# ucsdmanorlab/bootstrapper

Measured on AMD Instinct MI355X. Metric: Mvoxels/s predict+segment, 1024^3 vol in 128^3 blocks, higher is better.
Workload: dtype bf16x3

## Files before the change

### bootstrapper_amd/_lib.py

```python
import ctypes as C
import os

import torch

_HERE = os.path.dirname(os.path.abspath(__file__))
LIB_PATH = os.environ.get("BSMI_LIB") or os.path.join(_HERE, "libbsmi.so")

MAX_LEVELS, MAX_CONVS, MAX_HEADS, NAME_LEN = 8, 4, 4, 32
PREC_F32, PREC_BF16, PREC_BF16X3 = 0, 1, 2
RAW_U8, RAW_F32, RAW_U8_UNIT = 0, 1, 2
ERR_INVALID, ERR_HIP, ERR_STATE, ERR_MISSING, ERR_OVERFLOW = -1, -2, -3, -4, -5


class UNetConfig(C.Structure):
    _fields_ = [
        ("in_channels", C.c_int32),
        ("num_fmaps", C.c_int32),
        ("fmap_inc_factor", C.c_int32),
        ("num_levels", C.c_int32),
        ("downsample_factors", (C.c_int32 * 3) * MAX_LEVELS),
        ("n_convs_down", C.c_int32 * MAX_LEVELS),
        ("kernel_size_down", ((C.c_int32 * 3) * MAX_CONVS) * MAX_LEVELS),
        ("n_convs_up", C.c_int32 * MAX_LEVELS),
        ("kernel_size_up", ((C.c_int32 * 3) * MAX_CONVS) * MAX_LEVELS),
        ("num_heads", C.c_int32),
        ("head_name", (C.c_char * NAME_LEN) * MAX_HEADS),
        ("head_dims", C.c_int32 * MAX_HEADS),
        ("num_fmaps_out", C.c_int32),
    ]


class StepInfo(C.Structure):
    _fields_ = [("type", C.c_int32), ("materialised", C.c_int32), ("shape", C.c_int32 * 4), ("conv_index", C.c_int32),
                ("form", C.c_int32), ("flags", C.c_int32), ("bn", C.c_int32), ("ksteps", C.c_int32), ("head", C.c_int32),
                ("factor", C.c_int32 * 3), ("offset", C.c_int32 * 3), ("prefix", C.c_char * 64)]


class TrainWgradInfo(C.Structure):
    _fields_ = [(n, C.c_int32) for n in ("family", "residual", "n", "c", "cbase", "kx", "tile_n", "tile_c", "ranges", "lines_per_range",
                                         "det_workspace")]


class TrainStepInfo(C.Structure):
    _fields_ = [("type", C.c_int32), ("n_wgrad", C.c_int32), ("wgrad", TrainWgradInfo * 4), ("dgrad", C.c_int32), ("dgrad_raw", C.c_int32),
                ("dgrad_converted", C.c_int32), ("dgrad_bn", C.c_int32), ("dgrad_ksteps", C.c_int32), ("dgrad_split_k", C.c_int32),
                ("dgrad_scatter", C.c_int32), ("dgrad_residual", C.c_int32), ("border", C.c_int32 * 3), ("has_split", C.c_int32),
                ("bias", C.c_int32), ("up", C.c_int32), ("fwd_split", C.c_int32), ("deterministic", C.c_int32)]


WGRAD_FAMILIES = ("none", "wave-f32", "tiled-f32", "split-bf16")
TRAIN_TENSORS = {"dout": 0, "gmask": 1, "gsplit": 2, "gsplit_hi": 3, "gsplit_lo": 4, "dcat": 5, "head_dp": 6, "pad_count": 7}
STEP_TYPES = ("input", "conv", "pool", "up", "head")
CONV_FORMS = ("gather", "raster-halo", "box-halo", "halo-resident", "first-pass", "winograd F(2x2)", "winograd F(4x4)")
STEP_FLAGS = {1: "fused-up", 2: "res-low", 4: "split-k"}
STEP_BELOW_UP = 8


class Codec(C.Structure):
    _fields_ = [("id", C.c_int32), ("level", C.c_int32), ("cname", C.c_int32), ("shuffle", C.c_int32),
                ("typesize", C.c_int32), ("blocksize", C.c_int32)]


class ChunkCopy(C.Structure):
    _fields_ = [("path", C.c_char_p), ("base", C.c_void_p), ("start", C.c_int64 * 4), ("extent", C.c_int64 * 4),
                ("stride", C.c_int64 * 4), ("read_modify_write", C.c_int32), ("reserved", C.c_int32)]


class BatchFragArgs(C.Structure):
    _fields_ = [("affs_dev", C.c_void_p), ("frags_dev", C.c_void_p), ("max_id_dev", C.c_void_p), ("labels_dev", C.c_void_p),
                ("num_labels_dev", C.c_void_p), ("id_offset", C.c_uint64), ("size_dev", C.c_void_p), ("sums_dev", C.c_void_p)]


class BatchGraphArgs(C.Structure):
    _fields_ = [("affs_dev", C.c_void_p), ("frags_dev", C.c_void_p), ("edges_dev", C.c_void_p), ("sums_dev", C.c_void_p),
                ("pair_counts_dev", C.c_void_p), ("counts_dev", C.c_void_p), ("edge_capacity", C.c_uint64)]


class Aug2dDraw(C.Structure):
    _fields_ = [("a", C.c_float * 4), ("src", C.c_float * 2), ("inv_spacing", C.c_float * 2), ("flags", C.c_int32), ("n", C.c_int32 * 2),
                ("lattice_offset", C.c_int32), ("crop", C.c_int32 * 2), ("crop_offset", C.c_int32), ("reserved", C.c_int32)]


class Aug2dIDraw(C.Structure):
    _fields_ = [("seed", C.c_uint64), ("impulse_threshold", C.c_uint64), ("noise_sigma", C.c_float), ("contrast_scale", C.c_float),
                ("nodes", C.c_int32), ("radius", C.c_int32), ("taps_offset", C.c_int32), ("reserved", C.c_int32 * 3)]


CODEC_RAW, CODEC_ZLIB, CODEC_GZIP, CODEC_ZSTD, CODEC_LZ4, CODEC_BLOSC = range(6)
BLOSC_LZ4, BLOSC_ZLIB, BLOSC_ZSTD = 1, 3, 4
CHUNK_MISSING = 1
MORPH_DILATE, MORPH_ERODE = 0, 1
RESCALE_DOWN, RESCALE_UP = 0, 1


class BsmiError(RuntimeError):
    def __init__(self, code, msg):
        super().__init__(f"libbsmi error {code}: {msg}")
        self.code = code
        self.msg = msg


def _load():
    if not os.path.exists(LIB_PATH):
        raise ImportError(
            f"{LIB_PATH} not found: build it with `python -c 'import __graft_entry__ as g; g.build()'` "
            "(or `make -C bootstrapper_amd/csrc`).  There is no CPU fallback.")
    lib = C.CDLL(LIB_PATH)
    p, i32, i64p, vp = C.c_void_p, C.c_int, C.POINTER(C.c_int64), C.c_void_p
    sigs = {
        "bsmi_last_error": (C.c_char_p, []),
        "bsmi_version": (i32, []),
        "bsmi_unet_create": (i32, [C.POINTER(UNetConfig), i32, C.POINTER(p)]),
        "bsmi_unet_destroy": (i32, [p]),
        "bsmi_unet_load_weight": (i32, [p, C.c_char_p, vp, i64p, i32]),
        "bsmi_unet_finalize": (i32, [p, i32]),
        "bsmi_unet_output_shape": (i32, [p, i64p, i64p]),
        "bsmi_unet_flops": (i32, [p, i64p, C.POINTER(C.c_double)]),
        "bsmi_unet_forward": (i32, [p, i32, vp, i32, i64p, C.POINTER(vp), C.POINTER(vp), vp]),
        "bsmi_unet_debug_activation": (i32, [p, i32, i32, i64p, vp, C.c_uint64]),
        "bsmi_unet_debug_step_info": (i32, [p, i32, C.POINTER(StepInfo), C.POINTER(i32)]),
        "bsmi_unet_profile_enable": (i32, [p, i32]),
        "bsmi_unet_profile_read": (i32, [p, i32, C.POINTER(i32), C.POINTER(C.c_int32), C.POINTER(C.c_double),
                                         C.POINTER(C.c_double)]),
        "bsmi_unet_profile_totals": (i32, [p, C.POINTER(C.c_double), C.POINTER(C.c_double), i64p, i32]),
        "bsmi_extract_block_reflect_u8": (i32, [vp, i64p, i64p, i64p, vp, vp]),
        "bsmi_seg_create": (i32, [i32, i64p, C.POINTER(p)]),
        "bsmi_seg_destroy": (i32, [p]),
        "bsmi_ws_fragments_u8": (i32, [p, vp, i64p, i32, i32, vp, vp, vp]),
        "bsmi_ws_fragments_seeds_u8": (i32, [p, vp, i64p, i32, i32, vp, vp, vp, vp]),
        "bsmi_rag_agglomerate_u8": (i32, [p, vp, vp, i64p, C.c_float, C.c_int, vp]),
        "bsmi_rag_edge_stats": (i32, [p, vp, vp, C.c_uint64, vp]),
        "bsmi_agglomerate_mean_u8": (i32, [p, vp, vp, i64p, C.POINTER(C.c_float), i32, vp, vp]),
        "bsmi_agglomerate_hist_u8": (i32, [p, vp, vp, i64p, C.POINTER(C.c_float), i32, i32, i32, vp, vp]),
        "bsmi_agglomerate_hist_graph": (i32, [C.c_uint32, C.c_uint32, vp, vp, vp, i32, i32, C.POINTER(C.c_float), i32, vp]),
        "bsmi_frag_postprocess_u8": (i32, [p, vp, vp, i64p, C.c_double, C.c_int64, i64p, i64p, C.c_uint64, vp, vp, vp]),
        "bsmi_label_stats": (i32, [p, vp, i64p, C.c_uint64, C.c_uint64, vp, vp, vp]),
        "bsmi_rag_merge_scores_u8": (i32, [p, vp, vp, i64p, C.c_float, C.c_int, vp, vp, C.c_uint64, vp, vp, vp, vp]),
        "bsmi_lut_relabel": (i32, [C.c_int, vp, C.c_uint64, vp, vp, C.c_uint64, vp, vp]),
        "bsmi_lut_relabel_multi": (i32, [i32, vp, C.c_uint64, vp, vp, C.c_uint64, i32, vp, vp]),
        "bsmi_connected_components": (i32, [vp, C.c_uint64, vp, vp, C.c_uint64, C.c_float, vp]),
        "bsmi_connected_components_multi": (i32, [vp, C.c_uint64, vp, vp, C.c_uint64, vp, C.c_int, vp]),
        "bsmi_cc_affs_u8": (i32, [p, vp, i64p, C.c_int, C.c_int64, vp, vp, vp, vp]),
        "bsmi_mws_agglom_f64": (i32, [C.c_int, vp, C.c_int, vp, vp, C.c_uint32, i64p, vp, vp]),
        "bsmi_mws_cluster": (i32, [C.c_uint64, vp, vp, C.c_uint64, vp]),
        "bsmi_frag_pair_affinity_u8": (i32, [C.c_int, vp, C.c_int, vp, vp, i64p, C.c_uint64, vp, vp, vp, vp, vp]),
        "bsmi_label_table_u64": (i32, [p, vp, i64p, C.c_int64, vp, vp, vp, vp, C.c_uint64, vp, vp]),
        "bsmi_seg_status": (i32, [p, vp]),
        "bsmi_seg_set_host_flood": (i32, [p, i32]),
        "bsmi_seg_batch_create": (i32, [C.POINTER(p), i32, C.POINTER(p)]),
        "bsmi_seg_batch_destroy": (i32, [p]),
        "bsmi_seg_batch_fragments_u8": (i32, [p, i32, C.POINTER(BatchFragArgs), i64p, i32, i32, C.c_double, C.c_int64, i64p, i64p, C.c_uint64, vp]),
        "bsmi_seg_batch_rag_graph_u8": (i32, [p, i32, C.POINTER(BatchGraphArgs), i64p, vp]),
        "bsmi_rag_graph_u8": (i32, [p, vp, vp, i64p, vp, vp, vp, C.c_uint64, vp, vp]),
        "bsmi_rag_merge_scores_host": (i32, [i32, vp, vp, vp, vp, C.c_float, i32, vp, i32]),
        "bsmi_rag_merge_scores_host_rule": (i32, [i32, vp, vp, vp, vp, C.c_float, i32, i32, vp, i32]),
        "bsmi_unet_train_set_arithmetic": (i32, [p, i32]),
        "bsmi_unet_train_set_deterministic": (i32, [p, i32]),
        "bsmi_unet_train_begin": (i32, [p, i64p]),
        "bsmi_unet_train_forward_backward": (i32, [p, vp, C.POINTER(C.c_void_p), C.POINTER(C.c_void_p), C.POINTER(C.c_float), vp]),
        "bsmi_unet_train_num_params": (i32, [p, C.POINTER(C.c_uint64)]),
        "bsmi_unet_train_buffers": (i32, [p, C.POINTER(C.c_void_p), C.POINTER(C.c_void_p)]),
        "bsmi_unet_train_param_info": (i32, [p, C.c_char_p, C.POINTER(C.c_uint64), C.POINTER(C.c_uint64)]),
        "bsmi_unet_train_adam_step": (i32, [p, C.c_float, C.c_float, C.c_float, C.c_float, C.c_float, vp]),
        "bsmi_unet_train_read_param": (i32, [p, C.c_char_p, C.c_int, vp]),
        "bsmi_unet_train_last_loss": (i32, [p, C.POINTER(C.c_float), vp]),
        "bsmi_unet_train_prediction": (i32, [p, i32, C.POINTER(C.c_void_p), C.POINTER(C.c_uint64)]),
        "bsmi_unet_train_grad_groups": (i32, [p, i32, C.POINTER(i32), C.POINTER(C.c_uint64), C.POINTER(C.c_uint64)]),
        "bsmi_unet_train_wait_grad_group": (i32, [p, i32, vp]),
        "bsmi_unet_train_write_param": (i32, [p, C.c_char_p, C.c_int, vp]),
        "bsmi_unet_train_step_count": (i32, [p, C.c_int, C.POINTER(C.c_int)]),
        "bsmi_unet_train_end": (i32, [p]),
        "bsmi_unet_train_debug_tensor": (i32, [p, i32, i32, i64p, vp, C.c_uint64]),
        "bsmi_unet_train_debug_step_info": (i32, [p, i32, C.POINTER(TrainStepInfo)]),
        "bsmi_train_affinity_targets": (i32, [C.c_int, vp, vp, i64p, C.POINTER(C.c_int32), C.c_int, C.c_int, C.c_int, C.c_float,
                                              C.c_float, vp, vp, vp]),
        "bsmi_train_lsd_targets": (i32, [C.c_int, vp, vp, i64p, i64p, i64p, C.POINTER(C.c_float), C.POINTER(C.c_float), C.c_int, vp, vp, vp]),
        "bsmi_train_lsd2d_targets": (i32, [C.c_int, vp, vp, C.c_int, i64p, i64p, i64p, C.POINTER(C.c_float), C.POINTER(C.c_float), C.c_int,
                                           vp, vp, vp]),
        "bsmi_train_affinity_targets_roi": (i32, [C.c_int, vp, vp, C.c_int, i64p, i64p, i64p, C.POINTER(C.c_int32), C.c_int, C.c_int,
                                                  C.c_int, C.c_float, C.c_float, vp, vp, vp]),
        "bsmi_train_mask_sat": (i32, [C.c_int, vp, C.c_int, C.c_int, C.c_int, vp, vp]),
        "bsmi_unet_set_persistent_grid": (i32, [p, C.c_int]),
        "bsmi_unet_profile_executed": (i32, [p, C.POINTER(C.c_double), C.c_int]),
        "bsmi_debug_lds_canary": (i32, [i32, i32, i32, vp, vp]),
        "bsmi_debug_check_guards": (i32, []),
        "bsmi_stream_create_cu_mask": (i32, [C.c_int, vp, C.c_int, C.POINTER(C.c_void_p)]),
        "bsmi_stream_destroy": (i32, [C.c_int, vp]),
        "bsmi_eval_create": (i32, [i32, C.c_uint64, C.POINTER(p)]),
        "bsmi_eval_destroy": (i32, [p]),
        "bsmi_eval_aff_errors_u8": (i32, [p, vp, i64p, i64p, vp, i32, i64p, vp, C.POINTER(C.c_int32), i64p, C.c_float, C.c_float,
                                          C.c_int64, vp, vp, vp, vp]),
        "bsmi_eval_lsd_errors_u8": (i32, [p, vp, i64p, i64p, vp, vp, i64p, i64p, i64p, i64p, C.POINTER(C.c_float), C.POINTER(C.c_float),
                                          i32, C.c_float, C.c_float, C.c_int64, C.c_uint64, vp, vp, vp, vp, vp, vp, vp, vp]),
        "bsmi_eval_pairs_u64": (i32, [p, vp, vp, vp, i64p, i32, vp]),
        "bsmi_eval_pairs_read": (i32, [p, vp, vp, vp, C.c_uint64, vp, vp]),
        "bsmi_eval_status": (i32, [p, vp]),
        "bsmi_label_morph_u64": (i32, [i32, vp, i64p, i32, i32, i32, vp, vp, vp]),
        "bsmi_label_fill_holes_scratch_bytes": (C.c_size_t, [i64p, C.c_uint64]),
        "bsmi_label_fill_holes_u64": (i32, [i32, vp, i64p, i32, vp, vp, C.c_size_t, C.c_uint64, C.POINTER(C.c_uint64), vp]),
        "bsmi_mask_closing_work_bytes": (C.c_size_t, [i64p, i32]),
        "bsmi_mask_closing_disk_u8": (i32, [i32, vp, i64p, i32, vp, vp, C.c_size_t, vp]),
        "bsmi_downscale_mean": (i32, [i32, vp, i32, i64p, C.POINTER(C.c_int32), C.POINTER(C.c_int32), vp, i64p, vp]),
        "bsmi_rescale_sample": (i32, [i32, vp, i32, i64p, C.POINTER(C.c_int32), C.POINTER(C.c_int32), i32, vp, i64p, vp]),
        "bsmi_nonzero_bbox": (i32, [i32, vp, i32, i64p, i64p, vp, vp]),
        "bsmi_synth_create": (i32, [i32, i64p, C.POINTER(p)]),
        "bsmi_synth_destroy": (i32, [p]),
        "bsmi_synth_dilate_points": (i32, [p, i64p, vp, i32, vp, vp, vp, vp, vp]),
        "bsmi_synth_label_i32": (i32, [p, vp, i64p, vp, C.POINTER(C.c_uint64), vp]),
        "bsmi_synth_expand_i32": (i32, [p, vp, i64p, i32, C.c_int32, vp, vp]),
        "bsmi_synth_tubes_i32": (i32, [p, vp, i64p, vp, C.POINTER(C.c_uint64), vp]),
        "bsmi_synth_gaussian_f32": (i32, [p, vp, i64p, vp, i32, vp, vp]),
        "bsmi_synth_argmax_filter_f32": (i32, [p, vp, i64p, i32, vp, vp]),
        "bsmi_synth_basins_f32": (i32, [p, vp, vp, vp, i64p, vp, C.POINTER(C.c_uint64), vp]),
        "bsmi_synth_finish_i32": (i32, [p, vp, i64p, i32, i32, i32, vp, vp]),
        "bsmi_synth_grow_boundary_i64": (i32, [i32, vp, i64p, C.c_uint64, i32, vp, vp]),
        "bsmi_synth_merge_i64": (i32, [i32, vp, i64p, C.POINTER(C.c_int32), i32, C.c_int64, C.c_int64, vp]),
        "bsmi_synth_stamp_i64": (i32, [i32, vp, i64p, i32, i32, i32, vp, i32, i32, C.c_int64, vp]),
        "bsmi_synth_present_i64": (i32, [p, vp, C.c_uint64, vp, C.c_uint32, C.POINTER(C.c_uint32), vp]),
        "bsmi_synth_split_i64": (i32, [p, vp, i64p, C.c_int64, i32, C.POINTER(C.c_int32), i32, C.c_int64, C.POINTER(C.c_uint64), vp]),
        "bsmi_aug_coords": (i32, [i32, i64p, C.POINTER(C.c_float), C.POINTER(C.c_float), C.POINTER(C.c_float), i32, i32, vp, vp,
                                  C.POINTER(C.c_int32), C.POINTER(C.c_float), vp, vp]),
        "bsmi_aug_sample_f32_u8": (i32, [i32, vp, i64p, i64p, i64p, vp, i64p, vp, vp]),
        "bsmi_aug_sample_nearest_i64": (i32, [i32, vp, i64p, i64p, i64p, vp, i64p, vp, vp]),
        "bsmi_aug_sample_nearest_u8": (i32, [i32, vp, i64p, i64p, i64p, vp, i64p, vp, vp]),
        "bsmi_aug_sample_unit_f32_u8": (i32, [i32, vp, i64p, i64p, i64p, vp, i64p, vp, vp]),
        "bsmi_aug_noise_f32": (i32, [i32, i64p, vp, C.c_uint64, C.c_float, vp]),
        "bsmi_aug_section_stats_f32": (i32, [i32, i64p, vp, vp, vp, vp]),
        "bsmi_aug_intensity_f32": (i32, [i32, i64p, vp, vp, vp, vp, vp]),
        "bsmi_aug_gamma_f32": (i32, [i32, i64p, vp, vp, vp, vp]),
        "bsmi_aug_impulse_f32": (i32, [i32, i64p, vp, C.c_uint64, C.c_uint64, vp]),
        "bsmi_aug_smooth_f32": (i32, [i32, i64p, vp, vp, C.POINTER(C.c_float), i32, vp]),
        "bsmi_aug_defect_f32": (i32, [i32, i64p, vp, vp, vp, C.c_float, i32, vp]),
        "bsmi_aug2d_coords": (i32, [i32, C.POINTER(Aug2dDraw), vp, i32, i32, i64p, i64p, i64p, vp, vp, C.c_int64, vp, vp]),
        "bsmi_aug2d_sample_f32_u8": (i32, [i32, C.POINTER(Aug2dDraw), vp, i32, i32, vp, i64p, i64p, i64p, vp, C.c_int64, vp, vp]),
        "bsmi_aug2d_sample_nearest_i64": (i32, [i32, C.POINTER(Aug2dDraw), vp, i32, i32, vp, i64p, i64p, i64p, vp, C.c_int64, vp, vp]),
        "bsmi_aug2d_sample_nearest_u8": (i32, [i32, C.POINTER(Aug2dDraw), vp, i32, i32, vp, i64p, i64p, i64p, vp, C.c_int64, vp, vp]),
        "bsmi_aug2d_sample_unit_f32_u8": (i32, [i32, C.POINTER(Aug2dDraw), vp, C.POINTER(Aug2dIDraw), vp, i32, i32, vp, i64p, i64p, i64p, vp,
                                                C.c_int64, vp, vp]),
        "bsmi_aug2d_noise_f32": (i32, [i32, C.POINTER(Aug2dIDraw), vp, i32, i32, i64p, vp, vp]),
        "bsmi_aug2d_intensity_f32": (i32, [i32, C.POINTER(Aug2dIDraw), vp, i32, i32, i64p, vp, vp, vp, vp, vp]),
        "bsmi_aug2d_gamma_f32": (i32, [i32, C.POINTER(Aug2dIDraw), vp, i32, i32, i64p, vp, vp, vp, vp]),
        "bsmi_aug2d_impulse_f32": (i32, [i32, C.POINTER(Aug2dIDraw), vp, i32, i32, i64p, vp, vp]),
        "bsmi_aug2d_smooth_f32": (i32, [i32, C.POINTER(Aug2dIDraw), vp, i32, i32, i64p, vp, vp, vp, C.c_int64, vp]),
        "bsmi_aug2d_defect_f32": (i32, [i32, C.POINTER(Aug2dIDraw), vp, i32, i32, i64p, vp, vp, C.POINTER(C.c_int32), vp, i32, vp]),
        "bsmi_augin_group_mean_f32": (i32, [i32, i64p, vp, vp, i32, vp, vp]),
        "bsmi_augin_intensity_f32": (i32, [i32, i64p, vp, vp, vp, vp, i32, vp]),
        "bsmi_augin_smooth_f32": (i32, [i32, i64p, vp, vp, vp, vp, i32, vp]),
        "bsmi_augin_contrast_f32": (i32, [i32, i64p, vp, vp, vp, C.c_float, vp]),
        "bsmi_codec_bound": (C.c_size_t, [C.POINTER(Codec), C.c_size_t]),
        "bsmi_codec_decode": (i32, [C.POINTER(Codec), vp, C.c_size_t, vp, C.c_size_t, C.POINTER(C.c_size_t)]),
        "bsmi_codec_encode": (i32, [C.POINTER(Codec), vp, C.c_size_t, vp, C.c_size_t, C.POINTER(C.c_size_t)]),
        "bsmi_chunks_read": (i32, [C.POINTER(Codec), i32, C.POINTER(C.c_char_p), C.POINTER(vp), C.POINTER(C.c_size_t),
                                   C.POINTER(C.c_size_t), C.POINTER(i32), i32]),
        "bsmi_chunks_write": (i32, [C.POINTER(Codec), i32, C.POINTER(C.c_char_p), C.POINTER(vp), C.POINTER(C.c_size_t),
                                    C.POINTER(i32), i32]),
        "bsmi_blosc_dev_frame_bound": (C.c_size_t, [C.c_size_t]),
        "bsmi_blosc_dev_scratch_bytes": (C.c_size_t, [i32, C.c_size_t]),
        "bsmi_blosc_encode_dev_u64": (i32, [i32, vp, C.c_int64, C.c_int64, i32, i64p, i64p, i64p, vp, C.c_size_t, vp, C.c_size_t, vp, vp]),
        "bsmi_blosc_dev_u8_frame_bound": (C.c_size_t, [C.c_size_t]),
        "bsmi_blosc_dev_u8_scratch_bytes": (C.c_size_t, [i32, C.c_size_t]),
        "bsmi_blosc_encode_dev_u8": (i32, [i32, vp, i64p, i32, i64p, i64p, i64p, vp, C.c_size_t, vp, C.c_size_t, vp, vp]),
        "bsmi_rag_write_sqlite": (i32, [C.c_char_p, C.c_uint64, vp, vp, vp, C.c_uint64, vp, vp]),
        "bsmi_chunks_read_into": (i32, [C.POINTER(Codec), i32, C.POINTER(ChunkCopy), i64p, i32, vp, C.POINTER(i32), i32]),
        "bsmi_chunks_write_from": (i32, [C.POINTER(Codec), i32, C.POINTER(ChunkCopy), i64p, i32, vp, C.POINTER(i32), i32]),
    }
    for name, (res, args) in sigs.items():
        fn = getattr(lib, name)
        fn.restype = res
        fn.argtypes = args
    return lib, sorted(sigs)


lib, SYMBOLS = _load()
# ... 14 lines not shown
```

### bootstrapper_amd/csrc/unet_debug.hip

```cpp
#include <cstring>

#include "unet_internal.h"

extern "C" {

int bsmi_unet_debug_activation(bsmi_unet* h, int step, int what, int64_t shape_out[4], float* host_out, uint64_t capacity) {
  if (!h || !shape_out) BSMI_FAIL(BSMI_ERR_INVALID, "null argument");
  Plan* plan = h->last_plan;
  if (!plan) BSMI_FAIL(BSMI_ERR_STATE, "no forward has run");
  if (step < 0 || step >= (int)plan->steps.size()) BSMI_FAIL(BSMI_ERR_INVALID, "step %d out of range (%zu steps)", step, plan->steps.size());
  const PlanStep& st = plan->steps[step];
  if (st.type == PlanStep::HEAD) BSMI_FAIL(BSMI_ERR_INVALID, "head steps write into the caller's buffers");
  if (plan->fused_first && step < 2)
    BSMI_FAIL(BSMI_ERR_STATE, "step %d is not materialised: the first ConvPass ran as one launch (first_pass), which writes step 2 only", step);
  if (st.type == PlanStep::UP && st.skip)
    BSMI_FAIL(BSMI_ERR_STATE, "step %d is not materialised: the upsampling is fused into the Winograd stages that read it", step);
  const TDesc& t = st.out;
  shape_out[0] = t.D; shape_out[1] = t.H; shape_out[2] = t.W; shape_out[3] = t.C;
  if (!host_out) return BSMI_OK;
  const size_t nvox = (size_t)t.D * t.H * t.W;
  if (capacity < nvox * t.C) BSMI_FAIL(BSMI_ERR_INVALID, "buffer of %llu floats too small", (unsigned long long)capacity);
  BSMI_HIP(hipSetDevice(h->device));
  BSMI_HIP(hipDeviceSynchronize());
  const int es = esize(plan->prec);
  const bool split = t.lo_off != 0;
  const size_t bytes = nvox * t.Cpad * es * (split ? 2 : 1);
  std::vector<uint8_t> raw(bytes);
  BSMI_HIP(hipMemcpy(raw.data(), t.ptr, raw.size(), hipMemcpyDeviceToHost));
  for (size_t v = 0; v < nvox; ++v)
    for (int c = 0; c < t.C; ++c) {
      float x;
      if (plan->prec == BSMI_PREC_F32) {
        x = ((const float*)raw.data())[v * t.Cpad + c];
      } else if (!split) {
        x = host_bf16_to_f32(((const uint16_t*)raw.data())[v * t.Cpad + c]);
      } else {
        const size_t i = 2 * v * t.Cpad + (size_t)((c >> 3) << 4) + (c & 7);
        const float hi = host_bf16_to_f32(((const uint16_t*)raw.data())[i]);
        const float lo = host_bf16_to_f32(((const uint16_t*)raw.data())[i + 8]);
        x = what == 1 ? hi : (what == 2 ? lo : hi + lo);
      }
      host_out[v * t.C + c] = x;
    }
  return BSMI_OK;
}

int bsmi_unet_debug_step_info(bsmi_unet* h, int step, bsmi_unet_step_info* info, int* n_steps) {
  if (!h) BSMI_FAIL(BSMI_ERR_INVALID, "null handle");
  Plan* plan = h->last_plan;
  if (!plan) BSMI_FAIL(BSMI_ERR_STATE, "no forward has run");
  if (n_steps) *n_steps = (int)plan->steps.size();
  if (!info) return BSMI_OK;
  if (step < 0 || step >= (int)plan->steps.size()) BSMI_FAIL(BSMI_ERR_INVALID, "step %d out of range (%zu steps)", step, plan->steps.size());
  const PlanStep& st = plan->steps[step];
  memset(info, 0, sizeof *info);
  info->type = (int32_t)st.type;
  const bool in_first = plan->fused_first && step < 3;
  info->materialised = !((plan->fused_first && step < 2) || (st.type == PlanStep::UP && st.skip));
  const TDesc& t = st.type == PlanStep::HEAD ? st.in : st.out;
  info->shape[0] = t.D; info->shape[1] = t.H; info->shape[2] = t.W;
  info->shape[3] = st.type == PlanStep::HEAD ? h->heads[st.head].cout : t.C;
  const std::string* prefix = nullptr;
  if (st.type == PlanStep::HEAD) {
    info->head = st.head;
    prefix = &h->heads[st.head].prefix;
  } else if (st.type == PlanStep::POOL || st.type == PlanStep::UP) {
    for (int d = 0; d < 3; ++d) { info->factor[d] = st.f[d]; info->offset[d] = st.type == PlanStep::UP ? st.o[d] : 0; }
  } else if (st.type == PlanStep::CONV) {
    prefix = &st.site->prefix;
    info->conv_index = st.ci;
    const int sk_grid = h->sk_grid > 0 ? h->sk_grid : 0;
    if (in_first) {
      info->form = BSMI_FORM_FIRST_PASS;
    } else if (st.use_wino) {
      info->form = st.wino_in.m == 4 ? BSMI_FORM_WINO4 : BSMI_FORM_WINO2;
      info->bn = tile_bn(st.tile);
      info->ksteps = st.wino_gemm.nsteps;
      bool up = false;
      for (int q = 0; q < st.wino_in.nsrc; ++q) up = up || st.wino_in.upf[q] > 0;
      if (up || st.wino_out.low || st.wino_has_below) info->flags |= BSMI_STEP_FUSED_UP;
      if (st.wino_has_below) info->flags |= BSMI_STEP_BELOW_UP;
      if (st.wino_has_res_low) info->flags |= BSMI_STEP_RES_LOW;
      if (conv_igemm_split_k(st.wino_gemm, plan->prec, st.tile, sk_grid) ||
          (st.wino_has_res && conv_igemm_split_k(st.wino_res, plan->prec, st.tile, sk_grid)) ||
          (st.wino_has_res_low && conv_igemm_split_k(st.wino_res_low, plan->prec, st.tile, sk_grid)) ||
          (st.wino_has_below && conv_igemm_split_k(st.wino_below, plan->prec, st.below_tile, sk_grid)))
        info->flags |= BSMI_STEP_SPLIT_K;
    } else if (st.use_h16) {
      info->form = BSMI_FORM_HALO_RESIDENT;
      info->bn = st.h16.Npad;
      info->ksteps = st.h16.nsteps;
    } else if (st.use_box) {
      info->form = BSMI_FORM_BOX_HALO;
    } else if (st.use_rh) {
      info->form = BSMI_FORM_RASTER_HALO;
      info->bn = tile_bn(st.tile);
      info->ksteps = st.rh.nsteps;
      if (conv_rh_split_k(st.rh, st.tile, sk_grid)) info->flags |= BSMI_STEP_SPLIT_K;
    } else {
      info->form = BSMI_FORM_GATHER;
      info->bn = tile_bn(st.tile);
      info->ksteps = st.conv.nsteps;
      if (conv_igemm_split_k(st.conv, plan->prec, st.tile, sk_grid)) info->flags |= BSMI_STEP_SPLIT_K;
    }
  }
  if (prefix) snprintf(info->prefix, sizeof info->prefix, "%s", prefix->c_str());
  return BSMI_OK;
}

}
```

### bootstrapper_amd/csrc/unet_internal.h

```cpp
#pragma once
#include <cstring>
#include <map>
#include <memory>
#include <string>
#include <vector>

#include "conv_igemm.h"
#include "conv_rh.h"
#include "conv_h16.h"
#include "conv_box.h"
#include "first_pass.h"
#include "wino.h"

namespace bsmi {

struct HostWeight {
  std::vector<int64_t> shape;
  std::vector<float> data;
  bool loaded = false;
};

struct PackEntry {
  int slot;
  int dz, dy, dx;
  int c0;
  int wsrc;
  int tap;
  int cin_base;
  int creal;
  bool dummy;
  int phase;
};

struct PackPhase {
  int slot, c0, kind, first_unit, nunits;
};

struct PackedConv {
  bool ready = false;
  std::vector<PackEntry> entries;
  std::vector<PackPhase> phases;
  void* w = nullptr;
  int ks = 1;
  size_t lo_image_bytes = 0;
  float* bias = nullptr;
  int Npad = 0;
  TileCfg tile = TILE_256x32;
};

struct PackedWino {
  bool ready = false;
  int m = 2;
  bool fused_only = false;
  std::vector<WinoUnit> units;
  std::vector<int> cin_of_v;
  int Cv = 0;
  void* w = nullptr;
  size_t lo_image_bytes = 0, batch_bytes = 0;
  int Npad = 0;
  TileCfg tile = TILE_256x32;
  std::vector<PackEntry> res_entries;
  void* res_w = nullptr;
  size_t res_lo_image_bytes = 0;
  std::vector<PackEntry> res_part[2];
  void* res_part_w[2] = {nullptr, nullptr};
  size_t res_part_lo[2] = {0, 0};
  bool below_ready = false;
  std::vector<WinoUnit> skip_units, below_units;
  std::vector<int> skip_cin_of_v;
  int skip_Cv = 0;
  void* skip_w = nullptr;
  size_t skip_lo_image_bytes = 0, skip_batch_bytes = 0;
  void* below_w = nullptr;
  size_t below_lo_image_bytes = 0, below_batch_bytes = 0;
  int below_Npad = 0;
  bool below_dense = false;
  TileCfg below_tile = TILE_256x320;
};

struct H16PhaseHost {
  int slot, c0, dz, kind;
  int first_step, nsteps;
};
struct PackedH16 {
  bool ready = false;
  std::vector<PackEntry> entries;
  std::vector<H16PhaseHost> phases;
  void* w = nullptr;
  size_t lo_image_bytes = 0;
  int Npad = 0;
};

struct PassSite {
  std::string prefix;
  int nslots = 1;
  int cin[2] = {0, 0};
  int cout = 0;
  int nconv = 0;
  int k[BSMI_MAX_CONVS][3];
  PackedConv packed[BSMI_NUM_PREC][BSMI_MAX_CONVS];
  PackedWino wino[BSMI_MAX_CONVS];
  PackedH16 h16[BSMI_MAX_CONVS];
};

struct HeadSite {
  std::string prefix;
  int cin = 0, cout = 0;
  float* hw = nullptr;
  float* hb = nullptr;
};

struct TDesc {
  void* ptr = nullptr;
  int C = 0, Cpad = 0, D = 0, H = 0, W = 0;
  size_t lo_off = 0;
};

struct PlanStep {
  enum Type { INPUT, CONV, POOL, UP, HEAD } type;
  ConvArgs conv;
  RhArgs rh;
  bool use_rh = false;
  H16Args h16;
  bool use_h16 = false;
  int h16_rows = 0;
  BoxArgs box;
  bool use_box = false;
  bool use_wino = false;
  WinoInArgs wino_in;
  ConvArgs wino_gemm, wino_res, wino_res_low;
  bool wino_has_res = false, wino_has_res_low = false;
  ConvArgs wino_below;
  bool wino_has_below = false;
  TileCfg below_tile = TILE_256x320;
  WinoOutArgs wino_out;
  TileCfg tile;
  TDesc in, out;
  int f[3], o[3];
  bool skip = false;
  bool pool_fused = false;
  int head = 0;
  double flops = 0;
  double exec_flops = 0;
  struct PassSite* site = nullptr;
  int ci = 0;
  TDesc slots[kMaxConvTensors];
  int so[kMaxConvTensors][3] = {{0, 0, 0}, {0, 0, 0}, {0, 0, 0}};
  int nsl = 0;
  struct TrainFwdX3* tx3 = nullptr;
};

struct Plan {
  std::vector<float> last_ms;
  bool pending = false;
  std::vector<void*> allocs;
  std::vector<PlanStep> steps;
  int64_t out_shape[3] = {0, 0, 0};
  double flops = 0;
  size_t bytes = 0;
  std::vector<hipEvent_t> events;
  std::vector<std::vector<hipEvent_t>> inflight, spare;
  bool profiled = false;
  bool fused_first = false;
  int prec = 0;
};

struct TrainState;

static inline uint16_t host_f32_to_bf16(float f) {
  uint32_t u;
  memcpy(&u, &f, 4);
  if ((u & 0x7fffffffu) > 0x7f800000u) return (uint16_t)((u >> 16) | 0x40);
  u += 0x7fffu + ((u >> 16) & 1u);
  return (uint16_t)(u >> 16);
}
static inline float host_bf16_to_f32(uint16_t b) {
  const uint32_t u = (uint32_t)b << 16;
  float f;
  memcpy(&f, &u, 4);
  return f;
}

int esize(int prec);
int ksplit(int prec);
int bke(int prec);
int sube(int prec);
void build_entries(const PassSite& p, int ci, int prec, std::vector<PackEntry>& out, std::vector<PackPhase>* phases_out = nullptr);

}

using namespace bsmi;

struct bsmi_unet {
  bsmi_unet_config cfg;
  int device = 0;
  int nl = 0;
  std::vector<PassSite> l_conv, r_conv;
  std::vector<HeadSite> heads;
  int crop_factor[BSMI_MAX_LEVELS][3];
  std::map<std::string, HostWeight> weights;
  bool finalized[BSMI_NUM_PREC] = {false, false, false};
  int profile_period = 0;
  uint64_t profile_count = 0;
  Plan* last_plan = nullptr;
  double prof_ms[5] = {0, 0, 0, 0, 0}, prof_flops[5] = {0, 0, 0, 0, 0};
  double prof_exec = 0;
  int64_t prof_launches[5] = {0, 0, 0, 0, 0};
  std::map<std::vector<int64_t>, std::unique_ptr<Plan>> plans;
  float* sk_ws = nullptr;
  int sk_grid = 0;
  int sk_request = -1;
  bsmi::TrainState* train = nullptr;
  bool train_forward = false;
  int train_split = 1;
  int train_det = 0;
  bsmi::FirstPassWeights first_pass;
  bsmi::FirstPassWeights first_pass_x3;
};

namespace bsmi {
int pack_conv(bsmi_unet* h, PassSite& p, int ci, int prec);
int pack_wino(bsmi_unet* h, PassSite& p, int ci);
int pack_h16(bsmi_unet* h, PassSite& p, int ci);
void release(PackedConv& pc);
void release(PackedWino& pw);
void release(PackedH16& ph);

bool x3_fused_for(TileCfg tile);
bool wino_eligible(const PassSite& p, int ci);
int wino_tile_edge();
bool wino_narrow_last(const bsmi_unet* h, const PassSite& p, int ci);
bool below_up_site(const bsmi_unet* h, const PassSite& p, int ci);
bool fuse_up_enabled();
bool pool_fuse_enabled();
int h16_mode();
int h16_only_npad();
bool h16_balanced();
bool rh_enabled(int prec, TileCfg tile, size_t nsteps);
bool box_enabled();
bool first_pass_eligible(const bsmi_unet* h);

int check_shape_arg(const int64_t s[3]);
int get_plan(bsmi_unet* h, int precision, const int64_t in_shape[3], Plan** out);
int dry_plan(bsmi_unet* h, const int64_t in_shape[3], Plan& plan);
void free_plan(Plan* p);
void free_train_state(bsmi_unet* h);
int train_forward_conv_x3(bsmi_unet* h, const PlanStep& st, hipStream_t s);
int train_refresh_f32_images(bsmi_unet* h, hipStream_t s);
}
```

### bootstrapper_amd/csrc/unet_pack.hip

```cpp
#include <cstdlib>
#include <cstring>

#include "unet_internal.h"

#include "dev_guard.h"

namespace bsmi {

int esize(int prec) { return prec == BSMI_PREC_F32 ? 4 : 2; }
int ksplit(int prec) { return prec == BSMI_PREC_BF16X3 ? 3 : 1; }
int bke(int prec) { return kStepRowBytes / esize(prec); }
int sube(int prec) { return 32 / esize(prec); }

static inline void split_bf16(float v, uint16_t& hi, uint16_t& lo) {
  hi = host_f32_to_bf16(v);
  lo = host_f32_to_bf16(v - host_bf16_to_f32(hi));
}

template <class T>
static void release_image(T*& w) {
  if (w) (void)hipFree(w);
  w = nullptr;
}
void release(PackedConv& pc) {
// ... 27 lines not shown
  auto add_taps = [&](int slot, const int* k, int cin_base, int creal) {
    const int cpad = round_up(creal, kChanPad);
    if (cpad == SUB) {
      PackPhase ph{slot, 0, 0, (int)out.size(), 0};
      for (int z = 0; z < k[0]; ++z)
        for (int y = 0; y < k[1]; ++y)
          for (int x = 0; x < k[2]; x += kUnitsPerStep)
            for (int j = 0; j < kUnitsPerStep; ++j) {
              if (x + j < k[2])
                out.push_back(PackEntry{slot, z, y, x + j, 0, 0, (z * k[1] + y) * k[2] + x + j, cin_base, creal, false, (int)phases.size()});
              else
                out.push_back(PackEntry{slot, 0, 0, 0, 0, 0, 0, 0, 0, true, (int)phases.size()});
            }
      close_phase(ph);
      return;
    }
    for (int c32 = 0; c32 < cpad; c32 += kUnitsPerStep * SUB) {
      PackPhase ph{slot, c32, 0, (int)out.size(), 0};
      for (int z = 0; z < k[0]; ++z)
        for (int y = 0; y < k[1]; ++y)
          for (int x = 0; x < k[2]; ++x) {
            for (int c0 = c32; c0 < std::min(cpad, c32 + kUnitsPerStep * SUB); c0 += SUB)
              out.push_back(PackEntry{slot, z, y, x, c0, 0, (z * k[1] + y) * k[2] + x, cin_base, creal, false, (int)phases.size()});
            while ((out.size() - ph.first_unit) % kUnitsPerStep)
              out.push_back(PackEntry{slot, 0, 0, 0, 0, 0, 0, 0, 0, true, (int)phases.size()});
          }
      close_phase(ph);
    }
  };
  auto add_residual = [&](int slot, const int* crop, int cin_base, int creal) {
    const int cpad = round_up(creal, kChanPad);
    for (int c32 = 0; c32 < cpad; c32 += kUnitsPerStep * SUB) {
      PackPhase ph{slot, c32, 1, (int)out.size(), 0};
      for (int c0 = c32; c0 < std::min(cpad, c32 + kUnitsPerStep * SUB); c0 += SUB)
        out.push_back(PackEntry{slot, crop[0] / 2, crop[1] / 2, crop[2] / 2, c0, 1, 0, cin_base, creal, false, (int)phases.size()});
      close_phase(ph);
    }
  };
  const int* k = p.k[ci];
  if (ci == 0) {
    int base = 0;
    for (int s = 0; s < p.nslots; ++s) {
      add_taps(s, k, base, p.cin[s]);
      base += p.cin[s];
    }
  } else {
    add_taps(0, k, 0, p.cout);
  }
  if (last) {
    int crop[3] = {0, 0, 0};
    for (int i = 0; i < p.nconv; ++i)
      for (int d = 0; d < 3; ++d) crop[d] += p.k[i][d] - 1;
    const int first_slot = ci == 0 ? 0 : 1;
    int base = 0;
    for (int s = 0; s < p.nslots; ++s) {
      add_residual(first_slot + s, crop, base, p.cin[s]);
      base += p.cin[s];
    }
  }
  if ((out.size() / kUnitsPerStep) % 2)
    for (int j = 0; j < kUnitsPerStep; ++j) out.push_back(PackEntry{0, 0, 0, 0, 0, 0, 0, 0, 0, true, (int)phases.size() - 1});
  if (phases_out) *phases_out = phases;
}

int pack_conv(bsmi_unet* h, PassSite& p, int ci, int prec) {
  PackedConv& pc = p.packed[prec][ci];
  if (pc.ready) return BSMI_OK;
  pc.entries.clear();
  build_entries(p, ci, prec, pc.entries, &pc.phases);
  pc.tile = choose_tile(p.cout);
  pc.Npad = round_up(p.cout, tile_bn(pc.tile));
  const int BKE = bke(prec);
  const bool last = ci == p.nconv - 1;
  const HostWeight& wm = h->weights[p.prefix + ".conv_pass." + std::to_string(2 * ci) + ".weight"];
  const HostWeight& bm = h->weights[p.prefix + ".conv_pass." + std::to_string(2 * ci) + ".bias"];
  const HostWeight& wr = h->weights[p.prefix + ".residual.0.weight"];
  const HostWeight& br = h->weights[p.prefix + ".residual.0.bias"];
  const int64_t cin_m = wm.shape[1], ntap_m = wm.shape[2] * wm.shape[3] * wm.shape[4];
  const int64_t cin_r = wr.shape[1];
  const int SUB = sube(prec);
  const bool fused = prec == BSMI_PREC_BF16X3 && x3_fused_for(pc.tile);
  const int KS = pc.ks = fused ? 1 : ksplit(prec);
  const size_t nsteps = pc.entries.size() / kUnitsPerStep * KS;
  const size_t nelem = (nsteps * (size_t)pc.Npad + kWeightRowSlack) * BKE;
  std::vector<float> bias(pc.Npad, 0.f);
  for (int n = 0; n < p.cout; ++n) bias[n] = bm.data[n] + (last ? br.data[n] : 0.f);

  pc.lo_image_bytes = fused ? nelem * esize(prec) : 0;
  std::vector<uint8_t> packed(nelem * esize(prec) * (fused ? 2 : 1), 0);
  host_parallel_for((size_t)p.cout, [&](size_t n_) {
    const int n = (int)n_;
    for (size_t u = 0; u < pc.entries.size(); ++u) {
      const PackEntry& e = pc.entries[u];
      if (e.dummy) continue;
      const size_t s = u / kUnitsPerStep, j = u % kUnitsPerStep;
      for (int kk = 0; kk < SUB; ++kk) {
        const int c = e.c0 + kk;
        if (c >= e.creal) break;
        float v;
        if (e.wsrc == 0) v = wm.data[((size_t)n * cin_m + (e.cin_base + c)) * ntap_m + e.tap];
        else v = wr.data[(size_t)n * cin_r + (e.cin_base + c)];
        const size_t idx = (s * KS * pc.Npad + n) * BKE + j * SUB + kk;
        if (prec == BSMI_PREC_F32) {
          ((float*)packed.data())[idx] = v;
        } else if (prec == BSMI_PREC_BF16) {
          ((uint16_t*)packed.data())[idx] = host_f32_to_bf16(v);
        } else {
          uint16_t hi, lo;
          split_bf16(v, hi, lo);
          uint16_t* w16 = (uint16_t*)packed.data();
          if (fused) {
            w16[idx] = hi;
            w16[idx + nelem] = lo;
          } else {
            const size_t blk = (size_t)pc.Npad * BKE;
            w16[idx] = hi;
            w16[idx + blk] = hi;
            w16[idx + 2 * blk] = lo;
          }
        }
      }
    }
  });
  BSMI_HIP(hipMalloc(&pc.w, packed.size()));
  BSMI_HIP(hipMemcpy(pc.w, packed.data(), packed.size(), hipMemcpyHostToDevice));
  BSMI_HIP(hipMalloc((void**)&pc.bias, bias.size() * sizeof(float)));
  BSMI_HIP(hipMemcpy(pc.bias, bias.data(), bias.size() * sizeof(float), hipMemcpyHostToDevice));
  pc.ready = true;
  return BSMI_OK;
}

int pack_wino(bsmi_unet* h, PassSite& p, int ci) {
  PackedWino& pw = p.wino[ci];
  release(pw);
  pw.fused_only = wino_narrow_last(h, p, ci);
  if (!wino_eligible(p, ci) && !pw.fused_only) return BSMI_OK;
  const HostWeight& wm = h->weights[p.prefix + ".conv_pass." + std::to_string(2 * ci) + ".weight"];
  const HostWeight& wr = h->weights[p.prefix + ".residual.0.weight"];
  const int cin_m = (int)wm.shape[1];
  pw.cin_of_v.clear();
  if (ci == 0) {
    int base = 0;
    for (int s = 0; s < p.nslots; ++s) {
      for (int c = 0; c < round_up(p.cin[s], kChanPad); ++c) pw.cin_of_v.push_back(c < p.cin[s] ? base + c : -1);
      base += p.cin[s];
    }
  } else {
    for (int c = 0; c < round_up(p.cout, kChanPad); ++c) pw.cin_of_v.push_back(c < p.cout ? c : -1);
  }
  pw.Cv = (int)pw.cin_of_v.size();
  pw.m = wino_tile_edge();
  pw.tile = choose_tile(p.cout);
  pw.Npad = round_up(p.cout, tile_bn(pw.tile));
  wino_units(pw.Cv, pw.units);
  {
    size_t image_elems = 0, batch_elems = 0;
    static const bool on_host = [] { const char* e = getenv("BSMI_WINO_PACK_HOST"); return e && e[0] == '1'; }();
    if (on_host) {
      std::vector<uint16_t> packed;
      wino_pack_weights(wm.data.data(), p.cout, cin_m, pw.cin_of_v, pw.Npad, pw.units, packed, image_elems, batch_elems, pw.m);
      BSMI_HIP(hipMalloc(&pw.w, packed.size() * 2));
      BSMI_HIP(hipMemcpy(pw.w, packed.data(), packed.size() * 2, hipMemcpyHostToDevice));
    } else {
      const int rc = wino_pack_weights_dev(wm.data.data(), p.cout, cin_m, pw.cin_of_v, pw.Npad, pw.units, pw.m, &pw.w, image_elems, batch_elems);
      if (rc) return rc;
    }
    pw.lo_image_bytes = image_elems * 2;
    pw.batch_bytes = batch_elems * 2;
  }
  pw.res_entries.clear();
  if (ci == p.nconv - 1) {
    std::vector<PackEntry> all;
    build_entries(p, ci, BSMI_PREC_BF16X3, all);
    for (size_t u = 0; u + 1 < all.size(); u += kUnitsPerStep) {
      bool res = false;
      for (int j = 0; j < kUnitsPerStep; ++j) res |= !all[u + j].dummy && all[u + j].wsrc == 1;
      if (res)
        for (int j = 0; j < kUnitsPerStep; ++j) pw.res_entries.push_back(all[u + j]);
    }
    if ((pw.res_entries.size() / kUnitsPerStep) % 2)
      for (int j = 0; j < kUnitsPerStep; ++j) pw.res_entries.push_back(PackEntry{0, 0, 0, 0, 0, 0, 0, 0, 0, true, 0});
    const int64_t cin_r = wr.shape[1];
    auto pack_res = [&](const std::vector<PackEntry>& ents, void** w_out, size_t* lo_out) -> int {
      const size_t nsteps = ents.size() / kUnitsPerStep;
      const size_t nelem = (nsteps * (size_t)pw.Npad + kWeightRowSlack) * 32;
      std::vector<uint16_t> packed(2 * nelem, 0);
      for (size_t u = 0; u < ents.size(); ++u) {
        const PackEntry& e = ents[u];
        if (e.dummy) continue;
        const size_t s = u / kUnitsPerStep, j = u % kUnitsPerStep;
        for (int n = 0; n < p.cout; ++n)
          for (int kk = 0; kk < 16; ++kk) {
            const int c = e.c0 + kk;
            if (c >= e.creal) break;
            const float v = wr.data[(size_t)n * cin_r + (e.cin_base + c)];
            const size_t idx = (s * pw.Npad + n) * 32 + j * 16 + kk;
            split_bf16(v, packed[idx], packed[nelem + idx]);
          }
      }
      *lo_out = nelem * 2;
      BSMI_HIP(hipMalloc(w_out, packed.size() * 2));
      BSMI_HIP(hipMemcpy(*w_out, packed.data(), packed.size() * 2, hipMemcpyHostToDevice));
      return BSMI_OK;
    };
    int rc = pack_res(pw.res_entries, &pw.res_w, &pw.res_lo_image_bytes);
    if (rc) return rc;
    for (int part = 0; part < 2; ++part) pw.res_part[part].clear();
    if (p.nslots == 2) {
      const int up_slot = (ci == 0 ? 0 : 1) + 1;
      for (size_t u = 0; u + 1 < pw.res_entries.size(); u += kUnitsPerStep) {
        int slot = -1;
        for (int j = 0; j < kUnitsPerStep; ++j)
          if (!pw.res_entries[u + j].dummy) slot = pw.res_entries[u + j].slot;
        if (slot < 0) continue;
        for (int j = 0; j < kUnitsPerStep; ++j) pw.res_part[slot == up_slot ? 1 : 0].push_back(pw.res_entries[u + j]);
      }
      for (int part = 0; part < 2; ++part) {
        if ((pw.res_part[part].size() / kUnitsPerStep) % 2)
          for (int j = 0; j < kUnitsPerStep; ++j) pw.res_part[part].push_back(PackEntry{0, 0, 0, 0, 0, 0, 0, 0, 0, true, 0});
        if ((rc = pack_res(pw.res_part[part], &pw.res_part_w[part], &pw.res_part_lo[part]))) return rc;
      }
    }
  }
  if (below_up_site(h, p, ci) && pw.m == 4) {
    pw.skip_cin_of_v.assign(pw.cin_of_v.begin(), pw.cin_of_v.begin() + round_up(p.cin[0], kChanPad));
    pw.skip_Cv = (int)pw.skip_cin_of_v.size();
    wino_units(pw.skip_Cv, pw.skip_units);
    size_t image_elems = 0, batch_elems = 0;
    int rc = wino_pack_weights_dev(wm.data.data(), p.cout, cin_m, pw.skip_cin_of_v, pw.Npad, pw.skip_units, pw.m, &pw.skip_w, image_elems, batch_elems);
    if (rc) return rc;
    pw.skip_lo_image_bytes = image_elems * 2;
    pw.skip_batch_bytes = batch_elems * 2;
    const int cpad_low = round_up(p.cin[1], kChanPad), cpad_out = round_up(p.cout, kChanPad);
    wino_units(cpad_low, pw.below_units);
    pw.below_dense = p.cout <= 64;
    pw.below_tile = pw.below_dense ? TILE_256x320 : pw.tile;
    pw.below_Npad = pw.below_dense ? round_up(9 * cpad_out, tile_bn(pw.below_tile)) : pw.Npad;
    const size_t nsteps = pw.below_units.size() / kUnitsPerStep;
    const size_t tap_elems = nsteps * (size_t)pw.below_Npad * 32;
    const size_t nelem = (pw.below_dense ? 1 : 9) * tap_elems + (size_t)kWeightRowSlack * 32;
    std::vector<uint16_t> packed(2 * nelem, 0);
    const bool dense = pw.below_dense;
    const int cin1 = p.cin[1], cbase = p.cin[0];
    host_parallel_for((size_t)p.cout, [&](size_t n_) {
      const int n = (int)n_;
      for (size_t u = 0; u < pw.below_units.size(); ++u) {
        const WinoUnit& un = pw.below_units[u];
        if (un.dummy) continue;
        const size_t s = u / kUnitsPerStep, j = u % kUnitsPerStep;
        for (int kk = 0; kk < 16; ++kk) {
          const int c = un.vc0 + kk;
          if (c >= cin1) break;
          const float* g = wm.data.data() + (((size_t)n * cin_m + (cbase + c)) * 3 + un.kz) * 9;
          for (int tap = 0; tap < 9; ++tap) {
            const size_t idx = dense ? (s * pw.below_Npad + (size_t)tap * cpad_out + n) * 32 + j * 16 + kk
                                     : (size_t)tap * tap_elems + (s * pw.below_Npad + n) * 32 + j * 16 + kk;
            split_bf16(g[tap], packed[idx], packed[nelem + idx]);
          }
        }
      }
    });
    pw.below_lo_image_bytes = nelem * 2;
    pw.below_batch_bytes = dense ? 0 : tap_elems * 2;
    BSMI_HIP(hipMalloc(&pw.below_w, packed.size() * 2));
    BSMI_HIP(hipMemcpy(pw.below_w, packed.data(), packed.size() * 2, hipMemcpyHostToDevice));
    pw.below_ready = true;
  }
  pw.ready = true;
  return BSMI_OK;
}

static void build_entries_h16(const PassSite& p, int ci, std::vector<PackEntry>& out, std::vector<H16PhaseHost>& phases) {
  const bool last = ci == p.nconv - 1;
  const int* k = p.k[ci];
  const PackEntry dummy{0, 0, 0, 0, 0, 0, 0, 0, 0, true, 0};
  auto add_taps = [&](int slot, int cin_base, int creal) {
    const int cpad = round_up(creal, kChanPad);
    for (int z = 0; z < k[0]; ++z)
      for (int c0 = 0; c0 < cpad; c0 += 16) {
        H16PhaseHost ph{slot, c0, z, 0, (int)(out.size() / kUnitsPerStep), 0};
        const int ntap = k[1] * k[2];
        for (int i = 0; i < ntap; i += 2) {
          for (int j = 0; j < 2; ++j) {
            if (i + j < ntap) {
              const int y = (i + j) / k[2], x = (i + j) % k[2];
              out.push_back(PackEntry{slot, z, y, x, c0, 0, (z * k[1] + y) * k[2] + x, cin_base, creal, false, (int)phases.size()});
            } else {
              out.push_back(dummy);
            }
          }
          ++ph.nsteps;
        }
        phases.push_back(ph);
      }
  };
  if (ci == 0) {
    int base = 0;
    for (int s = 0; s < p.nslots; ++s) {
      add_taps(s, base, p.cin[s]);
      base += p.cin[s];
    }
  } else {
    add_taps(0, 0, p.cout);
  }
  if (last) {
    int crop[3] = {0, 0, 0};
    for (int i = 0; i < p.nconv; ++i)
      for (int d = 0; d < 3; ++d) crop[d] += p.k[i][d] - 1;
    const int first_slot = ci == 0 ? 0 : 1;
    int base = 0;
    for (int s = 0; s < p.nslots; ++s) {
      const int cpad = round_up(p.cin[s], kChanPad);
      for (int c0 = 0; c0 < cpad; c0 += 16) {
        phases.push_back(H16PhaseHost{first_slot + s, c0, crop[0] / 2, 1, (int)(out.size() / kUnitsPerStep), 1});
        out.push_back(PackEntry{first_slot + s, crop[0] / 2, crop[1] / 2, crop[2] / 2, c0, 1, 0, base, p.cin[s], false, (int)phases.size() - 1});
        out.push_back(dummy);
      }
// ... 43 lines not shown
```

### bootstrapper_amd/csrc/unet_plan.hip

```cpp
#include <algorithm>
#include <cmath>
#include <cstdlib>
#include <cstring>
#include <memory>

#include "unet_plan.h"

#include "dev_guard.h"

namespace bsmi {

int upload_ksteps(Plan* plan, const std::vector<KStep>& ks, ConvArgs& a) {
  KStep* dks = nullptr;
  BSMI_HIP(hipMalloc((void**)&dks, ks.size() * sizeof(KStep)));
  plan->allocs.push_back(dks);
  BSMI_HIP(hipMemcpy(dks, ks.data(), ks.size() * sizeof(KStep), hipMemcpyHostToDevice));
  a.steps = dks;
  a.nsteps = (int)ks.size();
  return BSMI_OK;
}

void set_strides(ConvArgs& a, const void* base, int H, int W, int C, int bytes_per_channel) {
  for (int sl = 0; sl < kMaxConvTensors; ++sl) {
    a.t[sl].base = (uint64_t)(uintptr_t)base;
// ... 308 lines not shown
    TDesc o;
    o.C = p.cout;
    o.D = sp[0] - (p.k[ci][0] - 1);
    o.H = sp[1] - (p.k[ci][1] - 1);
    o.W = sp[2] - (p.k[ci][2] - 1);
    if (o.D <= 0 || o.H <= 0 || o.W <= 0)
      BSMI_FAIL(BSMI_ERR_INVALID, "%s: input extent (%d,%d,%d) too small for kernel (%d,%d,%d)",
                p.prefix.c_str(), sp[0], sp[1], sp[2], p.k[ci][0], p.k[ci][1], p.k[ci][2]);
    int rc = alloc(o);
    if (rc) return rc;

    TDesc slots[kMaxConvTensors];
    int so[kMaxConvTensors][3] = {{0, 0, 0}, {0, 0, 0}, {0, 0, 0}};
    int nsl = 0;
    if (ci == 0) {
      for (int s = 0; s < p.nslots; ++s) {
        slots[nsl] = in[s];
        for (int d = 0; d < 3; ++d) so[nsl][d] = org[s][d];
        ++nsl;
      }
    } else {
      slots[nsl++] = cur;
      if (last)
        for (int s = 0; s < p.nslots; ++s) {
          slots[nsl] = in[s];
          for (int d = 0; d < 3; ++d) so[nsl][d] = org[s][d];
          ++nsl;
        }
    }

    const double M = (double)o.D * o.H * o.W;
    double kreal = 0;
    {
      std::vector<PackEntry> ents;
      build_entries(p, ci, prec, ents);
      for (auto& e : ents) if (!e.dummy) kreal += std::max(0, std::min(e.creal - e.c0, sube(prec)));
    }
    plan->flops += 2.0 * M * p.cout * kreal;

    if (!dry) {
      PackedConv& pc = p.packed[prec][ci];
      PlanStep st;
      st.type = PlanStep::CONV;
      st.tile = pc.tile;
      ConvArgs& a = st.conv;
      memset(&a, 0, sizeof a);
      const int KS = pc.ks;
      std::vector<KStep> ks(pc.entries.size() / kUnitsPerStep * KS);
      const int64_t es = esize(prec) * (prec == BSMI_PREC_BF16X3 ? 2 : 1);
      for (int sl = 0; sl < kMaxConvTensors; ++sl) {
        const TDesc& t = slots[sl < nsl ? sl : 0];
        a.t[sl].base = (uint64_t)(uintptr_t)t.ptr;
        a.t[sl].sz = (int32_t)((int64_t)t.H * t.W * t.Cpad * es);
        a.t[sl].sy = (int32_t)((int64_t)t.W * t.Cpad * es);
        a.t[sl].sx = (int32_t)((int64_t)t.Cpad * es);
      }
      for (size_t s = 0; s < ks.size() / KS; ++s) {
        const int slot = pc.entries[kUnitsPerStep * s].slot;
        const TDesc& t = slots[slot];
        KStep k;
        memset(&k, 0, sizeof k);
        k.tensor = slot;
        for (int j = 0; j < kUnitsPerStep; ++j) {
          const PackEntry& e = pc.entries[kUnitsPerStep * s + j];
          if (e.dummy) continue;
          const int64_t off = ((((int64_t)(e.dz + so[slot][0]) * t.H) + (e.dy + so[slot][1])) * t.W +
                               (e.dx + so[slot][2])) * t.Cpad + e.c0;
          k.delta[j] = (int32_t)(off * es);
        }
        ks[s * KS] = k;
        if (KS == 3) {
          KStep lo = k;
          for (int j = 0; j < kUnitsPerStep; ++j)
            if (!pc.entries[kUnitsPerStep * s + j].dummy) lo.delta[j] = (int32_t)(k.delta[j] + (int64_t)t.lo_off);
          ks[s * KS + 1] = lo;
          ks[s * KS + 2] = k;
        }
      }
      if ((rc = upload_ksteps(plan, ks, a))) return rc;
      a.w = pc.w;
      a.w_lo = pc.lo_image_bytes ? (const char*)pc.w + pc.lo_image_bytes : nullptr;
      a.bias = pc.bias;
      a.out = o.ptr;
      a.Do = o.D; a.Ho = o.H; a.Wo = o.W; a.Co = o.Cpad;
      a.M = o.D * o.H * o.W;
      a.Npad = pc.Npad;
      a.relu = 1;
      st.flops = 2.0 * M * p.cout * kreal;
      {
        const double x3 = prec == BSMI_PREC_BF16X3 ? 3.0 : 1.0;
        const double kstep = (double)kUnitsPerStep * sube(prec);
        st.exec_flops = 2.0 * (double)round_up(a.M, 256) * pc.Npad * ((double)(ks.size() / KS) * kstep) * x3;
      }
      st.site = &p;
      st.ci = ci;
      st.nsl = nsl;
      for (int sl = 0; sl < nsl; ++sl) {
        st.slots[sl] = slots[sl];
        for (int d = 0; d < 3; ++d) st.so[sl][d] = so[sl][d];
      }
      st.out = o;
      rc = plan_rh(p, ci, pc, slots, so, o, st);
      if (rc) return rc;
      rc = plan_box(p, ci, slots, so, o, st);
      if (rc) return rc;
      rc = plan_wino(p, ci, pc, slots, so, nsl, o, st);
      if (rc) return rc;
      if (!st.use_wino && !st.use_box) {
        rc = plan_h16(p, ci, pc, slots, so, o, st);
        if (rc) return rc;
      }
      if (getenv("BSMI_PLAN_DEBUG"))
        fprintf(stderr, "[bsmi plan] %s conv %d: out (%d,%d,%d)x%d tile BN=%d K-steps %d %s\n", p.prefix.c_str(), ci, o.D, o.H, o.W,
                p.cout, tile_bn(st.tile), st.use_wino ? st.wino_gemm.nsteps : a.nsteps,
                st.use_wino ? (st.wino_in.m == 4 ? "winograd F(4x4,3x3)" : "winograd F(2x2,3x3)") : st.use_h16 ? "halo-resident" : st.use_box ? "box-halo" : st.use_rh ? "raster-halo" : "gather");
      plan->steps.push_back(st);
    }
    cur = o;
    sp[0] = o.D; sp[1] = o.H; sp[2] = o.W;
  }
  out = cur;
  return BSMI_OK;
}

int Planner::rec(int level, const TDesc& f_in, TDesc& f_out) {
  const int i = h->nl - level - 1;
  TDesc f_left;
  const int org0[1][3] = {{0, 0, 0}};
  const int sp[3] = {f_in.D, f_in.H, f_in.W};
  int rc = pass(h->l_conv[i], &f_in, org0, sp, f_left);
  if (rc) return rc;
  if (level == 0) {
    f_out = f_left;
    return BSMI_OK;
  }
  const int* f = h->cfg.downsample_factors[i];
  const int dims[3] = {f_left.D, f_left.H, f_left.W};
  for (int d = 2; d >= 0; --d)
    if (dims[d] % f[d] != 0)
      BSMI_FAIL(BSMI_ERR_INVALID,
                "Can not downsample shape (%d, %d, %d) with factor (%d, %d, %d), mismatch in spatial dimension %d",
                dims[0], dims[1], dims[2], f[0], f[1], f[2], d);
  TDesc g_in;
  g_in.C = f_left.C; g_in.D = f_left.D / f[0]; g_in.H = f_left.H / f[1]; g_in.W = f_left.W / f[2];
  rc = alloc(g_in);
  if (rc) return rc;
  if (!dry) {
    PlanStep st;
    st.type = PlanStep::POOL;
    st.in = f_left; st.out = g_in;
    for (int d = 0; d < 3; ++d) st.f[d] = f[d];
    PlanStep& prod = plan->steps.back();
    if (pool_fuse_enabled() && prec == BSMI_PREC_BF16X3 && f[0] == 1 && f[1] == 2 && f[2] == 2 && prod.type == PlanStep::CONV && prod.use_wino &&
        prod.wino_out.m == 4 && !prod.wino_out.low && prod.wino_out.out == f_left.ptr && !(f_left.H & 1) && !(f_left.W & 1)) {
      prod.wino_out.pool = g_in.ptr;
      st.pool_fused = true;
    }
    plan->steps.push_back(st);
  }
  TDesc g_out;
  rc = rec(level - 1, g_in, g_out);
  if (rc) return rc;

  PassSite& rp = h->r_conv[i];
  const int up[3] = {g_out.D * f[0], g_out.H * f[1], g_out.W * f[2]};
  int conv_crop[3] = {0, 0, 0};
  for (int c = 0; c < rp.nconv; ++c)
    for (int d = 0; d < 3; ++d) conv_crop[d] += rp.k[c][d] - 1;
  int target[3];
  for (int d = 0; d < 3; ++d) {
    const int cf = h->crop_factor[i][d];
    const int n = (int)std::floor((double)(up[d] - conv_crop[d]) / cf);
    target[d] = n * cf + conv_crop[d];
    if (target[d] != up[d] && target[d] <= conv_crop[d])
      BSMI_FAIL(BSMI_ERR_INVALID,
                "Feature map with shape (%d, %d, %d) is too small to ensure translation equivariance",
                up[0], up[1], up[2]);
  }
  TDesc g_c;
  g_c.C = g_out.C; g_c.D = target[0]; g_c.H = target[1]; g_c.W = target[2];
  rc = alloc(g_c);
  if (rc) return rc;
  int so[2][3];
  for (int d = 0; d < 3; ++d) {
    so[0][d] = (dims[d] - target[d]) / 2;
    so[1][d] = 0;
    if (dims[d] < target[d])
      BSMI_FAIL(BSMI_ERR_INVALID, "skip connection (%d,%d,%d) smaller than upsampled map (%d,%d,%d)",
                dims[0], dims[1], dims[2], target[0], target[1], target[2]);
  }
  UpFuse uf;
  bool fuse = false;
  if (!dry && prec == BSMI_PREC_BF16X3 && f[0] == 1 && f[1] == 2 && f[2] == 2 && rp.nslots == 2 && rp.wino[0].ready &&
      rp.wino[rp.nconv - 1].ready && !rp.wino[rp.nconv - 1].res_part[1].empty() && g_out.ptr) {
    fuse = fuse_up_enabled();
    int sp[3] = {target[0], target[1], target[2]};
    for (int c = 0; c < rp.nconv && fuse; ++c) {
      for (int d = 0; d < 3; ++d) sp[d] -= rp.k[c][d] - 1;
      const int wm = rp.wino[c].m;
      if ((c == 0 || c == rp.nconv - 1) && ((wm == 2 && ((sp[1] & 1) || (sp[2] & 1))) || sp[0] <= 0 || sp[1] <= 0 || sp[2] <= 0)) fuse = false;
      if ((c == 0 || c == rp.nconv - 1) && (size_t)(sp[0] + 2) * ((sp[1] + wm - 1) / wm) * ((sp[2] + wm - 1) / wm) * rp.wino[c].Cv * 4 >= ((size_t)1 << 31)) fuse = false;
    }
  }
  if (!dry) {
    PlanStep st;
    st.type = PlanStep::UP;
    st.in = g_out; st.out = g_c;
    for (int d = 0; d < 3; ++d) { st.f[d] = f[d]; st.o[d] = (up[d] - target[d]) / 2; }
    st.skip = fuse;
    plan->steps.push_back(st);
  }
  if (fuse) {
    uf.low = g_out;
    for (int d = 0; d < 3; ++d) { uf.f[d] = f[d]; uf.o[d] = (up[d] - target[d]) / 2; }
    fuse_up = &uf;
    if (getenv("BSMI_PLAN_DEBUG")) fprintf(stderr, "[bsmi plan] %s: upsampling fused into the Winograd stages\n", rp.prefix.c_str());
  }
  const TDesc ins[2] = {f_left, g_c};
  rc = pass(rp, ins, so, target, f_out);
  fuse_up = nullptr;
  return rc;
}

int Planner::run(const int64_t in_shape[3]) {
  TDesc x;
  x.C = h->cfg.in_channels; x.D = (int)in_shape[0]; x.H = (int)in_shape[1]; x.W = (int)in_shape[2];
  int rc = alloc(x);
  if (rc) return rc;
  if (!dry) {
    PlanStep st;
    st.type = PlanStep::INPUT;
    st.out = x;
    plan->steps.push_back(st);
  }
  TDesc z;
  rc = rec(h->nl - 1, x, z);
  if (rc) return rc;
  plan->out_shape[0] = z.D; plan->out_shape[1] = z.H; plan->out_shape[2] = z.W;
  for (size_t hd = 0; hd < h->heads.size(); ++hd) {
    plan->flops += 2.0 * 2.0 * (double)z.D * z.H * z.W * h->heads[hd].cin * h->heads[hd].cout;
    if (!dry) {
      PlanStep st;
      st.type = PlanStep::HEAD;
      st.in = z;
      st.head = (int)hd;
      st.flops = 2.0 * 2.0 * (double)z.D * z.H * z.W * h->heads[hd].cin * h->heads[hd].cout;
      plan->steps.push_back(st);
    }
  }
  return BSMI_OK;
}

void free_plan(Plan* p) {
for (void* a : p->allocs) (void)hipFree(a);
p->allocs.clear();
for (auto* sets : {&p->inflight, &p->spare})
  for (auto& set : *sets)
    for (hipEvent_t e : set) (void)hipEventDestroy(e);
p->inflight.clear();
p->spare.clear();
p->events.clear();
}

int get_plan(bsmi_unet* h, int precision, const int64_t in_shape[3], Plan** out) {
  const std::vector<int64_t> key = {precision, in_shape[0], in_shape[1], in_shape[2]};
  auto it = h->plans.find(key);
  if (it == h->plans.end()) {
    std::unique_ptr<Plan> plan(new Plan);
    plan->prec = precision;
    Planner pl{h, precision, plan.get(), false};
    const int rc = pl.run(in_shape);
    if (rc) {
      free_plan(plan.get());
      return rc;
    }
    const std::vector<PlanStep>& ps = plan->steps;
    const bool fp_ready = precision == BSMI_PREC_BF16 ? h->first_pass.ready : precision == BSMI_PREC_BF16X3 && h->first_pass_x3.ready;
    plan->fused_first = fp_ready && first_pass_eligible(h) && ps.size() > 3 &&
                        ps[0].type == PlanStep::INPUT && ps[1].type == PlanStep::CONV && ps[2].type == PlanStep::CONV &&
                        ps[1].site == &h->l_conv[0] && ps[2].site == &h->l_conv[0] && ps[2].out.Cpad == 16;
    if (plan->fused_first && plan->steps[3].type == PlanStep::POOL && plan->steps[3].pool_fused) {
      plan->steps[3].pool_fused = false;
      plan->steps[2].wino_out.pool = nullptr;
    }
    BSMI_HIP(hipDeviceSynchronize());
    it = h->plans.emplace(key, std::move(plan)).first;
  }
  *out = it->second.get();
  return BSMI_OK;
}

int check_shape_arg(const int64_t s[3]) {
  for (int d = 0; d < 3; ++d)
    if (s[d] <= 0 || s[d] > 4096) BSMI_FAIL(BSMI_ERR_INVALID, "bad input shape (%lld,%lld,%lld)", (long long)s[0], (long long)s[1], (long long)s[2]);
  return BSMI_OK;
}

int dry_plan(bsmi_unet* h, const int64_t in_shape[3], Plan& plan) {
  int rc = check_shape_arg(in_shape);
  if (rc) return rc;
  Planner pl{h, BSMI_PREC_BF16, &plan, true};
  return pl.run(in_shape);
}

}
```

### bootstrapper_amd/csrc/unet_plan_wino.hip

```cpp
#include <cstring>

#include "unet_plan.h"

#include "dev_guard.h"

namespace bsmi {

namespace {

void raw_gemm(ConvArgs& a, const void* w, size_t lo_image_bytes, int Npad) {
  a.w = w;
  a.w_lo = (const char*)w + lo_image_bytes;
  a.Npad = Npad;
  a.relu = 0;
  a.raw = 1;
  a.nbatch = 0;
  a.a_batch = a.w_batch = 0;
}

struct WinoStage {
  Plan* plan;
  const UpFuse* fuse_up;
  const PassSite& p;
  int ci;
  const PackedConv& pc;
  const PackedWino& pw;
  const TDesc* slots;
  const int (*so)[3];
  const TDesc& o;
  PlanStep& st;
  bool below;
  bool cut;
  int wm, nbatch, Dv, Ty, Tx, Cv;
  size_t vbatch, Mrows;
  void *V = nullptr, *Mbuf = nullptr, *addend = nullptr, *low = nullptr, *Ybuf = nullptr;
  size_t Mbelow = 0;
  int low_off[3] = {0, 0, 0}, below_off[3] = {0, 0, 0};

  int input_transform() {
    WinoInArgs& wi = st.wino_in;
    memset(&wi, 0, sizeof wi);
    const int nsrc = below ? 1 : ci == 0 ? p.nslots : 1;
    int cv0 = 0;
    for (int q = 0; q < nsrc; ++q) {
      const TDesc& t = slots[q];
      wi.src[q] = t.ptr;
      wi.H[q] = t.H; wi.W[q] = t.W; wi.Cpad[q] = t.Cpad;
      wi.oz[q] = so[q][0]; wi.oy[q] = so[q][1]; wi.ox[q] = so[q][2];
      wi.cv0[q] = cv0;
      cv0 += t.Cpad;
      if (fuse_up && ci == 0 && q == 1) {
        if (fuse_up->low.Cpad != t.Cpad) BSMI_FAIL(BSMI_ERR_STATE, "%s: fused upsampling with a different channel padding", p.prefix.c_str());
        wi.src[q] = fuse_up->low.ptr;
        wi.H[q] = fuse_up->low.H; wi.W[q] = fuse_up->low.W;
        wi.oz[q] += fuse_up->o[0]; wi.oy[q] += fuse_up->o[1]; wi.ox[q] += fuse_up->o[2];
        wi.upf[q] = fuse_up->f[1];
      }
    }
    if (cv0 != Cv) BSMI_FAIL(BSMI_ERR_STATE, "%s conv %d: winograd channel layout %d != %d", p.prefix.c_str(), ci, cv0, Cv);
    wi.nsrc = nsrc;
    wi.V = V;
    wi.Dv = Dv; wi.Ty = Ty; wi.Tx = Tx; wi.Cv = Cv;
    wi.m = wm;
    return BSMI_OK;
  }

  int batched_gemm() {
    const std::vector<WinoUnit>& units = below ? pw.skip_units : pw.units;
    ConvArgs& g = st.wino_gemm;
    memset(&g, 0, sizeof g);
    set_strides(g, V, Ty, Tx, Cv, 4);
    std::vector<KStep> ks(units.size() / kUnitsPerStep);
    for (size_t s = 0; s < ks.size(); ++s) {
      KStep k;
      memset(&k, 0, sizeof k);
      for (int j = 0; j < kUnitsPerStep; ++j) {
        const WinoUnit& u = units[kUnitsPerStep * s + j];
        if (!u.dummy) k.delta[j] = (int32_t)(((int64_t)u.kz * Ty * Tx * Cv + u.vc0) * 4);
      }
      ks[s] = k;
    }
    const int rc = upload_ksteps(plan, ks, g);
    if (rc) return rc;
    raw_gemm(g, below ? pw.skip_w : pw.w, below ? pw.skip_lo_image_bytes : pw.lo_image_bytes, pw.Npad);
    g.bias = pc.bias;
    g.out = Mbuf;
    g.Do = o.D; g.Ho = Ty; g.Wo = Tx; g.Co = o.Cpad;
    g.M = (int)Mrows;
    g.nbatch = nbatch;
    g.a_batch = (int64_t)vbatch;
    g.w_batch = (int64_t)(below ? pw.skip_batch_bytes : pw.batch_bytes);
    return BSMI_OK;
  }

  int below_up() {
    const TDesc& lt = fuse_up->low;
    for (int d = 0; d < 3; ++d) below_off[d] = so[1][d] + fuse_up->o[d];
    if (fuse_up->f[1] != 2 || fuse_up->f[2] != 2 || lt.Cpad != slots[1].Cpad || below_off[0] < 0 || below_off[0] + o.D + 2 > lt.D || below_off[1] < 0 ||
        below_off[2] < 0 || below_off[1] + o.H + 2 > 2 * lt.H || below_off[2] + o.W + 2 > 2 * lt.W)
      BSMI_FAIL(BSMI_ERR_STATE, "%s: the low-resolution tensor does not cover the stage's input", p.prefix.c_str());
    Mbelow = (size_t)o.D * lt.H * lt.W;
    const size_t ybytes = 9 * Mbelow * o.Cpad * sizeof(float);
    if (Mbelow * 9 >= ((size_t)1 << 31)) BSMI_FAIL(BSMI_ERR_STATE, "%s: too many rows of sums below the upsampling", p.prefix.c_str());
    BSMI_HIP(hipMalloc(&Ybuf, ybytes));
    plan->allocs.push_back(Ybuf);
    plan->bytes += ybytes;
    ConvArgs& r = st.wino_below;
    memset(&r, 0, sizeof r);
    set_strides(r, lt.ptr, lt.H, lt.W, lt.Cpad, 4);
    std::vector<KStep> ks(pw.below_units.size() / kUnitsPerStep);
    for (size_t s = 0; s < ks.size(); ++s) {
      KStep k;
      memset(&k, 0, sizeof k);
      for (int j = 0; j < kUnitsPerStep; ++j) {
        const WinoUnit& u = pw.below_units[kUnitsPerStep * s + j];
        if (!u.dummy) k.delta[j] = (int32_t)(((int64_t)(u.kz + below_off[0]) * lt.H * lt.W * lt.Cpad + u.vc0) * 4);
      }
      ks[s] = k;
    }
    const int rc = upload_ksteps(plan, ks, r);
    if (rc) return rc;
    raw_gemm(r, pw.below_w, pw.below_lo_image_bytes, pw.below_Npad);
    r.bias = pc.bias;
    r.out = Ybuf;
    r.Do = o.D; r.Ho = lt.H; r.Wo = lt.W;
    r.Co = pw.below_dense ? 9 * o.Cpad : o.Cpad;
    r.M = (int)Mbelow;
    r.nbatch = pw.below_dense ? 0 : 9;
    r.w_batch = (int64_t)pw.below_batch_bytes;
    st.below_tile = pw.below_tile;
    st.wino_has_below = true;
    return BSMI_OK;
  }

  int residual_low() {
    const TDesc& g = fuse_up->low;
    const size_t Mlow = (size_t)g.D * g.H * g.W;
    BSMI_HIP(hipMalloc(&low, Mlow * o.Cpad * sizeof(float)));
    plan->allocs.push_back(low);
    plan->bytes += Mlow * o.Cpad * sizeof(float);
    ConvArgs& r = st.wino_res_low;
    memset(&r, 0, sizeof r);
    set_strides(r, g.ptr, g.H, g.W, g.Cpad, 4);
    const std::vector<PackEntry>& ents = pw.res_part[1];
    std::vector<KStep> ks(ents.size() / kUnitsPerStep);
    int up_slot = -1;
    for (size_t s = 0; s < ks.size(); ++s) {
      KStep k;
      memset(&k, 0, sizeof k);
      for (int j = 0; j < kUnitsPerStep; ++j) {
        const PackEntry& e = ents[kUnitsPerStep * s + j];
        if (e.dummy) continue;
        k.delta[j] = (int32_t)((int64_t)e.c0 * 4);
        up_slot = e.slot;
        low_off[0] = e.dz; low_off[1] = e.dy; low_off[2] = e.dx;
      }
      ks[s] = k;
    }
    if (up_slot < 0) BSMI_FAIL(BSMI_ERR_STATE, "%s: empty low-resolution residual", p.prefix.c_str());
    for (int d = 0; d < 3; ++d) low_off[d] += so[up_slot][d] + fuse_up->o[d];
    const int rc = upload_ksteps(plan, ks, r);
    if (rc) return rc;
    raw_gemm(r, pw.res_part_w[1], pw.res_part_lo[1], pw.Npad);
    r.bias = pc.bias;
    r.out = low;
    r.Do = g.D; r.Ho = g.H; r.Wo = g.W; r.Co = o.Cpad;
    r.M = (int)Mlow;
    st.wino_has_res_low = true;
    return BSMI_OK;
  }

  int residual() {
    const std::vector<PackEntry>& res_entries = cut ? pw.res_part[0] : pw.res_entries;
    BSMI_HIP(hipMalloc(&addend, (size_t)o.D * o.H * o.W * o.Cpad * sizeof(float)));
    plan->allocs.push_back(addend);
    plan->bytes += (size_t)o.D * o.H * o.W * o.Cpad * sizeof(float);
    ConvArgs& r = st.wino_res;
    r = st.conv;
    std::vector<KStep> ks(res_entries.size() / kUnitsPerStep);
    for (size_t s = 0; s < ks.size(); ++s) {
      KStep k;
      memset(&k, 0, sizeof k);
      const PackEntry& e0 = res_entries[kUnitsPerStep * s];
      k.tensor = e0.dummy ? 0 : e0.slot;
      for (int j = 0; j < kUnitsPerStep; ++j) {
        const PackEntry& e = res_entries[kUnitsPerStep * s + j];
        if (e.dummy) continue;
        const TDesc& t = slots[e.slot];
        const int64_t off = ((((int64_t)(e.dz + so[e.slot][0]) * t.H) + (e.dy + so[e.slot][1])) * t.W + (e.dx + so[e.slot][2])) * t.Cpad + e.c0;
        k.delta[j] = (int32_t)(off * 4);
      }
      ks[s] = k;
    }
    const int rc = upload_ksteps(plan, ks, r);
    if (rc) return rc;
    raw_gemm(r, cut ? pw.res_part_w[0] : pw.res_w, cut ? pw.res_part_lo[0] : pw.res_lo_image_bytes, pw.Npad);
    r.out = addend;
    return BSMI_OK;
  }

  void output_transform(int prec) {
    WinoOutArgs& wo = st.wino_out;
    memset(&wo, 0, sizeof wo);
    wo.M = (const float*)Mbuf;
    wo.addend = (const float*)addend;
    if (cut) {
      wo.low = (const float*)low;
      wo.lD = fuse_up->low.D; wo.lH = fuse_up->low.H; wo.lW = fuse_up->low.W;
      wo.lf = fuse_up->f[1];
      wo.loz = low_off[0]; wo.loy = low_off[1]; wo.lox = low_off[2];
    }
    if (below) {
      wo.below = (const float*)Ybuf;
      wo.btap = pw.below_dense ? (int64_t)o.Cpad : (int64_t)Mbelow * o.Cpad;
      wo.brow = pw.below_dense ? 9 * o.Cpad : o.Cpad;
      wo.boy = below_off[1]; wo.box = below_off[2];
      wo.lD = fuse_up->low.D; wo.lH = fuse_up->low.H; wo.lW = fuse_up->low.W;
      wo.lf = fuse_up->f[1];
    }
    wo.bias = pc.bias;
    wo.out = o.ptr;
    wo.Do = o.D; wo.Ty = Ty; wo.Tx = Tx; wo.Co = o.Cpad;
    wo.m = wm; wo.Ho = o.H; wo.Wo = o.W;
    wo.relu = 1;
    const double kstep = (double)kUnitsPerStep * sube(prec);
    st.exec_flops = 2.0 * (double)round_up((int)Mrows, 256) * pw.Npad * ((double)st.wino_gemm.nsteps * kstep) * nbatch * 3.0;
    if (st.wino_has_res) st.exec_flops += 2.0 * (double)round_up(st.wino_res.M, 256) * pw.Npad * ((double)st.wino_res.nsteps * kstep) * 3.0;
    if (st.wino_has_res_low) st.exec_flops += 2.0 * (double)round_up(st.wino_res_low.M, 256) * pw.Npad * ((double)st.wino_res_low.nsteps * kstep) * 3.0;
    if (st.wino_has_below)
      st.exec_flops += 2.0 * (double)round_up(st.wino_below.M, 256) * pw.below_Npad * (pw.below_dense ? 1 : 9) * ((double)st.wino_below.nsteps * kstep) * 3.0;
  }
};

}

int Planner::plan_wino(PassSite& p, int ci, const PackedConv& pc, const TDesc* slots, const int (*so)[3], int nsl, const TDesc& o, PlanStep& st) {
  st.use_wino = false;
  const PackedWino& pw = p.wino[ci];
  const bool wants_fused = fuse_up && (ci == 0 || ci == p.nconv - 1);
  if (pw.fused_only && !fuse_up) return BSMI_OK;
  const int wm = pw.m, nbatch = wino_batches(wm);
  if (prec != BSMI_PREC_BF16X3 || !pw.ready || (wm == 2 && ((o.H & 1) || (o.W & 1))) || st.use_box || st.use_rh) {
    if (wants_fused) BSMI_FAIL(BSMI_ERR_STATE, "%s conv %d: the upsampling was fused into this stage, which cannot take the Winograd form", p.prefix.c_str(), ci);
    return BSMI_OK;
  }
  const bool below = fuse_up && ci == 0 && pw.below_ready && wm == 4 && nsl == 2;
  const int Dv = o.D + 2, Ty = (o.H + wm - 1) / wm, Tx = (o.W + wm - 1) / wm, Cv = below ? pw.skip_Cv : pw.Cv;
  const size_t vbatch = (size_t)Dv * Ty * Tx * Cv * 4;
  if (vbatch >= ((size_t)1 << 31)) {
    if (wants_fused) BSMI_FAIL(BSMI_ERR_STATE, "%s conv %d: fused upsampling, but the transformed input is too large", p.prefix.c_str(), ci);
    return BSMI_OK;
  }
  const size_t Mrows = (size_t)o.D * Ty * Tx;
  const bool cut = fuse_up && ci == p.nconv - 1;
  WinoStage w{plan, fuse_up, p, ci, pc, pw, slots, so, o, st, below, cut, wm, nbatch, Dv, Ty, Tx, Cv, vbatch, Mrows};
  BSMI_HIP(hipMalloc(&w.V, nbatch * vbatch + 4096));
  plan->allocs.push_back(w.V);
  BSMI_HIP(hipMalloc(&w.Mbuf, nbatch * Mrows * o.Cpad * sizeof(float)));
  plan->allocs.push_back(w.Mbuf);
  plan->bytes += nbatch * (vbatch + Mrows * o.Cpad * sizeof(float));
  int rc = w.input_transform();
  if (rc || (rc = w.batched_gemm())) return rc;
  st.wino_has_below = false;
  if (below && (rc = w.below_up())) return rc;
  if (cut && (pw.res_part[0].empty() || pw.res_part[1].empty())) BSMI_FAIL(BSMI_ERR_STATE, "%s: fused upsampling without a cut residual branch", p.prefix.c_str());
  st.wino_has_res = !(cut ? pw.res_part[0] : pw.res_entries).empty();
  st.wino_has_res_low = false;
  if (cut && (rc = w.residual_low())) return rc;
  if (st.wino_has_res && (rc = w.residual())) return rc;
  w.output_transform(prec);
  st.tile = pw.tile;
  st.use_wino = true;
  return BSMI_OK;
}

}
```

### bootstrapper_amd/csrc/unet_rules.hip

```cpp
#include <cstdlib>

#include "unet_internal.h"

namespace bsmi {

static int x3_fused_mode() {
  static const int m = [] { const char* e = getenv("BSMI_X3_FUSED"); return e ? atoi(e) : 1; }();
  return m;
}
bool x3_fused_for(TileCfg tile) {
  if (!two_waves_per_simd()) return false;
  return x3_fused_mode() == 1 || x3_fused_mode() == 2 || (x3_fused_mode() == 3 && tile != TILE_256x320);
}

static int wino_mode() {
  static const int m = [] { const char* e = getenv("BSMI_WINO"); return e ? atoi(e) : 1; }();
  return m;
}

static int wino4_mode() {
  static const int m = [] { const char* e = getenv("BSMI_WINO4"); return e ? atoi(e) : 1; }();
  return m;
}
int wino_tile_edge() { return wino4_mode() == 0 ? 2 : 4; }

bool wino_eligible(const PassSite& p, int ci) {
  if (wino_mode() == 0 || p.k[ci][0] != 3 || p.k[ci][1] != 3 || p.k[ci][2] != 3) return false;
  if (ci == 0 && p.nslots > kWinoMaxSrc) return false;
  if (!x3_fused_for(choose_tile(p.cout))) return false;
  if (wino_mode() >= 2) return true;
  int cin = p.cout;
  if (ci == 0) {
    cin = 0;
    for (int s = 0; s < p.nslots; ++s) cin += p.cin[s];
  }
  if (cin >= 256 && p.cout >= 256) return true;
  return wino4_mode() == 1 && (int64_t)cin * p.cout >= 16384 && cin >= 32 && p.cout >= 32;
}

static bool fuse_up_narrow() {
  static const bool on = [] { const char* e = getenv("BSMI_FUSE_UP_NARROW"); return !(e && e[0] == '0'); }();
  return on;
}
bool wino_narrow_last(const bsmi_unet* h, const PassSite& p, int ci) {
  if (!fuse_up_narrow() || wino_mode() == 0 || p.nslots != 2 || p.nconv < 2 || ci != p.nconv - 1) return false;
  if (&p < h->r_conv.data() || &p >= h->r_conv.data() + h->r_conv.size()) return false;
  const int* f = h->cfg.downsample_factors[&p - h->r_conv.data()];
  if (f[0] != 1 || f[1] != 2 || f[2] != 2) return false;
  if (p.k[ci][0] != 3 || p.k[ci][1] != 3 || p.k[ci][2] != 3 || p.cout < 32 || !x3_fused_for(choose_tile(p.cout))) return false;
  return wino_eligible(p, 0) && !wino_eligible(p, ci);
}

static int conv_below_up_mode() {
  static const int m = [] { const char* e = getenv("BSMI_CONV_BELOW_UP"); return e ? atoi(e) : -1; }();
  return m;
}
bool below_up_site(const bsmi_unet* h, const PassSite& p, int ci) {
  if (conv_below_up_mode() == 0 || ci != 0 || p.nslots != 2 || p.nconv < 2 || !wino_eligible(p, 0)) return false;
  if (&p < h->r_conv.data() || &p >= h->r_conv.data() + h->r_conv.size()) return false;
  const int* f = h->cfg.downsample_factors[&p - h->r_conv.data()];
  if (f[0] != 1 || f[1] != 2 || f[2] != 2) return false;
  if (p.cout <= 64 && !x3_fused_for(TILE_256x320)) return false;
  return true;
}

bool fuse_up_enabled() {
  static const bool on = [] { const char* e = getenv("BSMI_FUSE_UP"); return !(e && e[0] == '0'); }();
  return on;
}
bool pool_fuse_enabled() {
  static const bool pool_fuse = [] { const char* e = getenv("BSMI_POOL_FUSE"); return !(e && e[0] == '0'); }();
  return pool_fuse;
}

int h16_mode() {
  static const int m = [] { const char* e = getenv("BSMI_H16"); return e ? atoi(e) : 1; }();
  return m;
}
int h16_only_npad() {
  static const int only_npad = [] { const char* e = getenv("BSMI_H16_NPAD"); return e ? atoi(e) : 0; }();
  return only_npad;
}
bool h16_balanced() {
  static const bool balanced = [] { const char* e = getenv("BSMI_H16_BALANCE"); return !(e && e[0] == '0'); }();
  return balanced;
}

bool rh_enabled(int prec, TileCfg tile, size_t nsteps) {
  static const int mode = [] { const char* e = getenv("BSMI_USE_RH"); return !e ? 2 : (e[0] == '1' ? 1 : 0); }();
  return prec != BSMI_PREC_BF16X3 && (mode == 1 || (mode == 2 && tile_bn(tile) <= 64 && nsteps >= 200));
}

bool box_enabled() {
  static const bool enabled = [] { const char* e = getenv("BSMI_USE_BOX"); return !(e && e[0] == '0'); }();
  return enabled;
}

bool first_pass_eligible(const bsmi_unet* h) {
  if (h->cfg.in_channels != 1 || h->l_conv.empty()) return false;
  const PassSite& p = h->l_conv[0];
  if (p.nconv != 2 || p.cout > 16) return false;
  for (int c = 0; c < 2; ++c)
    for (int d = 0; d < 3; ++d)
      if (p.k[c][d] != 3) return false;
  const char* e = getenv("BSMI_FUSED_FIRST");
  return !(e && e[0] == '0');
}

}
```

### bootstrapper_amd/csrc/wino.h

```cpp
#pragma once
#include <vector>

#include "conv_igemm.h"

namespace bsmi {

constexpr int kWinoBatch = 16;
constexpr int kWinoMaxBatch = 36;
inline int wino_batches(int m) { return (m + 2) * (m + 2); }
constexpr int kWinoMaxSrc = 2;

struct WinoInArgs {
  const void* src[kWinoMaxSrc];
  int H[kWinoMaxSrc], W[kWinoMaxSrc], Cpad[kWinoMaxSrc];
  int oz[kWinoMaxSrc], oy[kWinoMaxSrc], ox[kWinoMaxSrc];
  int cv0[kWinoMaxSrc];
  int upf[kWinoMaxSrc];
  int nsrc;
  void* V;
  int Dv, Ty, Tx, Cv;
  int m;
};

struct WinoOutArgs {
  const float* M;
  const float* addend;
  const float* low;
  int lD, lH, lW, lf, loz, loy, lox;
  const float* below;
  int64_t btap;
  int brow, boy, box;
  const float* bias;
  void* out;
  int Do, Ty, Tx, Co;
  int relu;
  int m, Ho, Wo;
  void* pool;
};

int launch_wino_in(const WinoInArgs& a, hipStream_t s);
int launch_wino_out(const WinoOutArgs& a, hipStream_t s);

struct WinoUnit {
  int kz, vc0;
  bool dummy;
};
void wino_units(int Cv, std::vector<WinoUnit>& out);

void wino_pack_weights(const float* w, int cout, int cin, const std::vector<int>& cin_of_v, int Npad, const std::vector<WinoUnit>& units,
                       std::vector<uint16_t>& packed, size_t& image_elems, size_t& batch_elems, int m = 2);

int wino_pack_weights_dev(const float* w, int cout, int cin, const std::vector<int>& cin_of_v, int Npad, const std::vector<WinoUnit>& units, int m,
                          void** image_dev, size_t& image_elems, size_t& batch_elems);

}
```

### bootstrapper_amd/csrc/wino.hip

```cpp
#include "wino.h"

#include <cstdlib>
#include <cstring>

#include "dev_guard.h"

namespace bsmi {

typedef uint32_t u32x4_t __attribute__((ext_vector_type(4)));
typedef float f32x4_t __attribute__((ext_vector_type(4)));

namespace {

__device__ __forceinline__ uint16_t to_bf16(float f) {
  __bf16 h = (__bf16)f;
  return __builtin_bit_cast(uint16_t, h);
}
__device__ __forceinline__ void unpack8(u32x4_t v, float* f) {
  const uint32_t w[4] = {v.x, v.y, v.z, v.w};
#pragma unroll
  for (int i = 0; i < 4; ++i) {
    f[2 * i] = __uint_as_float(w[i] << 16);
    f[2 * i + 1] = __uint_as_float(w[i] & 0xffff0000u);
  }
// ... 202 lines not shown
    float mm[4][8];
#pragma unroll
    for (int xi = 0; xi < 4; ++xi) {
      const float* p = a.M + ((size_t)(4 * xi + nu) * Mrows + m) * a.Co + 8 * cv;
      const f32x4_t v0 = __builtin_nontemporal_load((const f32x4_t*)p);
      const f32x4_t v1 = __builtin_nontemporal_load((const f32x4_t*)(p + 4));
#pragma unroll
      for (int k = 0; k < 4; ++k) {
        mm[xi][k] = v0[k];
        mm[xi][4 + k] = v1[k];
      }
    }
#pragma unroll
    for (int k = 0; k < 8; ++k) {
      tp[0][nu][k] = mm[0][k] + mm[1][k] + mm[2][k];
      tp[1][nu][k] = mm[1][k] - mm[2][k] - mm[3][k];
    }
  }
#pragma unroll
  for (int p = 0; p < 2; ++p)
#pragma unroll
    for (int k = 0; k < 8; ++k) {
      y[p][0][k] = tp[p][0][k] + tp[p][1][k] + tp[p][2][k];
      y[p][1][k] = tp[p][1][k] - tp[p][2][k] - tp[p][3][k];
    }
  float bv[8];
#pragma unroll
  for (int k = 0; k < 8; ++k) bv[k] = a.bias[8 * cv + k];
  const int Ho = 2 * a.Ty, Wo = 2 * a.Tx;
  uint16_t* out = (uint16_t*)a.out;
#pragma unroll
  for (int p = 0; p < 2; ++p)
#pragma unroll
    for (int q = 0; q < 2; ++q) {
      const size_t e = (((size_t)z * Ho + (2 * ty + p)) * Wo + (2 * tx + q)) * a.Co + 8 * cv;
      float v[8];
#pragma unroll
      for (int k = 0; k < 8; ++k) v[k] = y[p][q][k] + bv[k];
      if (a.addend) {
        const f32x4_t r0 = __builtin_nontemporal_load((const f32x4_t*)(a.addend + e));
        const f32x4_t r1 = __builtin_nontemporal_load((const f32x4_t*)(a.addend + e + 4));
#pragma unroll
        for (int k = 0; k < 4; ++k) {
          v[k] += r0[k];
          v[4 + k] += r1[k];
        }
      }
      if constexpr (LOW) {
        int y0, y1, x0, x1;
        float wy0, wy1, wx0, wx1;
        lin_src(2 * ty + p + a.loy, a.lf, a.lH, y0, y1, wy0, wy1);
        lin_src(2 * tx + q + a.lox, a.lf, a.lW, x0, x1, wx0, wx1);
        const float* base = a.low + ((size_t)(z + a.loz) * a.lH * a.lW) * a.Co + 8 * cv;
        float r[4][8];
        const size_t o[4] = {((size_t)y0 * a.lW + x0) * a.Co, ((size_t)y0 * a.lW + x1) * a.Co, ((size_t)y1 * a.lW + x0) * a.Co,
                             ((size_t)y1 * a.lW + x1) * a.Co};
#pragma unroll
        for (int t4 = 0; t4 < 4; ++t4) {
          const f32x4_t r0 = *(const f32x4_t*)(base + o[t4]);
          const f32x4_t r1 = *(const f32x4_t*)(base + o[t4] + 4);
#pragma unroll
          for (int k = 0; k < 4; ++k) {
            r[t4][k] = r0[k];
            r[t4][4 + k] = r1[k];
          }
        }
#pragma unroll
        for (int k = 0; k < 8; ++k) {
          const float pa = wx0 * r[0][k] + wx1 * r[1][k];
          const float pb = wx0 * r[2][k] + wx1 * r[3][k];
          v[k] += wy0 * pa + wy1 * pb;
        }
      }
      if (a.relu) {
#pragma unroll
        for (int k = 0; k < 8; ++k) v[k] = v[k] > 0.f ? v[k] : 0.f;
      }
      store_split8<false>(out, e, v);
    }
}


constexpr float kR2 = 1.41421356237309504880f;
__host__ __device__ constexpr float bt4(int i, int j) {
  constexpr float B[6][6] = {{1.f, 0.f, -2.5f, 0.f, 1.f, 0.f},
                             {0.f, kR2, 2.f, -0.5f * kR2, -1.f, 0.f},
                             {0.f, -kR2, 2.f, 0.5f * kR2, -1.f, 0.f},
                             {0.f, -kR2, -1.f, 2.f * kR2, 2.f, 0.f},
                             {0.f, kR2, -1.f, -2.f * kR2, 2.f, 0.f},
                             {0.f, 1.f, 0.f, -2.5f, 0.f, 1.f}};
  return B[i][j];
}
__device__ __forceinline__ void bt4_apply(const float (*d)[4], float (*r)[4]) {
#pragma unroll
  for (int k = 0; k < 4; ++k) {
    const float e = 2.f * d[2][k] - d[4][k], o = kR2 * (d[1][k] - 0.5f * d[3][k]);
    const float e2 = 2.f * d[4][k] - d[2][k], o2 = kR2 * (2.f * d[3][k] - d[1][k]);
    r[0][k] = d[0][k] - 2.5f * d[2][k] + d[4][k];
    r[1][k] = e + o;
    r[2][k] = e - o;
    r[3][k] = e2 + o2;
    r[4][k] = e2 - o2;
    r[5][k] = d[1][k] - 2.5f * d[3][k] + d[5][k];
  }
}
__device__ __forceinline__ void at4_apply(const float (*m)[4], float (*y)[4]) {
  constexpr float a = 0.70710678118654752440f, b = kR2, a3 = 0.35355339059327376220f, b3 = 2.82842712474619009760f;
#pragma unroll
  for (int k = 0; k < 4; ++k) {
    const float s12 = m[1][k] + m[2][k], d12 = m[1][k] - m[2][k], s34 = m[3][k] + m[4][k], d34 = m[3][k] - m[4][k];
    y[0][k] = m[0][k] + s12 + s34;
    y[1][k] = a * d12 + b * d34;
    y[2][k] = 0.5f * s12 + 2.f * s34;
    y[3][k] = a3 * d12 + b3 * d34 + m[5][k];
  }
}
typedef uint32_t u32x2_t __attribute__((ext_vector_type(2)));
__device__ __forceinline__ void load_split4(const uint16_t* base, size_t e, int hf, float* f) {
  const uint16_t* p = base + 2 * e + 4 * hf;
  const u32x2_t h = *(const u32x2_t*)p, l = *(const u32x2_t*)(p + 8);
  f[0] = __uint_as_float(h.x << 16) + __uint_as_float(l.x << 16);
  f[1] = __uint_as_float(h.x & 0xffff0000u) + __uint_as_float(l.x & 0xffff0000u);
  f[2] = __uint_as_float(h.y << 16) + __uint_as_float(l.y << 16);
  f[3] = __uint_as_float(h.y & 0xffff0000u) + __uint_as_float(l.y & 0xffff0000u);
}
__device__ __forceinline__ void store_split4(uint16_t* base, size_t e, int hf, const float* f) {
  uint16_t* p = base + 2 * e + 4 * hf;
  uint16_t hb[4], lb[4];
#pragma unroll
  for (int k = 0; k < 4; ++k) {
    hb[k] = to_bf16(f[k]);
    lb[k] = to_bf16(f[k] - __uint_as_float((uint32_t)hb[k] << 16));
  }
  const u32x2_t hv = {(uint32_t)hb[0] | ((uint32_t)hb[1] << 16), (uint32_t)hb[2] | ((uint32_t)hb[3] << 16)};
  const u32x2_t lv = {(uint32_t)lb[0] | ((uint32_t)lb[1] << 16), (uint32_t)lb[2] | ((uint32_t)lb[3] << 16)};
  *(u32x2_t*)p = hv;
  *(u32x2_t*)(p + 8) = lv;
}
__device__ __forceinline__ uint32_t swap_pair(uint32_t v) { return (uint32_t)__builtin_amdgcn_update_dpp(0, (int)v, 0xB1, 0xf, 0xf, false); }
__device__ __forceinline__ void store_split4_pair(uint16_t* p, int hf, const float* f) {
  uint16_t hb[4], lb[4];
#pragma unroll
  for (int k = 0; k < 4; ++k) {
    hb[k] = to_bf16(f[k]);
    lb[k] = to_bf16(f[k] - __uint_as_float((uint32_t)hb[k] << 16));
  }
  const u32x2_t hv = {(uint32_t)hb[0] | ((uint32_t)hb[1] << 16), (uint32_t)hb[2] | ((uint32_t)hb[3] << 16)};
  const u32x2_t lv = {(uint32_t)lb[0] | ((uint32_t)lb[1] << 16), (uint32_t)lb[2] | ((uint32_t)lb[3] << 16)};
  const uint32_t r0 = swap_pair(hf ? hv.x : lv.x), r1 = swap_pair(hf ? hv.y : lv.y);
  const u32x4_t o = {hf ? r0 : hv.x, hf ? r1 : hv.y, hf ? lv.x : r0, hf ? lv.y : r1};
  __builtin_nontemporal_store(o, (u32x4_t*)p);
}

__global__ __launch_bounds__(256, 2) void wino4_in_kernel(const WinoInArgs a, int src, size_t total, int S, int nseg) {
  const unsigned nb = gridDim.x, q = nb >> 3, r = nb & 7, xcd = blockIdx.x & 7, j = blockIdx.x >> 3;
  const unsigned blk = (xcd < r ? xcd * (q + 1) : r * (q + 1) + (xcd - r) * q) + j;
  const size_t i = (size_t)blk * blockDim.x + threadIdx.x;
  if (i >= total) return;
  const int ncg = a.Cpad[src] >> 2;
  const int cg = (int)(i % ncg), cv = cg >> 1, hf = cg & 1;
  size_t t = i / ncg;
  const int tx0 = (int)(t % nseg) * S, tx1 = tx0 + S < a.Tx ? tx0 + S : a.Tx;
  t /= nseg;
  const int ty = (int)(t % a.Ty);
  const int z = (int)(t / a.Ty);
  const uint16_t* sp = (const uint16_t*)a.src[src];
  const int H = a.H[src], W = a.W[src], C = a.Cpad[src];
  size_t erow[6];
#pragma unroll
  for (int rr = 0; rr < 6; ++rr) {
    int y = 4 * ty + a.oy[src] + rr;
    y = y < H - 1 ? y : H - 1;
    erow[rr] = (((size_t)(z + a.oz[src]) * H + y) * W) * C + 8 * cv;
  }
  const size_t plane = (size_t)a.Dv * a.Ty * a.Tx * a.Cv;
  const size_t e_out = (((size_t)z * a.Ty + ty) * a.Tx) * a.Cv + a.cv0[src] + 8 * cv;
  float col[6][6][4];
  auto load_col = [&](int c, int x) __attribute__((always_inline)) {
    x += a.ox[src];
    x = x < W - 1 ? x : W - 1;
    float d[6][4];
#pragma unroll
    for (int rr = 0; rr < 6; ++rr) load_split4(sp, erow[rr] + (size_t)x * C, hf, d[rr]);
    bt4_apply(d, col[c]);
  };
  load_col(0, 4 * tx0);
  load_col(1, 4 * tx0 + 1);
  uint16_t* vt = (uint16_t*)a.V + 2 * (e_out + (size_t)tx0 * a.Cv) + 8 * hf;
  for (int tx = tx0; tx < tx1; ++tx) {
#pragma unroll
    for (int c = 2; c < 6; ++c) load_col(c, 4 * tx + c);
    uint16_t* vp = vt;
#pragma unroll
    for (int xi = 0; xi < 6; ++xi) {
      float in[6][4], v[6][4];
#pragma unroll
      for (int c = 0; c < 6; ++c)
#pragma unroll
        for (int k = 0; k < 4; ++k) in[c][k] = col[c][xi][k];
      bt4_apply(in, v);
#pragma unroll
      for (int nu = 0; nu < 6; ++nu) {
        store_split4_pair(vp, hf, v[nu]);
        vp += 2 * plane;
      }
    }
    vt += 2 * a.Cv;
#pragma unroll
    for (int xi = 0; xi < 6; ++xi)
#pragma unroll
      for (int k = 0; k < 4; ++k) {
        col[0][xi][k] = col[4][xi][k];
        col[1][xi][k] = col[5][xi][k];
      }
  }
}

__host__ __device__ constexpr float up4(int par, int row, int k) {
  const int f = par ? row / 2 : (row + 1) / 2;
  const bool first_heavy = par ? (row & 1) == 0 : (row & 1) == 1;
  return k == f ? (first_heavy ? 0.75f : 0.25f) : (k == f + 1 ? (first_heavy ? 0.25f : 0.75f) : 0.f);
}
__host__ __device__ constexpr float tu4(int par, int xi, int k) {
  float s = 0.f;
  for (int r = 0; r < 6; ++r) s += bt4(xi, r) * up4(par, r, k);
  return s;
}
template <int PY, int PX>
__global__ __launch_bounds__(256, 2) void wino4_in_up_kernel(const WinoInArgs a, int src, size_t total, int S, int nseg) {
  const unsigned nb = gridDim.x, q = nb >> 3, r = nb & 7, xcd = blockIdx.x & 7, j = blockIdx.x >> 3;
  const unsigned blk = (xcd < r ? xcd * (q + 1) : r * (q + 1) + (xcd - r) * q) + j;
  const size_t i = (size_t)blk * blockDim.x + threadIdx.x;
  if (i >= total) return;
  const int ncg = a.Cpad[src] >> 2;
  const int cg = (int)(i % ncg), cv = cg >> 1, hf = cg & 1;
  size_t t = i / ncg;
  const int tx0 = (int)(t % nseg) * S, tx1 = tx0 + S < a.Tx ? tx0 + S : a.Tx;
  t /= nseg;
  const int ty = (int)(t % a.Ty);
  const int z = (int)(t / a.Ty);
  const uint16_t* sp = (const uint16_t*)a.src[src];
  const int H = a.H[src], W = a.W[src], C = a.Cpad[src];
  const size_t e_low = ((size_t)(z + a.oz[src]) * H) * W * C + 8 * cv;
  const int ay = ((4 * ty + a.oy[src]) >> 1) - 1 + PY;
  int wy[5];
#pragma unroll
  for (int k = 0; k < 5; ++k) {
    const int y = ay + k;
    wy[k] = y < 0 ? 0 : (y > H - 1 ? H - 1 : y);
  }
  const int bx = (a.ox[src] >> 1) - 1 + PX;
  const size_t plane = (size_t)a.Dv * a.Ty * a.Tx * a.Cv;
  const size_t e_out = (((size_t)z * a.Ty + ty) * a.Tx) * a.Cv + a.cv0[src] + 8 * cv;
  float ct[5][6][4];
  auto load_ct = [&](int c, int xlow) __attribute__((always_inline)) {
    const int x = xlow < 0 ? 0 : (xlow > W - 1 ? W - 1 : xlow);
    float L[5][4];
#pragma unroll
    for (int k = 0; k < 5; ++k) load_split4(sp, e_low + ((size_t)wy[k] * W + x) * C, hf, L[k]);
#pragma unroll
    for (int xi = 0; xi < 6; ++xi)
#pragma unroll
      for (int ch = 0; ch < 4; ++ch) {
        float acc = 0.f;
#pragma unroll
        for (int k = 0; k < 5; ++k)
          if (tu4(PY, xi, k) != 0.f) acc += tu4(PY, xi, k) * L[k][ch];
        ct[c][xi][ch] = acc;
      }
  };
  load_ct(0, bx + 2 * tx0);
  load_ct(1, bx + 2 * tx0 + 1);
  load_ct(2, bx + 2 * tx0 + 2);
  uint16_t* vt = (uint16_t*)a.V + 2 * (e_out + (size_t)tx0 * a.Cv) + 8 * hf;
  for (int tx = tx0; tx < tx1; ++tx) {
    load_ct(3, bx + 2 * tx + 3);
    load_ct(4, bx + 2 * tx + 4);
    uint16_t* vp = vt;
#pragma unroll
    for (int xi = 0; xi < 6; ++xi) {
#pragma unroll
      for (int nu = 0; nu < 6; ++nu) {
        float v[4];
#pragma unroll
        for (int ch = 0; ch < 4; ++ch) {
          float acc = 0.f;
#pragma unroll
          for (int c = 0; c < 5; ++c)
            if (tu4(PX, nu, c) != 0.f) acc += tu4(PX, nu, c) * ct[c][xi][ch];
          v[ch] = acc;
        }
        store_split4_pair(vp, hf, v);
        vp += 2 * plane;
      }
    }
    vt += 2 * a.Cv;
#pragma unroll
    for (int c = 0; c < 3; ++c)
#pragma unroll
      for (int xi = 0; xi < 6; ++xi)
#pragma unroll
        for (int ch = 0; ch < 4; ++ch) ct[c][xi][ch] = ct[c + 2][xi][ch];
  }
}

__device__ __forceinline__ constexpr int up2_rel(int e) { return (e >> 1) + (e & 1); }
template <bool LOW, bool POOL = false, int BELOW = -1>
__global__ __launch_bounds__(256) void wino4_out_kernel(const WinoOutArgs a, size_t total) {
  const size_t i = (size_t)blockIdx.x * blockDim.x + threadIdx.x;
  if (i >= total) return;
  const int ncg = a.Co >> 2;
  const int cg = (int)(i % ncg), cv = cg >> 1, hf = cg & 1;
  size_t t = i / ncg;
  const int tx = (int)(t % a.Tx);
  t /= a.Tx;
  const int ty = (int)(t % a.Ty);
  const int z = (int)(t / a.Ty);
  const size_t Mrows = (size_t)a.Do * a.Ty * a.Tx;
  const size_t m = ((size_t)z * a.Ty + ty) * a.Tx + tx;
  [[maybe_unused]] float bacc[4][4][4];
  if constexpr (BELOW >= 0) {
    constexpr int PY = BELOW >> 1, PX = BELOW & 1;
    const int uy = 4 * ty + a.boy, ux = 4 * tx + a.box;
    const int wy_0 = (uy >> 1) - 1, wx_0 = (ux >> 1) - 1;
    float wy0[6], wy1[6], wx0[6], wx1[6];
#pragma unroll
    for (int s = 0; s < 6; ++s) {
      int i0, i1;
      lin_src(uy + s, 2, a.lH, i0, i1, wy0[s], wy1[s]);
      lin_src(ux + s, 2, a.lW, i0, i1, wx0[s], wx1[s]);
    }
    uint32_t roff[5], coff[5];
#pragma unroll
    for (int r = 0; r < 5; ++r) {
      const int y = wy_0 + r, x = wx_0 + r;
      roff[r] = (uint32_t)(y < 0 ? 0 : (y > a.lH - 1 ? a.lH - 1 : y)) * (uint32_t)(a.lW * a.brow);
      coff[r] = (uint32_t)(x < 0 ? 0 : (x > a.lW - 1 ? a.lW - 1 : x)) * (uint32_t)a.brow;
    }
#pragma unroll
    for (int p = 0; p < 4; ++p)
#pragma unroll
      for (int q = 0; q < 4; ++q)
#pragma unroll
        for (int k = 0; k < 4; ++k) bacc[p][q][k] = 0.f;
    const float* yb = a.below + (size_t)z * a.lH * a.lW * a.brow + 4 * cg;
#pragma unroll
    for (int ky = 0; ky < 3; ++ky)
#pragma unroll
      for (int kx = 0; kx < 3; ++kx) {
        const float* yt = yb + (size_t)(3 * ky + kx) * a.btap;
        const int r_lo = up2_rel(PY + ky), nr = up2_rel(PY + ky + 3) + 2 - r_lo;
        const int c_lo = up2_rel(PX + kx), nc = up2_rel(PX + kx + 3) + 2 - c_lo;
        f32x4_t win[4][4];
#pragma unroll
        for (int r = 0; r < 4; ++r)
#pragma unroll
          for (int c = 0; c < 4; ++c)
            if (r < nr && c < nc) win[r][c] = *(const f32x4_t*)(yt + (roff[r_lo + r] + coff[c_lo + c]));
#pragma unroll
        for (int p = 0; p < 4; ++p) {
          const int ra = up2_rel(PY + ky + p) - r_lo;
          float rowb[4][4];
#pragma unroll
          for (int c = 0; c < 4; ++c)
            if (c < nc) {
#pragma unroll
              for (int k = 0; k < 4; ++k) rowb[c][k] = wy0[ky + p] * win[ra][c][k] + wy1[ky + p] * win[ra + 1][c][k];
            }
#pragma unroll
          for (int q = 0; q < 4; ++q) {
            const int ca = up2_rel(PX + kx + q) - c_lo;
#pragma unroll
            for (int k = 0; k < 4; ++k) bacc[p][q][k] += wx0[kx + q] * rowb[ca][k] + wx1[kx + q] * rowb[ca + 1][k];
          }
        }
#pragma unroll
        for (int p = 0; p < 4; ++p)
#pragma unroll
          for (int q = 0; q < 4; ++q)
#pragma unroll
            for (int k = 0; k < 4; ++k) asm volatile("" : "+v"(bacc[p][q][k]) : : "memory");
      }
  }
  float tp[6][4][4];
#pragma unroll
  for (int nu = 0; nu < 6; ++nu) {
    float mm[6][4];
#pragma unroll
    for (int xi = 0; xi < 6; ++xi) {
      const f32x4_t v = __builtin_nontemporal_load((const f32x4_t*)(a.M + ((size_t)(6 * xi + nu) * Mrows + m) * a.Co + 4 * cg));
#pragma unroll
      for (int k = 0; k < 4; ++k) mm[xi][k] = v[k];
    }
    at4_apply(mm, tp[nu]);
  }
  float bv[4];
#pragma unroll
  for (int k = 0; k < 4; ++k) bv[k] = a.bias[4 * cg + k];
  uint16_t* out = (uint16_t*)a.out;
  [[maybe_unused]] float even[4][4];
#pragma unroll
  for (int p = 0; p < 4; ++p) {
    float in[6][4], y[4][4];
#pragma unroll
    for (int nu = 0; nu < 6; ++nu)
#pragma unroll
      for (int k = 0; k < 4; ++k) in[nu][k] = tp[nu][p][k];
    at4_apply(in, y);
    const int oy = 4 * ty + p;
    if (oy >= a.Ho) continue;
    [[maybe_unused]] float left[4];
#pragma unroll
    for (int q = 0; q < 4; ++q) {
      const int ox = 4 * tx + q;
      if (ox >= a.Wo) continue;
      const size_t e8 = (((size_t)z * a.Ho + oy) * a.Wo + ox) * a.Co + 8 * cv;
      const size_t e = e8 + 4 * hf;
      float v[4];
#pragma unroll
      for (int k = 0; k < 4; ++k) v[k] = y[q][k] + bv[k];
      if constexpr (BELOW >= 0) {
#pragma unroll
        for (int k = 0; k < 4; ++k) v[k] += bacc[p][q][k];
      }
      if (a.addend) {
        const f32x4_t r0 = __builtin_nontemporal_load((const f32x4_t*)(a.addend + e));
#pragma unroll
        for (int k = 0; k < 4; ++k) v[k] += r0[k];
      }
      if constexpr (LOW) {
        int y0, y1, x0, x1;
        float wy0, wy1, wx0, wx1;
        lin_src(oy + a.loy, a.lf, a.lH, y0, y1, wy0, wy1);
        lin_src(ox + a.lox, a.lf, a.lW, x0, x1, wx0, wx1);
        const float* base = a.low + ((size_t)(z + a.loz) * a.lH * a.lW) * a.Co + 4 * cg;
        const f32x4_t r00 = *(const f32x4_t*)(base + ((size_t)y0 * a.lW + x0) * a.Co), r01 = *(const f32x4_t*)(base + ((size_t)y0 * a.lW + x1) * a.Co);
        const f32x4_t r10 = *(const f32x4_t*)(base + ((size_t)y1 * a.lW + x0) * a.Co), r11 = *(const f32x4_t*)(base + ((size_t)y1 * a.lW + x1) * a.Co);
#pragma unroll
        for (int k = 0; k < 4; ++k) {
          const float pa = wx0 * r00[k] + wx1 * r01[k];
          const float pb = wx0 * r10[k] + wx1 * r11[k];
          v[k] += wy0 * pa + wy1 * pb;
        }
      }
      if (a.relu) {
#pragma unroll
        for (int k = 0; k < 4; ++k) v[k] = v[k] > 0.f ? v[k] : 0.f;
      }
      store_split4(out, e8, hf, v);
      if constexpr (POOL) {
        float sv[4];
#pragma unroll
        for (int k = 0; k < 4; ++k) {
          const float h = __uint_as_float((uint32_t)to_bf16(v[k]) << 16);
          sv[k] = h + __uint_as_float((uint32_t)to_bf16(v[k] - h) << 16);
        }
        if ((p & 1) == 0) {
#pragma unroll
          for (int k = 0; k < 4; ++k) even[q][k] = sv[k];
        } else if ((q & 1) == 0) {
#pragma unroll
          for (int k = 0; k < 4; ++k) left[k] = sv[k];
        } else {
          float mx[4];
#pragma unroll
          for (int k = 0; k < 4; ++k) mx[k] = fmaxf(fmaxf(fmaxf(fmaxf(-INFINITY, even[q > 0 ? q - 1 : 0][k]), even[q][k]), left[k]), sv[k]);
          const size_t pe = (((size_t)z * (a.Ho >> 1) + (oy >> 1)) * (a.Wo >> 1) + (ox >> 1)) * a.Co + 8 * cv;
          store_split4((uint16_t*)a.pool, pe, hf, mx);
        }
      }
    }
  }
}

}

static int wino_in_seg_mode() {
  static const int m = [] { const char* e = getenv("BSMI_WINO_IN_SEG"); return e ? atoi(e) : -1; }();
  return m;
}
static void wino_in_segments(int Tx, int& S, int& nseg) {
  const int mode = wino_in_seg_mode();
  S = mode < 0 ? 1 : mode == 0 ? Tx : mode < Tx ? mode : Tx;
  nseg = (Tx + S - 1) / S;
}

int launch_wino_in(const WinoInArgs& a, hipStream_t s) {
  const int m = a.m == 4 ? 4 : 2;
  if (a.m != 0 && a.m != 2 && a.m != 4) BSMI_FAIL(BSMI_ERR_INVALID, "winograd input transform: tile edge %d (2 or 4)", a.m);
  if (a.nsrc < 1 || a.nsrc > kWinoMaxSrc || a.Dv <= 0 || a.Ty <= 0 || a.Tx <= 0 || a.Cv % 8) BSMI_FAIL(BSMI_ERR_INVALID, "winograd input transform: bad geometry");
  for (int q = 0; q < a.nsrc; ++q) {
    if (a.Cpad[q] % 8 || a.cv0[q] % 8 || a.cv0[q] + a.Cpad[q] > a.Cv) BSMI_FAIL(BSMI_ERR_INVALID, "winograd input transform: bad channel layout of source %d", q);
    const int upf = a.upf[q] > 0 ? a.upf[q] : 1;
    if (m == 2 && (a.oy[q] + 2 * a.Ty + 2 > a.H[q] * upf || a.ox[q] + 2 * a.Tx + 2 > a.W[q] * upf)) BSMI_FAIL(BSMI_ERR_INVALID, "winograd input transform: tiles leave source %d", q);
    if (m == 4 && (a.oy[q] < 0 || a.ox[q] < 0 || a.oy[q] + 4 * a.Ty + 2 > a.H[q] * upf + 3 || a.ox[q] + 4 * a.Tx + 2 > a.W[q] * upf + 3))
      BSMI_FAIL(BSMI_ERR_INVALID, "winograd input transform: F(4x4) tiles leave source %d by more than a tile's overhang", q);
    int S = a.Tx, nseg = 1;
    if (m == 4) wino_in_segments(a.Tx, S, nseg);
    const size_t total = (size_t)a.Dv * a.Ty * (a.Cpad[q] / (m == 4 ? 4 : 8)) * nseg;
    const dim3 grid((unsigned)((total + 255) / 256));
    if (a.upf[q] > 0) {
      if (a.upf[q] != 2 || a.oy[q] < 0 || a.ox[q] < 0) BSMI_FAIL(BSMI_ERR_INVALID, "winograd input transform: only a factor-2 upsampling can be fused");
      const int par = 2 * (a.oy[q] & 1) + (a.ox[q] & 1);
      if (m == 4) {
        if (par == 0) hipLaunchKernelGGL((wino4_in_up_kernel<0, 0>), grid, dim3(256), 0, s, a, q, total, S, nseg);
        else if (par == 1) hipLaunchKernelGGL((wino4_in_up_kernel<0, 1>), grid, dim3(256), 0, s, a, q, total, S, nseg);
        else if (par == 2) hipLaunchKernelGGL((wino4_in_up_kernel<1, 0>), grid, dim3(256), 0, s, a, q, total, S, nseg);
        else hipLaunchKernelGGL((wino4_in_up_kernel<1, 1>), grid, dim3(256), 0, s, a, q, total, S, nseg);
      } else if (par == 0) hipLaunchKernelGGL((wino_in_up_kernel<0, 0>), grid, dim3(256), 0, s, a, q, total);
      else if (par == 1) hipLaunchKernelGGL((wino_in_up_kernel<0, 1>), grid, dim3(256), 0, s, a, q, total);
      else if (par == 2) hipLaunchKernelGGL((wino_in_up_kernel<1, 0>), grid, dim3(256), 0, s, a, q, total);
      else hipLaunchKernelGGL((wino_in_up_kernel<1, 1>), grid, dim3(256), 0, s, a, q, total);
    } else if (m == 4) {
      hipLaunchKernelGGL(wino4_in_kernel, grid, dim3(256), 0, s, a, q, total, S, nseg);
    } else {
      hipLaunchKernelGGL(wino_in_kernel, grid, dim3(256), 0, s, a, q, total);
    }
  }
  BSMI_HIP(hipGetLastError());
  return BSMI_OK;
}

int launch_wino_out(const WinoOutArgs& a, hipStream_t s) {
  const int m = a.m == 4 ? 4 : 2;
  if (a.m != 0 && a.m != 2 && a.m != 4) BSMI_FAIL(BSMI_ERR_INVALID, "winograd output transform: tile edge %d (2 or 4)", a.m);
  if (a.Do <= 0 || a.Ty <= 0 || a.Tx <= 0 || a.Co % 8) BSMI_FAIL(BSMI_ERR_INVALID, "winograd output transform: bad geometry");
  const int Ho = m == 4 ? a.Ho : 2 * a.Ty, Wo = m == 4 ? a.Wo : 2 * a.Tx;
  if (m == 4 && (Ho < 1 || Wo < 1 || Ho > 4 * a.Ty || Wo > 4 * a.Tx || Ho + 3 < 4 * a.Ty || Wo + 3 < 4 * a.Tx)) BSMI_FAIL(BSMI_ERR_INVALID, "winograd output transform: output extent and F(4x4) tile counts disagree");
  if (a.pool && (m != 4 || a.low || (Ho & 1) || (Wo & 1))) BSMI_FAIL(BSMI_ERR_INVALID, "winograd output transform: a pooled output needs F(4x4), even extents and no low-resolution residual");
  if (a.low && (a.lf < 1 || a.loz < 0 || a.loz + a.Do > a.lD || a.loy < 0 || a.loy + Ho > a.lH * a.lf || a.lox < 0 || a.lox + Wo > a.lW * a.lf))
    BSMI_FAIL(BSMI_ERR_INVALID, "winograd output transform: the low-resolution residual does not cover the output");
  if (a.below) {
    if (m != 4 || a.lf != 2 || a.low || a.pool) BSMI_FAIL(BSMI_ERR_INVALID, "winograd output transform: sums below the upsampling need F(4x4), a factor of 2, no residual below it and no pooled output");
    if (a.lH < 1 || a.lW < 1 || (int64_t)a.lH * a.lW * a.brow >= ((int64_t)1 << 31) || a.brow < a.Co || a.btap < a.Co || a.boy < 0 || a.box < 0 || a.boy + Ho + 2 > 2 * a.lH || a.box + Wo + 2 > 2 * a.lW)
      BSMI_FAIL(BSMI_ERR_INVALID, "winograd output transform: the sums below the upsampling do not cover the stage's input");
  }
  const size_t total = (size_t)a.Do * a.Ty * a.Tx * (a.Co / (m == 4 ? 4 : 8));
  const dim3 grid((unsigned)((total + 255) / 256));
  if (m == 4) {
    if (a.below) {
      const int par = 2 * (a.boy & 1) + (a.box & 1);
      if (par == 0) hipLaunchKernelGGL((wino4_out_kernel<false, false, 0>), grid, dim3(256), 0, s, a, total);
      else if (par == 1) hipLaunchKernelGGL((wino4_out_kernel<false, false, 1>), grid, dim3(256), 0, s, a, total);
      else if (par == 2) hipLaunchKernelGGL((wino4_out_kernel<false, false, 2>), grid, dim3(256), 0, s, a, total);
      else hipLaunchKernelGGL((wino4_out_kernel<false, false, 3>), grid, dim3(256), 0, s, a, total);
    } else if (a.low) hipLaunchKernelGGL(wino4_out_kernel<true>, grid, dim3(256), 0, s, a, total);
    else if (a.pool) hipLaunchKernelGGL((wino4_out_kernel<false, true>), grid, dim3(256), 0, s, a, total);
    else hipLaunchKernelGGL(wino4_out_kernel<false>, grid, dim3(256), 0, s, a, total);
  } else if (a.low) hipLaunchKernelGGL(wino_out_kernel<true>, grid, dim3(256), 0, s, a, total);
  else hipLaunchKernelGGL(wino_out_kernel<false>, grid, dim3(256), 0, s, a, total);
  BSMI_HIP(hipGetLastError());
  return BSMI_OK;
}

void wino_units(int Cv, std::vector<WinoUnit>& out) {
  out.clear();
  for (int c32 = 0; c32 < Cv; c32 += 32)
    for (int kz = 0; kz < 3; ++kz)
      for (int j = 0; j < kUnitsPerStep; ++j) {
        const int c = c32 + 16 * j;
        if (c < Cv) out.push_back(WinoUnit{kz, c, false});
        else out.push_back(WinoUnit{0, 0, true});
      }
  if ((out.size() / kUnitsPerStep) % 2)
    for (int j = 0; j < kUnitsPerStep; ++j) out.push_back(WinoUnit{0, 0, true});
}

static inline uint16_t host_bf16(float f) {
  uint32_t u;
  memcpy(&u, &f, 4);
  if ((u & 0x7fffffffu) > 0x7f800000u) return (uint16_t)((u >> 16) | 0x40);
  u += 0x7fffu + ((u >> 16) & 1u);
  return (uint16_t)(u >> 16);
}
static inline float host_bf16_f32(uint16_t b) {
  const uint32_t u = (uint32_t)b << 16;
  float f;
  memcpy(&f, &u, 4);
  return f;
}

void wino_pack_weights(const float* w, int cout, int cin, const std::vector<int>& cin_of_v, int Npad, const std::vector<WinoUnit>& units,
                       std::vector<uint16_t>& packed, size_t& image_elems, size_t& batch_elems, int m) {
  const size_t nsteps = units.size() / kUnitsPerStep;
  const int T = m + 2, nbatch = T * T;
  batch_elems = nsteps * (size_t)Npad * 32;
  image_elems = nbatch * batch_elems + (size_t)kWeightRowSlack * 32;
  packed.assign(2 * image_elems, 0);
  static const double G2[4][3] = {{1, 0, 0}, {.5, .5, .5}, {.5, -.5, .5}, {0, 0, 1}};
  const double a = 0.70710678118654752440, b = 1.41421356237309504880;
  const double G4[6][3] = {{1, 0, 0}, {2. / 3, 2. / 3 * a, 1. / 3}, {2. / 3, -2. / 3 * a, 1. / 3}, {1. / 12, b / 12, 1. / 6}, {1. / 12, -b / 12, 1. / 6}, {0, 0, 1}};
  double G[6][3];
  for (int i = 0; i < T; ++i)
    for (int k = 0; k < 3; ++k) G[i][k] = m == 4 ? G4[i][k] : G2[i][k];
  host_parallel_for((size_t)cout, [&](size_t n_) {
    const int n = (int)n_;
    for (size_t u = 0; u < units.size(); ++u) {
      const WinoUnit& un = units[u];
      if (un.dummy) continue;
      const size_t s = u / kUnitsPerStep, j = u % kUnitsPerStep;
      for (int kk = 0; kk < 16; ++kk) {
        const int c = cin_of_v[un.vc0 + kk];
        if (c < 0) continue;
        const float* g = w + (((size_t)n * cin + c) * 3 + un.kz) * 9;
        double t[6][3];
        for (int xi = 0; xi < T; ++xi)
          for (int kx = 0; kx < 3; ++kx) t[xi][kx] = G[xi][0] * g[kx] + G[xi][1] * g[3 + kx] + G[xi][2] * g[6 + kx];
        for (int xi = 0; xi < T; ++xi)
          for (int nu = 0; nu < T; ++nu) {
            const float v = (float)(t[xi][0] * G[nu][0] + t[xi][1] * G[nu][1] + t[xi][2] * G[nu][2]);
            const size_t idx = (size_t)(T * xi + nu) * batch_elems + (s * Npad + n) * 32 + j * 16 + kk;
            const uint16_t hi = host_bf16(v);
            packed[idx] = hi;
            packed[image_elems + idx] = host_bf16(v - host_bf16_f32(hi));
          }
      }
    }
  });
}


struct WinoPackDev {
  const float* w;
  const int* cin_of_v;
  const int* unit_kz;
  const int* unit_vc0;
  uint16_t* image;
  size_t image_elems, batch_elems;
  int cout, cin, Npad, nunits, T;
};
template <int T>
__global__ __launch_bounds__(256) void wino_pack_kernel(const WinoPackDev a) {
#pragma clang fp contract(off)
  const size_t i = (size_t)blockIdx.x * blockDim.x + threadIdx.x;
  const size_t total = (size_t)(a.nunits / kUnitsPerStep) * a.cout * 32;
  if (i >= total) return;
  const int kk = (int)(i & 15), j = (int)((i >> 4) & 1);
  const size_t r = i >> 5;
  const int n = (int)(r % a.cout);
  const size_t s = r / a.cout;
  const int u = (int)(s * kUnitsPerStep + j);
  const int kz = a.unit_kz[u];
  if (kz < 0) return;
  const int c = a.cin_of_v[a.unit_vc0[u] + kk];
  if (c < 0) return;
  const float* g = a.w + (((size_t)n * a.cin + c) * 3 + kz) * 9;
  double gd[9];
#pragma unroll
  for (int k = 0; k < 9; ++k) gd[k] = (double)g[k];
  constexpr double aa = 0.70710678118654752440, bb = 1.41421356237309504880;
  constexpr double G4[6][3] = {{1, 0, 0}, {2. / 3, 2. / 3 * aa, 1. / 3}, {2. / 3, -2. / 3 * aa, 1. / 3}, {1. / 12, bb / 12, 1. / 6}, {1. / 12, -bb / 12, 1. / 6}, {0, 0, 1}};
  constexpr double G2[6][3] = {{1, 0, 0}, {.5, .5, .5}, {.5, -.5, .5}, {0, 0, 1}, {0, 0, 0}, {0, 0, 0}};
  double t[T][3];
#pragma unroll
  for (int xi = 0; xi < T; ++xi)
#pragma unroll
    for (int kx = 0; kx < 3; ++kx) {
      const double g0 = T == 6 ? G4[xi][0] : G2[xi][0], g1 = T == 6 ? G4[xi][1] : G2[xi][1], g2 = T == 6 ? G4[xi][2] : G2[xi][2];
      t[xi][kx] = g0 * gd[kx] + g1 * gd[3 + kx] + g2 * gd[6 + kx];
    }
#pragma unroll
  for (int xi = 0; xi < T; ++xi)
#pragma unroll
    for (int nu = 0; nu < T; ++nu) {
      const double g0 = T == 6 ? G4[nu][0] : G2[nu][0], g1 = T == 6 ? G4[nu][1] : G2[nu][1], g2 = T == 6 ? G4[nu][2] : G2[nu][2];
      const float v = (float)(t[xi][0] * g0 + t[xi][1] * g1 + t[xi][2] * g2);
      const size_t idx = (size_t)(T * xi + nu) * a.batch_elems + (s * a.Npad + n) * 32 + j * 16 + kk;
      const uint16_t hi = to_bf16(v);
      a.image[idx] = hi;
      a.image[a.image_elems + idx] = to_bf16(v - __uint_as_float((uint32_t)hi << 16));
    }
}

int wino_pack_weights_dev(const float* w, int cout, int cin, const std::vector<int>& cin_of_v, int Npad, const std::vector<WinoUnit>& units, int m,
                          void** image_dev, size_t& image_elems, size_t& batch_elems) {
  const size_t nsteps = units.size() / kUnitsPerStep;
  const int T = m + 2, nbatch = T * T;
  batch_elems = nsteps * (size_t)Npad * 32;
  image_elems = nbatch * batch_elems + (size_t)kWeightRowSlack * 32;
  uint16_t* image = nullptr;
  BSMI_HIP(hipMalloc((void**)&image, 2 * image_elems * sizeof(uint16_t)));
  hipError_t err = hipMemsetAsync(image, 0, 2 * image_elems * sizeof(uint16_t), nullptr);
  float* wd = nullptr;
  int* meta = nullptr;
  std::vector<int> hm(cin_of_v);
  const size_t o_kz = hm.size();
  for (const WinoUnit& u : units) hm.push_back(u.dummy ? -1 : u.kz);
  const size_t o_vc = hm.size();
  for (const WinoUnit& u : units) hm.push_back(u.dummy ? 0 : u.vc0);
  const size_t wbytes = (size_t)cout * cin * 27 * sizeof(float);
  if (err == hipSuccess) err = hipMalloc((void**)&wd, wbytes);
  if (err == hipSuccess) err = hipMalloc((void**)&meta, hm.size() * sizeof(int));
  if (err == hipSuccess) err = hipMemcpy(wd, w, wbytes, hipMemcpyHostToDevice);
  if (err == hipSuccess) err = hipMemcpy(meta, hm.data(), hm.size() * sizeof(int), hipMemcpyHostToDevice);
  if (err == hipSuccess) {
    WinoPackDev a;
    a.w = wd; a.cin_of_v = meta; a.unit_kz = meta + o_kz; a.unit_vc0 = meta + o_vc; a.image = image;
    a.image_elems = image_elems; a.batch_elems = batch_elems; a.cout = cout; a.cin = cin; a.Npad = Npad; a.nunits = (int)units.size(); a.T = T;
    const size_t total = nsteps * (size_t)cout * 32;
    if (T == 6) hipLaunchKernelGGL(wino_pack_kernel<6>, dim3((unsigned)((total + 255) / 256)), dim3(256), 0, nullptr, a);
    else hipLaunchKernelGGL(wino_pack_kernel<4>, dim3((unsigned)((total + 255) / 256)), dim3(256), 0, nullptr, a);
    err = hipGetLastError();
    if (err == hipSuccess) err = hipDeviceSynchronize();
  }
  if (wd) (void)hipFree(wd);
  if (meta) (void)hipFree(meta);
  if (err != hipSuccess) {
    (void)hipFree(image);
    BSMI_HIP(err);
  }
  *image_dev = image;
  return BSMI_OK;
}

}
```

### bootstrapper_amd/unet.py

```python
import ctypes as C
import json
import os

import numpy as np
import torch

from . import _lib
from ._lib import lib, check

HEAD_OF_OUTPUT = {"3d_affs": "affs_head", "3d_lsds": "lsds_head", "2d_affs": "aff_head", "2d_lsds": "lsd_head"}

PRECISIONS = {"f32": _lib.PREC_F32, "fp32": _lib.PREC_F32, "float32": _lib.PREC_F32,
              "bf16": _lib.PREC_BF16, "bfloat16": _lib.PREC_BF16,
              "bf16x3": _lib.PREC_BF16X3}


def _tuplify(x):
    return [[int(v) for v in ks] for ks in x]


def _lift(k):
    k = [int(v) for v in k]
    if len(k) == 2:
        return [1] + k
# ... 32 lines not shown
        for i, ks in enumerate(src):
            if len(ks) > _lib.MAX_CONVS:
                raise ValueError(f"at most {_lib.MAX_CONVS} convolutions per pass supported")
            dst_n[i] = len(ks)
            for j, k in enumerate(ks):
                k = _lift(k)
                for d in range(3):
                    dst_k[i][j][d] = k[d]
    heads = []
    for name, val in net_config["outputs"].items():
        if name not in HEAD_OF_OUTPUT:
            raise ValueError(f"output {name!r} has no head in this engine")
        heads.append((HEAD_OF_OUTPUT[name], int(val["dims"])))
    if len(heads) > _lib.MAX_HEADS:
        raise ValueError("too many heads")
    cfg.num_heads = len(heads)
    for i, (hn, dims) in enumerate(heads):
        cfg.head_name[i].value = hn.encode()
        cfg.head_dims[i] = dims
    return cfg, heads


class Model:

    def __init__(self, net_config, device=0, precision="bf16x3"):
        if isinstance(net_config, (str, os.PathLike)):
            with open(net_config) as f:
                net_config = json.load(f)
        self.net_config = net_config
        self.device = int(device)
        self.precision = PRECISIONS[precision]
        self._cfg, self.heads = make_config(net_config)
        dfs = net_config["downsample_factors"]
        self.two_d = bool(dfs) and len(dfs[0]) == 2
        self.raw_mode = _lib.RAW_U8 if "in_channels" in net_config else _lib.RAW_U8_UNIT
        self.stack_infer = False
        self.param_shapes = {}
        self._h = C.c_void_p()
        check(lib.bsmi_unet_create(C.byref(self._cfg), self.device, C.byref(self._h)))
        self._finalized = set()

    def __del__(self):
        h = getattr(self, "_h", None)
        if h:
            lib.bsmi_unet_destroy(h)
            self._h = None

    def load_state_dict(self, state_dict):
        self._state_dict = state_dict
        for k, v in state_dict.items():
            if hasattr(v, "detach"):
                v = v.detach().cpu().numpy()
            a = np.ascontiguousarray(v, dtype=np.float32)
            self.param_shapes[k] = tuple(a.shape)
            if self.two_d and a.ndim == 4:
                a = a[:, :, None]
            shape = (C.c_int64 * a.ndim)(*a.shape)
            check(lib.bsmi_unet_load_weight(self._h, k.encode(), a.ctypes.data_as(C.c_void_p), shape, a.ndim))
        self._finalized.clear()
        self._finalize(self.precision)
        return self

    def clone(self):
        sd = getattr(self, "_state_dict", None)
        if sd is None:
            raise RuntimeError("clone(): no weights loaded")
        other = Model(self.net_config, device=self.device, precision={v: k for k, v in PRECISIONS.items()}[self.precision])
        other.stack_infer = self.stack_infer
        return other.load_state_dict(sd)

    def load_checkpoint(self, checkpoint):
        path = checkpoint if os.path.exists(checkpoint) else f"{checkpoint}.ckpt"
        if not os.path.exists(path):
            raise FileNotFoundError(f"Neither {checkpoint} nor {checkpoint}.ckpt were found.")
        try:
            sd = torch.load(path, map_location="cpu", weights_only=True)
        except Exception:
            sd = torch.load(path, map_location="cpu", weights_only=False)
        sd = sd.get("state_dict", sd.get("model_state_dict", sd))
        sd = {k.removeprefix("model."): v for k, v in sd.items()}
        return self.load_state_dict(sd)

    def _finalize(self, prec):
        if prec not in self._finalized:
            check(lib.bsmi_unet_finalize(self._h, prec))
            self._finalized.add(prec)

    def set_precision(self, precision):
        self.precision = PRECISIONS[precision]
        self._finalize(self.precision)
        return self

    def eval(self):
        return self

    def set_persistent_grid(self, n_cus):
        check(lib.bsmi_unet_set_persistent_grid(self._h, int(n_cus)))
        return self

    def output_shape(self, in_shape):
        out = (C.c_int64 * 3)()
        check(lib.bsmi_unet_output_shape(self._h, _lib.i64x3(in_shape), out))
        return tuple(out)

    def flops(self, in_shape):
        f = C.c_double()
        check(lib.bsmi_unet_flops(self._h, _lib.i64x3(in_shape), C.byref(f)))
        return f.value

    def profile(self, on=True):
        check(lib.bsmi_unet_profile_enable(self._h, int(on)))
        return self

    def read_profile(self):
        n = C.c_int()
        cap = 256
        types = (C.c_int32 * cap)()
        ms = (C.c_double * cap)()
        fl = (C.c_double * cap)()
        check(lib.bsmi_unet_profile_read(self._h, cap, C.byref(n), types, ms, fl))
        return [(types[i], ms[i], fl[i]) for i in range(min(n.value, cap))]

    def profile_totals(self, reset=False):
        ms = (C.c_double * 5)()
        fl = (C.c_double * 5)()
        cnt = (C.c_int64 * 5)()
        check(lib.bsmi_unet_profile_totals(self._h, ms, fl, cnt, 1 if reset else 0))
        names = ["input", "conv", "pool", "upsample", "head"]
        return {names[i]: (ms[i], fl[i], cnt[i]) for i in range(5)}

    def profile_executed(self, reset=False):
        v = C.c_double()
        check(lib.bsmi_unet_profile_executed(self._h, C.byref(v), 1 if reset else 0))
        return v.value

    def debug_activation(self, step, what=0):
        shape = (C.c_int64 * 4)()
        check(lib.bsmi_unet_debug_activation(self._h, int(step), int(what), shape, None, 0))
        out = np.empty(tuple(shape), dtype=np.float32)
        check(lib.bsmi_unet_debug_activation(self._h, int(step), int(what), shape, out.ctypes.data_as(C.c_void_p), out.size))
        return out

    def plan_steps(self):
        n = C.c_int()
        check(lib.bsmi_unet_debug_step_info(self._h, 0, None, C.byref(n)))
        out = []
        for i in range(n.value):
            si = _lib.StepInfo()
            check(lib.bsmi_unet_debug_step_info(self._h, i, C.byref(si), None))
            d = {"step": i, "type": _lib.STEP_TYPES[si.type], "materialised": bool(si.materialised), "shape": tuple(si.shape)}
            if d["type"] == "conv":
                d.update(prefix=si.prefix.decode(), conv=si.conv_index, form=_lib.CONV_FORMS[si.form],
                         flags=tuple(name for bit, name in _lib.STEP_FLAGS.items() if si.flags & bit), bn=si.bn, ksteps=si.ksteps,
                         below_up=bool(si.flags & _lib.STEP_BELOW_UP))
            elif d["type"] == "head":
                d.update(prefix=si.prefix.decode(), head=si.head)
            elif d["type"] in ("pool", "up"):
                d.update(factor=tuple(si.factor))
                if d["type"] == "up":
                    d.update(offset=tuple(si.offset))
            out.append(d)
        return out

    def _run(self, raw, raw_dtype, in_shape, want_f32, want_u8):
        dev = torch.device("cuda", self.device)
        osz = self.output_shape(in_shape)
        nh = len(self.heads)
        f32 = [torch.empty((d,) + osz, dtype=torch.float32, device=dev) if want_f32 else None
               for _, d in self.heads]
        u8 = [torch.empty((d,) + osz, dtype=torch.uint8, device=dev) if want_u8 else None
              for _, d in self.heads]
        pf = (C.c_void_p * nh)(*[t.data_ptr() if t is not None else None for t in f32])
        pu = (C.c_void_p * nh)(*[t.data_ptr() if t is not None else None for t in u8])
        stream = torch.cuda.current_stream(dev).cuda_stream
        check(lib.bsmi_unet_forward(self._h, self.precision, C.c_void_p(raw.data_ptr()), raw_dtype,
                                    _lib.i64x3(in_shape), pf, pu, C.c_void_p(stream)))
        return f32, u8

    def forward(self, *inputs):
        if not all(t.is_cuda for t in inputs):
            raise RuntimeError("bootstrapper_amd.Model runs on the GPU only; move the input to cuda")
        input = inputs[0] if len(inputs) == 1 else torch.cat(inputs, dim=1)
        if self.two_d:
            if input.dim() == 5:
                n, c, d, hh, ww = input.shape
                input = input.reshape(n, c * d, hh, ww)
            if input.dim() != 4 or input.shape[0] != 1:
                raise ValueError("expected input of shape (1, C, H, W)")
            input = input[:, :, None]
        if input.dim() != 5 or input.shape[0] != 1:
            raise ValueError("expected input of shape (1, C, D, H, W)")
        if input.shape[1] != self._cfg.in_channels:
            raise ValueError(f"expected {self._cfg.in_channels} input channels, got {input.shape[1]}")
        x = input.to(torch.float32).contiguous()
        f32, _ = self._run(x, _lib.RAW_F32, x.shape[2:], True, False)
        outs = [t[None] for t in f32]
        if self.two_d and not self.stack_infer:
            outs = [t[:, :, 0] for t in outs]
        return outs[0] if len(outs) == 1 else tuple(outs)

    __call__ = forward

    def predict_u8(self, raw_u8, want_f32=False):
        if raw_u8.dtype != torch.uint8 or not raw_u8.is_cuda:
            raise ValueError("raw_u8 must be a uint8 CUDA tensor")
        x = raw_u8.contiguous()
        shape = x.shape[-3:]
        cin = 1 if x.dim() == 3 else x.shape[0]
        if cin != self._cfg.in_channels:
            raise ValueError(f"expected {self._cfg.in_channels} input channels, got {cin}")
        f32, u8 = self._run(x, self.raw_mode, shape, want_f32, True)
        return (u8, f32) if want_f32 else u8


def extract_block_reflect(vol_u8, offset, block_shape):
    out = torch.empty(tuple(int(s) for s in block_shape), dtype=torch.uint8, device=vol_u8.device)
    stream = torch.cuda.current_stream(vol_u8.device).cuda_stream
    check(lib.bsmi_extract_block_reflect_u8(C.c_void_p(vol_u8.data_ptr()), _lib.i64x3(vol_u8.shape),
                                            _lib.i64x3(offset), _lib.i64x3(block_shape),
                                            C.c_void_p(out.data_ptr()), C.c_void_p(stream)))
    return out
```

### include/bsmi.h

```cpp
#ifndef BSMI_H
#define BSMI_H

#include <stddef.h>
#include <stdint.h>

#ifdef __cplusplus
extern "C" {
#endif

#define BSMI_MAX_LEVELS 8
#define BSMI_MAX_CONVS 4
#define BSMI_MAX_HEADS 4
#define BSMI_NAME_LEN 32

#define BSMI_OK 0
#define BSMI_ERR_INVALID (-1)
#define BSMI_ERR_HIP (-2)
#define BSMI_ERR_STATE (-3)
#define BSMI_ERR_MISSING (-4)
#define BSMI_ERR_OVERFLOW (-5)

#define BSMI_PREC_F32 0
#define BSMI_PREC_BF16 1
#define BSMI_PREC_BF16X3 2
// ... 1 lines not shown

#define BSMI_RAW_U8 0
#define BSMI_RAW_F32 1
#define BSMI_RAW_U8_UNIT 2

const char *bsmi_last_error(void);
int bsmi_version(void);


typedef struct bsmi_unet_config {
  int32_t in_channels;
  int32_t num_fmaps;
  int32_t fmap_inc_factor;
  int32_t num_levels;
  int32_t downsample_factors[BSMI_MAX_LEVELS][3];
  int32_t n_convs_down[BSMI_MAX_LEVELS];
  int32_t kernel_size_down[BSMI_MAX_LEVELS][BSMI_MAX_CONVS][3];
  int32_t n_convs_up[BSMI_MAX_LEVELS];
  int32_t kernel_size_up[BSMI_MAX_LEVELS][BSMI_MAX_CONVS][3];
  int32_t num_heads;
  char head_name[BSMI_MAX_HEADS][BSMI_NAME_LEN];
  int32_t head_dims[BSMI_MAX_HEADS];
  int32_t num_fmaps_out;
} bsmi_unet_config;

typedef struct bsmi_unet bsmi_unet;

int bsmi_unet_create(const bsmi_unet_config *cfg, int device, bsmi_unet **out);
int bsmi_unet_destroy(bsmi_unet *h);

int bsmi_unet_load_weight(bsmi_unet *h, const char *key, const float *data_host,
                          const int64_t *shape, int ndim);
int bsmi_unet_finalize(bsmi_unet *h, int precision);

int bsmi_unet_output_shape(bsmi_unet *h, const int64_t in_shape[3], int64_t out_shape[3]);
int bsmi_unet_flops(bsmi_unet *h, const int64_t in_shape[3], double *flops);

int bsmi_unet_forward(bsmi_unet *h, int precision, const void *raw_dev, int raw_dtype,
                      const int64_t in_shape[3], float *const *out_f32_dev,
                      uint8_t *const *out_u8_dev, void *stream);

int bsmi_unet_train_set_arithmetic(bsmi_unet *h, int split_bf16);
int bsmi_unet_train_set_deterministic(bsmi_unet *h, int on);
int bsmi_unet_train_begin(bsmi_unet *h, const int64_t in_shape[3]);
int bsmi_unet_train_forward_backward(bsmi_unet *h, const float *raw_dev, const float *const *targets_dev,
                                     const float *const *weights_dev, float *loss_host, void *stream);
int bsmi_unet_train_num_params(bsmi_unet *h, uint64_t *count);
int bsmi_unet_train_buffers(bsmi_unet *h, float **params_dev, float **grads_dev);
int bsmi_unet_train_param_info(bsmi_unet *h, const char *key, uint64_t *offset, uint64_t *count);
int bsmi_unet_train_adam_step(bsmi_unet *h, float lr, float beta1, float beta2, float eps, float grad_scale,
                              void *stream);
int bsmi_unet_train_read_param(bsmi_unet *h, const char *key, int what, float *host_out);
int bsmi_unet_train_last_loss(bsmi_unet *h, float *loss_host, void *stream);
int bsmi_unet_train_prediction(bsmi_unet *h, int head, float **out_dev, uint64_t *count);
int bsmi_unet_train_grad_groups(bsmi_unet *h, int max_n, int *n, uint64_t *offsets, uint64_t *counts);
int bsmi_unet_train_wait_grad_group(bsmi_unet *h, int group, void *stream);
int bsmi_unet_train_write_param(bsmi_unet *h, const char *key, int what, const float *host_in);
int bsmi_unet_train_step_count(bsmi_unet *h, int set_to, int *value);
int bsmi_unet_train_end(bsmi_unet *h);

enum {
  BSMI_TRAIN_DBG_DOUT = 0,
  BSMI_TRAIN_DBG_GMASK = 1,
  BSMI_TRAIN_DBG_GSPLIT = 2,
  BSMI_TRAIN_DBG_GSPLIT_HI = 3,
  BSMI_TRAIN_DBG_GSPLIT_LO = 4,
  BSMI_TRAIN_DBG_DCAT = 5,
  BSMI_TRAIN_DBG_HEAD_DP = 6,
  BSMI_TRAIN_DBG_PAD_COUNT = 7
};
int bsmi_unet_train_debug_tensor(bsmi_unet *h, int step, int what, int64_t shape_out[4], float *host_out,
                                 uint64_t capacity);

enum { BSMI_WGRAD_NONE = 0, BSMI_WGRAD_WAVE_F32 = 1, BSMI_WGRAD_TILED_F32 = 2, BSMI_WGRAD_SPLIT = 3 };
typedef struct {
  int32_t family;
  int32_t residual;
  int32_t n, c, cbase;
  int32_t kx;
  int32_t tile_n, tile_c;
  int32_t ranges, lines_per_range;
  int32_t det_workspace;
} bsmi_unet_train_wgrad_info;
typedef struct {
  int32_t type;
  int32_t n_wgrad;
  bsmi_unet_train_wgrad_info wgrad[4];
  int32_t dgrad;
  int32_t dgrad_raw;
  int32_t dgrad_converted;
  int32_t dgrad_bn, dgrad_ksteps, dgrad_split_k, dgrad_scatter, dgrad_residual;
  int32_t border[3];
  int32_t has_split;
  int32_t bias;
  int32_t up;
  int32_t fwd_split;
  int32_t deterministic;
} bsmi_unet_train_step_info;
int bsmi_unet_train_debug_step_info(bsmi_unet *h, int step, bsmi_unet_train_step_info *info);

int bsmi_train_affinity_targets(int device, int64_t *labels_dev, const uint8_t *unlabelled_dev,
                                const int64_t shape[3], const int32_t *neighborhood, int n, int grow_steps,
                                int only_xy, float clip_min, float clip_max, float *affs_dev,
                                float *weights_dev, void *stream);

int bsmi_train_lsd_targets(int device, const int64_t *labels_dev, const uint8_t *unlabelled_dev, const int64_t shape[3],
                           const int64_t roi_offset[3], const int64_t roi_shape[3], const float sigma[3],
                           const float voxel_size[3], int downsample, float *lsds_dev, float *weights_dev, void *stream);

int bsmi_train_lsd2d_targets(int device, const int64_t *labels_dev, const uint8_t *unlabelled_dev, int n_sections,
                             const int64_t shape[2], const int64_t roi_offset[2], const int64_t roi_shape[2], const float sigma[2],
                             const float voxel_size[2], int downsample, float *lsds_dev, float *weights_dev, void *stream);

int bsmi_train_affinity_targets_roi(int device, int64_t *labels_dev, const uint8_t *unlabelled_dev, int n_samples,
                                    const int64_t shape[3], const int64_t roi_offset[3], const int64_t roi_shape[3],
                                    const int32_t *neighborhood, int n, int grow_steps, int only_xy, float clip_min,
                                    float clip_max, float *affs_dev, float *weights_dev, void *stream);

int bsmi_train_mask_sat(int device, const uint8_t *mask_dev, int n_sections, int height, int width, uint32_t *sat_dev,
                        void *stream);

int bsmi_unet_set_persistent_grid(bsmi_unet *h, int n_cus);

int bsmi_stream_create_cu_mask(int device, const uint32_t *cu_mask, int n_words, void **stream_out);
int bsmi_stream_destroy(int device, void *stream);

int bsmi_unet_profile_enable(bsmi_unet *h, int on);
int bsmi_unet_profile_read(bsmi_unet *h, int max_n, int *n, int32_t *types, double *ms,
                           double *flops);
int bsmi_unet_profile_totals(bsmi_unet *h, double ms_by_type[5], double flops_by_type[5],
                             int64_t launches_by_type[5], int reset);
int bsmi_unet_profile_executed(bsmi_unet *h, double *executed_flops, int reset);
int bsmi_debug_lds_canary(int lds_bytes, int blocks, int spins, unsigned long long *mismatches_dev, void *stream);
int bsmi_debug_check_guards(void);

int bsmi_unet_debug_activation(bsmi_unet *h, int step, int what, int64_t shape_out[4], float *host_out,
                               uint64_t capacity);

enum { BSMI_STEP_INPUT = 0, BSMI_STEP_CONV = 1, BSMI_STEP_POOL = 2, BSMI_STEP_UP = 3, BSMI_STEP_HEAD = 4 };
enum {
  BSMI_FORM_GATHER = 0,
  BSMI_FORM_RASTER_HALO = 1,
  BSMI_FORM_BOX_HALO = 2,
  BSMI_FORM_HALO_RESIDENT = 3,
  BSMI_FORM_FIRST_PASS = 4,
  BSMI_FORM_WINO2 = 5,
  BSMI_FORM_WINO4 = 6,
  BSMI_FORM_COUNT = 7
};
enum {
  BSMI_STEP_FUSED_UP = 1,
  BSMI_STEP_RES_LOW = 2,
  BSMI_STEP_SPLIT_K = 4,
  BSMI_STEP_BELOW_UP = 8
};
typedef struct {
  int32_t type;
  int32_t materialised;
  int32_t shape[4];
  int32_t conv_index;
  int32_t form;
  int32_t flags;
  int32_t bn;
  int32_t ksteps;
  int32_t head;
  int32_t factor[3];
  int32_t offset[3];
  char prefix[64];
} bsmi_unet_step_info;
int bsmi_unet_debug_step_info(bsmi_unet *h, int step, bsmi_unet_step_info *info, int *n_steps);

int bsmi_extract_block_reflect_u8(const uint8_t *vol_dev, const int64_t vol_shape[3],
                                  const int64_t offset[3], const int64_t block_shape[3],
                                  uint8_t *block_dev, void *stream);

typedef struct bsmi_seg bsmi_seg;
int bsmi_seg_create(int device, const int64_t max_shape[3], bsmi_seg **out);
int bsmi_seg_destroy(bsmi_seg *h);

int bsmi_ws_fragments_u8(bsmi_seg *h, const uint8_t *affs_dev, const int64_t shape[3],
                         int fragments_in_xy, int min_seed_distance, uint64_t *frags_dev,
                         uint64_t *max_id_dev, void *stream);

int bsmi_ws_fragments_seeds_u8(bsmi_seg *h, const uint8_t *affs_dev, const int64_t shape[3],
                               int fragments_in_xy, int min_seed_distance, uint64_t *frags_dev,
                               uint64_t *max_id_dev, uint64_t *seeds_dev, void *stream);

int bsmi_agglomerate_mean_u8(bsmi_seg *h, const uint8_t *affs_dev, const uint64_t *frags_dev,
                             const int64_t shape[3], const float *thresholds_host,
                             int n_thresholds, uint64_t *segs_dev, void *stream);

int bsmi_agglomerate_hist_u8(bsmi_seg *h, const uint8_t *affs_dev, const uint64_t *frags_dev,
                             const int64_t shape[3], const float *thresholds_host, int n_thresholds,
                             int quantile, int init_with_max, uint64_t *segs_dev, void *stream);

int bsmi_agglomerate_hist_graph(uint32_t n_nodes, uint32_t n_edges, const uint32_t *edge_u, const uint32_t *edge_v,
                                uint32_t *hist, int quantile, int init_with_max, const float *thresholds,
                                int n_thresholds, uint32_t *roots_out);

int bsmi_frag_postprocess_u8(bsmi_seg *h, const uint8_t *affs_dev, uint64_t *frags_dev,
                             const int64_t shape[3], double filter_value, int64_t min_size,
                             const int64_t crop_offset[3], const int64_t crop_shape[3],
                             uint64_t id_offset, uint64_t *out_dev, uint64_t *num_labels_dev,
                             void *stream);

int bsmi_label_stats(bsmi_seg *h, const uint64_t *labels_dev, const int64_t shape[3], uint64_t id_offset,
                     uint64_t num, uint64_t *size_dev, uint64_t *sums_dev, void *stream);

int bsmi_rag_merge_scores_u8(bsmi_seg *h, const uint8_t *affs_dev, const uint64_t *frags_dev,
                             const int64_t shape[3], float threshold, int discretize_queue,
                             uint64_t *edges_dev, float *scores_dev, uint64_t edge_capacity,
                             uint64_t *merges_dev, float *merge_scores_dev, uint64_t *counts_dev,
                             void *stream);

int bsmi_rag_graph_u8(bsmi_seg *h, const uint8_t *affs_dev, const uint64_t *frags_dev, const int64_t shape[3],
                      uint64_t *edges_dev, uint64_t *sums_dev, uint32_t *pair_counts_dev, uint64_t edge_capacity,
                      uint64_t *counts_dev, void *stream);
int bsmi_rag_merge_scores_host(int n_graphs, const uint64_t *n_edges, uint64_t *const *edges, uint64_t *const *sums,
                               uint32_t *const *pair_counts, float threshold, int discretize_queue, float *const *scores,
                               int n_threads);
#define BSMI_QUEUE_BINS_N_MINUS_1 0
#define BSMI_QUEUE_BINS_N 1
int bsmi_rag_merge_scores_host_rule(int n_graphs, const uint64_t *n_edges, uint64_t *const *edges, uint64_t *const *sums,
                                    uint32_t *const *pair_counts, float threshold, int discretize_queue, int bin_rule,
                                    float *const *scores, int n_threads);

int bsmi_rag_agglomerate_u8(bsmi_seg *h, const uint8_t *affs_dev, uint64_t *frags_dev, const int64_t shape[3],
                            float threshold, int discretize_queue, void *stream);

int bsmi_rag_edge_stats(bsmi_seg *h, uint64_t *sums_dev, uint64_t *counts_dev, uint64_t capacity, void *stream);

int bsmi_lut_relabel(int device, const uint64_t *in_dev, uint64_t n, const uint64_t *keys_dev,
                     const uint64_t *vals_dev, uint64_t m, uint64_t *out_dev, void *stream);
int bsmi_lut_relabel_multi(int device, const uint64_t *in_dev, uint64_t n, const uint64_t *keys_dev,
                           const uint64_t *vals_dev, uint64_t m, int n_columns, uint64_t *out_dev, void *stream);

int bsmi_connected_components(const uint64_t *nodes, uint64_t n, const uint64_t *edges,
                              const float *scores, uint64_t m, float threshold, uint64_t *components);
int bsmi_connected_components_multi(const uint64_t *nodes, uint64_t n, const uint64_t *edges,
                                    const float *scores, uint64_t m, const float *thresholds,
                                    int n_thresholds, uint64_t *components);

int bsmi_cc_affs_u8(bsmi_seg *h, const uint8_t *affs_dev, const int64_t shape[3], int cut, int64_t min_size,
                    uint64_t *frags_dev, uint64_t *seg_dev, uint64_t *num_labels_dev, void *stream);

int bsmi_mws_agglom_f64(int device, const double *affs_dev, int n_offsets, const int32_t *offsets,
                        const int32_t *strides, uint32_t random_seed, const int64_t shape[3],
                        uint64_t *labels_dev, void *stream);

int bsmi_mws_cluster(uint64_t n_nodes, const uint64_t *edges, const double *scores, uint64_t m,
                     uint64_t *labels_out);

int bsmi_frag_pair_affinity_u8(int device, const uint8_t *affs_dev, int n_offsets, const int32_t *offsets,
                               const uint64_t *dense_dev, const int64_t shape[3], uint64_t capacity,
                               uint64_t *pairs_out, uint64_t *sums_out, uint64_t *counts_out,
                               uint64_t *n_pairs, void *stream);

int bsmi_label_table_u64(bsmi_seg *h, const uint64_t *labels_dev, const int64_t shape[3], int64_t z0,
                         uint64_t *ids_dev, uint64_t *counts_dev, int32_t *zmin_dev, int32_t *zmax_dev,
                         uint64_t capacity, uint64_t *n_dev, void *stream);

int bsmi_seg_set_host_flood(bsmi_seg *h, int on);

int bsmi_seg_status(bsmi_seg *h, void *stream);

typedef struct bsmi_seg_batch bsmi_seg_batch;
typedef struct {
  const uint8_t *affs_dev;
  uint64_t *frags_dev;
  uint64_t *max_id_dev;
  uint64_t *labels_dev;
  uint64_t *num_labels_dev;
  uint64_t id_offset;
  uint64_t *size_dev;
  uint64_t *sums_dev;
} bsmi_batch_frag_args;
typedef struct {
  const uint8_t *affs_dev;
  const uint64_t *frags_dev;
  uint64_t *edges_dev;
  uint64_t *sums_dev;
  uint32_t *pair_counts_dev;
  uint64_t *counts_dev;
  uint64_t edge_capacity;
} bsmi_batch_graph_args;
int bsmi_seg_batch_create(bsmi_seg *const *handles, int n, bsmi_seg_batch **out);
int bsmi_seg_batch_destroy(bsmi_seg_batch *b);
int bsmi_seg_batch_fragments_u8(bsmi_seg_batch *b, int n_blocks, const bsmi_batch_frag_args *args, const int64_t shape[3],
                                int fragments_in_xy, int min_seed_distance, double filter_value, int64_t min_size,
                                const int64_t crop_offset[3], const int64_t crop_shape[3], uint64_t stats_num, void *stream);
int bsmi_seg_batch_rag_graph_u8(bsmi_seg_batch *b, int n_blocks, const bsmi_batch_graph_args *args, const int64_t shape[3],
                                void *stream);

typedef struct bsmi_eval bsmi_eval;
int bsmi_eval_create(int device, uint64_t pair_capacity, bsmi_eval **out);
int bsmi_eval_destroy(bsmi_eval *h);

int bsmi_eval_aff_errors_u8(bsmi_eval *h, const uint64_t *seg_dev, const int64_t seg_shape[3], const int64_t seg_origin[3],
                            const uint8_t *pred_dev, int n_channels, const int64_t tile_shape[3], const uint8_t *mask_dev,
                            const int32_t *offsets, const int64_t chunk_shape[3], float floor_, float ceil_, int64_t count_z_end,
                            uint8_t *error_map_dev, uint8_t *error_mask_dev, uint64_t *hist_dev, void *stream);

int bsmi_eval_lsd_errors_u8(bsmi_eval *h, const uint64_t *seg_dev, const int64_t seg_shape[3], const int64_t seg_origin[3],
                            const uint8_t *pred_dev, const uint8_t *mask_dev, const int64_t tile_shape[3],
                            const int64_t chunk_shape[3], const int64_t margin[3], const int64_t context[3], const float sigma[3],
                            const float voxel_size[3], int downsample, float floor_, float ceil_, int64_t count_z_end,
                            uint64_t scratch_limit_bytes, uint8_t *error_map_dev, uint8_t *error_mask_dev, uint64_t *hist_dev,
                            float *debug_desc_dev, float *debug_diff_dev, float *debug_max_dev, uint8_t *debug_raw_mask_dev,
                            void *stream);

int bsmi_eval_pairs_u64(bsmi_eval *h, const uint64_t *gt_dev, const uint64_t *seg_dev, const uint8_t *mask_dev,
                        const int64_t shape[3], int reset, void *stream);

int bsmi_eval_pairs_read(bsmi_eval *h, uint64_t *gt_out_dev, uint64_t *seg_out_dev, uint64_t *count_out_dev,
                         uint64_t out_capacity, uint64_t *n_dev, void *stream);

int bsmi_eval_status(bsmi_eval *h, void *stream);

#define BSMI_MORPH_DILATE 0
#define BSMI_MORPH_ERODE 1
int bsmi_label_morph_u64(int device, const uint64_t *in_dev, const int64_t shape[3], int op, int iterations, int xy,
                         uint64_t *out_dev, uint64_t *tmp_dev, void *stream);

// ... 150 lines not shown
```

Baseline: 114.8.

## Add Winograd F(2,3) transform along z for wide 3D convolutions

Adds an optional z-axis Winograd F(2,3) transform on top of the existing 2D F(4x4) transform, giving a 6x6x4 transform domain with 144 GEMM batches over half as many z rows. Weights are packed with the extra z transform and the z taps folded in, the input transform adds or subtracts pairs of z planes, and a new output kernel applies the inverse z transform. By default it activates only for conv sites with at least 1024 input and output channels that are not fused with upsampling or pooling. The goal is fewer multiplies per output in the deepest layers, at the cost of larger transform buffers, another rounding stage and lower occupancy in the input kernel.

Result: faster. 117.0, median of 6 (+1.9%).

```diff
diff --git a/bootstrapper_amd/_lib.py b/bootstrapper_amd/_lib.py
--- a/bootstrapper_amd/_lib.py
+++ b/bootstrapper_amd/_lib.py
@@ -54,6 +54,7 @@
 CONV_FORMS = ("gather", "raster-halo", "box-halo", "halo-resident", "first-pass", "winograd F(2x2)", "winograd F(4x4)")
 STEP_FLAGS = {1: "fused-up", 2: "res-low", 4: "split-k"}
 STEP_BELOW_UP = 8
+STEP_WINO_Z = 16
 
 
 class Codec(C.Structure):
@@ -119,6 +120,8 @@
         "bsmi_unet_forward": (i32, [p, i32, vp, i32, i64p, C.POINTER(vp), C.POINTER(vp), vp]),
         "bsmi_unet_debug_activation": (i32, [p, i32, i32, i64p, vp, C.c_uint64]),
         "bsmi_unet_debug_step_info": (i32, [p, i32, C.POINTER(StepInfo), C.POINTER(i32)]),
+        "bsmi_debug_wino_pack_host": (i32, [vp, i32, i32, i32, vp, C.c_uint64, C.POINTER(C.c_uint64), C.POINTER(C.c_uint64),
+                                            C.POINTER(i32), C.POINTER(i32)]),
         "bsmi_unet_profile_enable": (i32, [p, i32]),
         "bsmi_unet_profile_read": (i32, [p, i32, C.POINTER(i32), C.POINTER(C.c_int32), C.POINTER(C.c_double),
                                          C.POINTER(C.c_double)]),
diff --git a/bootstrapper_amd/csrc/unet_debug.hip b/bootstrapper_amd/csrc/unet_debug.hip
--- a/bootstrapper_amd/csrc/unet_debug.hip
+++ b/bootstrapper_amd/csrc/unet_debug.hip
@@ -3,6 +3,30 @@
 #include "unet_internal.h"
 
 extern "C" {
+
+int bsmi_debug_wino_pack_host(const float* w, int cout, int cin, int wz, uint16_t* out, uint64_t capacity, uint64_t* image_elems, uint64_t* batch_elems,
+                              int* npad, int* ksteps) {
+  if (!w || cout < 1 || cin < 1) BSMI_FAIL(BSMI_ERR_INVALID, "bad argument");
+  std::vector<int> cin_of_v;
+  for (int c = 0; c < round_up(cin, kChanPad); ++c) cin_of_v.push_back(c < cin ? c : -1);
+  const int Npad = round_up(cout, tile_bn(choose_tile(cout)));
+  std::vector<WinoUnit> units;
+  wino_units((int)cin_of_v.size(), units, wz ? 1 : 3);
+  if (image_elems || batch_elems || out) {
+    std::vector<uint16_t> packed;
+    size_t ie = 0, be = 0;
+    wino_pack_weights(w, cout, cin, cin_of_v, Npad, units, packed, ie, be, 4, wz != 0);
+    if (image_elems) *image_elems = ie;
+    if (batch_elems) *batch_elems = be;
+    if (out) {
+      if (capacity < packed.size()) BSMI_FAIL(BSMI_ERR_INVALID, "buffer of %llu values too small", (unsigned long long)capacity);
+      memcpy(out, packed.data(), packed.size() * sizeof(uint16_t));
+    }
+  }
+  if (npad) *npad = Npad;
+  if (ksteps) *ksteps = (int)(units.size() / kUnitsPerStep);
+  return BSMI_OK;
+}
 
 int bsmi_unet_debug_activation(bsmi_unet* h, int step, int what, int64_t shape_out[4], float* host_out, uint64_t capacity) {
   if (!h || !shape_out) BSMI_FAIL(BSMI_ERR_INVALID, "null argument");
@@ -81,6 +105,7 @@
       if (up || st.wino_out.low || st.wino_has_below) info->flags |= BSMI_STEP_FUSED_UP;
       if (st.wino_has_below) info->flags |= BSMI_STEP_BELOW_UP;
       if (st.wino_has_res_low) info->flags |= BSMI_STEP_RES_LOW;
+      if (st.wino_in.wz) info->flags |= BSMI_STEP_WINO_Z;
       if (conv_igemm_split_k(st.wino_gemm, plan->prec, st.tile, sk_grid) ||
           (st.wino_has_res && conv_igemm_split_k(st.wino_res, plan->prec, st.tile, sk_grid)) ||
           (st.wino_has_res_low && conv_igemm_split_k(st.wino_res_low, plan->prec, st.tile, sk_grid)) ||
diff --git a/bootstrapper_amd/csrc/unet_internal.h b/bootstrapper_amd/csrc/unet_internal.h
--- a/bootstrapper_amd/csrc/unet_internal.h
+++ b/bootstrapper_amd/csrc/unet_internal.h
@@ -52,6 +52,7 @@
   bool ready = false;
   int m = 2;
   bool fused_only = false;
+  bool wz = false;
   std::vector<WinoUnit> units;
   std::vector<int> cin_of_v;
   int Cv = 0;
@@ -231,6 +232,7 @@
 int wino_tile_edge();
 bool wino_narrow_last(const bsmi_unet* h, const PassSite& p, int ci);
 bool below_up_site(const bsmi_unet* h, const PassSite& p, int ci);
+bool wino_z_site(const bsmi_unet* h, const PassSite& p, int ci);
 bool fuse_up_enabled();
 bool pool_fuse_enabled();
 int h16_mode();
diff --git a/bootstrapper_amd/csrc/unet_pack.hip b/bootstrapper_amd/csrc/unet_pack.hip
--- a/bootstrapper_amd/csrc/unet_pack.hip
+++ b/bootstrapper_amd/csrc/unet_pack.hip
@@ -203,17 +203,18 @@
   pw.m = wino_tile_edge();
   pw.tile = choose_tile(p.cout);
   pw.Npad = round_up(p.cout, tile_bn(pw.tile));
-  wino_units(pw.Cv, pw.units);
+  pw.wz = !pw.fused_only && pw.m == 4 && wino_z_site(h, p, ci);
+  wino_units(pw.Cv, pw.units, pw.wz ? 1 : 3);
   {
     size_t image_elems = 0, batch_elems = 0;
     static const bool on_host = [] { const char* e = getenv("BSMI_WINO_PACK_HOST"); return e && e[0] == '1'; }();
     if (on_host) {
       std::vector<uint16_t> packed;
-      wino_pack_weights(wm.data.data(), p.cout, cin_m, pw.cin_of_v, pw.Npad, pw.units, packed, image_elems, batch_elems, pw.m);
+      wino_pack_weights(wm.data.data(), p.cout, cin_m, pw.cin_of_v, pw.Npad, pw.units, packed, image_elems, batch_elems, pw.m, pw.wz);
       BSMI_HIP(hipMalloc(&pw.w, packed.size() * 2));
       BSMI_HIP(hipMemcpy(pw.w, packed.data(), packed.size() * 2, hipMemcpyHostToDevice));
     } else {
-      const int rc = wino_pack_weights_dev(wm.data.data(), p.cout, cin_m, pw.cin_of_v, pw.Npad, pw.units, pw.m, &pw.w, image_elems, batch_elems);
+      const int rc = wino_pack_weights_dev(wm.data.data(), p.cout, cin_m, pw.cin_of_v, pw.Npad, pw.units, pw.m, &pw.w, image_elems, batch_elems, pw.wz);
       if (rc) return rc;
     }
     pw.lo_image_bytes = image_elems * 2;
diff --git a/bootstrapper_amd/csrc/unet_plan.hip b/bootstrapper_amd/csrc/unet_plan.hip
--- a/bootstrapper_amd/csrc/unet_plan.hip
+++ b/bootstrapper_amd/csrc/unet_plan.hip
@@ -484,7 +484,7 @@
     for (int d = 0; d < 3; ++d) st.f[d] = f[d];
     PlanStep& prod = plan->steps.back();
     if (pool_fuse_enabled() && prec == BSMI_PREC_BF16X3 && f[0] == 1 && f[1] == 2 && f[2] == 2 && prod.type == PlanStep::CONV && prod.use_wino &&
-        prod.wino_out.m == 4 && !prod.wino_out.low && prod.wino_out.out == f_left.ptr && !(f_left.H & 1) && !(f_left.W & 1)) {
+        prod.wino_out.m == 4 && !prod.wino_out.low && !prod.wino_out.wz && prod.wino_out.out == f_left.ptr && !(f_left.H & 1) && !(f_left.W & 1)) {
       prod.wino_out.pool = g_in.ptr;
       st.pool_fused = true;
     }
diff --git a/bootstrapper_amd/csrc/unet_plan_wino.hip b/bootstrapper_amd/csrc/unet_plan_wino.hip
--- a/bootstrapper_amd/csrc/unet_plan_wino.hip
+++ b/bootstrapper_amd/csrc/unet_plan_wino.hip
@@ -31,6 +31,7 @@
   PlanStep& st;
   bool below;
   bool cut;
+  bool wz;
   int wm, nbatch, Dv, Ty, Tx, Cv;
   size_t vbatch, Mrows;
   void *V = nullptr, *Mbuf = nullptr, *addend = nullptr, *low = nullptr, *Ybuf = nullptr;
@@ -62,6 +63,8 @@
     wi.V = V;
     wi.Dv = Dv; wi.Ty = Ty; wi.Tx = Tx; wi.Cv = Cv;
     wi.m = wm;
+    wi.wz = wz ? 1 : 0;
+    wi.Dz = o.D + 2;
     return BSMI_OK;
   }
 
@@ -85,7 +88,7 @@
     raw_gemm(g, below ? pw.skip_w : pw.w, below ? pw.skip_lo_image_bytes : pw.lo_image_bytes, pw.Npad);
     g.bias = pc.bias;
     g.out = Mbuf;
-    g.Do = o.D; g.Ho = Ty; g.Wo = Tx; g.Co = o.Cpad;
+    g.Do = wz ? Dv : o.D; g.Ho = Ty; g.Wo = Tx; g.Co = o.Cpad;
     g.M = (int)Mrows;
     g.nbatch = nbatch;
     g.a_batch = (int64_t)vbatch;
@@ -223,6 +226,7 @@
     wo.Do = o.D; wo.Ty = Ty; wo.Tx = Tx; wo.Co = o.Cpad;
     wo.m = wm; wo.Ho = o.H; wo.Wo = o.W;
     wo.relu = 1;
+    wo.wz = wz ? 1 : 0;
     const double kstep = (double)kUnitsPerStep * sube(prec);
     st.exec_flops = 2.0 * (double)round_up((int)Mrows, 256) * pw.Npad * ((double)st.wino_gemm.nsteps * kstep) * nbatch * 3.0;
     if (st.wino_has_res) st.exec_flops += 2.0 * (double)round_up(st.wino_res.M, 256) * pw.Npad * ((double)st.wino_res.nsteps * kstep) * 3.0;
@@ -239,24 +243,27 @@
   const PackedWino& pw = p.wino[ci];
   const bool wants_fused = fuse_up && (ci == 0 || ci == p.nconv - 1);
   if (pw.fused_only && !fuse_up) return BSMI_OK;
-  const int wm = pw.m, nbatch = wino_batches(wm);
+  const bool wz = pw.wz;
+  const int wm = pw.m, nbatch = wino_batches(wm) * (wz ? kWinoZ : 1);
+  if (wz && (wm != 4 || wants_fused)) BSMI_FAIL(BSMI_ERR_STATE, "%s conv %d: packed for the z transform, but planned behind a fused upsampling", p.prefix.c_str(), ci);
   if (prec != BSMI_PREC_BF16X3 || !pw.ready || (wm == 2 && ((o.H & 1) || (o.W & 1))) || st.use_box || st.use_rh) {
     if (wants_fused) BSMI_FAIL(BSMI_ERR_STATE, "%s conv %d: the upsampling was fused into this stage, which cannot take the Winograd form", p.prefix.c_str(), ci);
     return BSMI_OK;
   }
   const bool below = fuse_up && ci == 0 && pw.below_ready && wm == 4 && nsl == 2;
-  const int Dv = o.D + 2, Ty = (o.H + wm - 1) / wm, Tx = (o.W + wm - 1) / wm, Cv = below ? pw.skip_Cv : pw.Cv;
+  const int Dv = wz ? (o.D + 1) / 2 : o.D + 2, Ty = (o.H + wm - 1) / wm, Tx = (o.W + wm - 1) / wm, Cv = below ? pw.skip_Cv : pw.Cv;
   const size_t vbatch = (size_t)Dv * Ty * Tx * Cv * 4;
   if (vbatch >= ((size_t)1 << 31)) {
     if (wants_fused) BSMI_FAIL(BSMI_ERR_STATE, "%s conv %d: fused upsampling, but the transformed input is too large", p.prefix.c_str(), ci);
     return BSMI_OK;
   }
-  const size_t Mrows = (size_t)o.D * Ty * Tx;
+  const size_t Mrows = (size_t)(wz ? Dv : o.D) * Ty * Tx;
+  if (Mrows >= ((size_t)1 << 31)) BSMI_FAIL(BSMI_ERR_STATE, "%s conv %d: too many rows in a batch of the transform-domain GEMM", p.prefix.c_str(), ci);
   const bool cut = fuse_up && ci == p.nconv - 1;
-  WinoStage w{plan, fuse_up, p, ci, pc, pw, slots, so, o, st, below, cut, wm, nbatch, Dv, Ty, Tx, Cv, vbatch, Mrows};
-  BSMI_HIP(hipMalloc(&w.V, nbatch * vbatch + 4096));
+  WinoStage w{plan, fuse_up, p, ci, pc, pw, slots, so, o, st, below, cut, wz, wm, nbatch, Dv, Ty, Tx, Cv, vbatch, Mrows};
+  BSMI_HIP(hipMalloc(&w.V, (size_t)nbatch * vbatch + 4096));
   plan->allocs.push_back(w.V);
-  BSMI_HIP(hipMalloc(&w.Mbuf, nbatch * Mrows * o.Cpad * sizeof(float)));
+  BSMI_HIP(hipMalloc(&w.Mbuf, (size_t)nbatch * Mrows * o.Cpad * sizeof(float)));
   plan->allocs.push_back(w.Mbuf);
   plan->bytes += nbatch * (vbatch + Mrows * o.Cpad * sizeof(float));
   int rc = w.input_transform();
diff --git a/bootstrapper_amd/csrc/unet_rules.hip b/bootstrapper_amd/csrc/unet_rules.hip
--- a/bootstrapper_amd/csrc/unet_rules.hip
+++ b/bootstrapper_amd/csrc/unet_rules.hip
@@ -73,6 +73,34 @@
   return pool_fuse;
 }
 
+static int wino_z_mode() {
+  static const int m = [] { const char* e = getenv("BSMI_WINO_Z"); return e ? atoi(e) : -1; }();
+  return m;
+}
+bool wino_z_site(const bsmi_unet* h, const PassSite& p, int ci) {
+  if (wino_z_mode() == 0 || wino_tile_edge() != 4 || !wino_eligible(p, ci)) return false;
+  int cin = p.cout;
+  if (ci == 0) {
+    cin = 0;
+    for (int s = 0; s < p.nslots; ++s) cin += p.cin[s];
+  }
+  if (&p >= h->r_conv.data() && &p < h->r_conv.data() + h->r_conv.size()) {
+    const int* f = h->cfg.downsample_factors[&p - h->r_conv.data()];
+    const bool fusable = fuse_up_enabled() && p.nslots == 2 && f[0] == 1 && f[1] == 2 && f[2] == 2;
+    if (fusable && (ci == 0 || ci == p.nconv - 1)) return false;
+  } else if (&p >= h->l_conv.data() && &p < h->l_conv.data() + h->l_conv.size()) {
+    const size_t i = &p - h->l_conv.data();
+    if (i + 1 < h->l_conv.size() && ci == p.nconv - 1) {
+      const int* f = h->cfg.downsample_factors[i];
+      if (pool_fuse_enabled() && f[0] == 1 && f[1] == 2 && f[2] == 2) return false;
+    }
+  } else {
+    return false;
+  }
+  if (wino_z_mode() >= 1) return true;
+  return cin >= 1024 && p.cout >= 1024;
+}
+
 int h16_mode() {
   static const int m = [] { const char* e = getenv("BSMI_H16"); return e ? atoi(e) : 1; }();
   return m;
diff --git a/bootstrapper_amd/csrc/wino.h b/bootstrapper_amd/csrc/wino.h
--- a/bootstrapper_amd/csrc/wino.h
+++ b/bootstrapper_amd/csrc/wino.h
@@ -6,8 +6,9 @@
 namespace bsmi {
 
 constexpr int kWinoBatch = 16;
-constexpr int kWinoMaxBatch = 36;
+constexpr int kWinoMaxBatch = 144;
 inline int wino_batches(int m) { return (m + 2) * (m + 2); }
+constexpr int kWinoZ = 4;
 constexpr int kWinoMaxSrc = 2;
 
 struct WinoInArgs {
@@ -20,6 +21,7 @@
   void* V;
   int Dv, Ty, Tx, Cv;
   int m;
+  int wz, Dz;
 };
 
 struct WinoOutArgs {
@@ -36,6 +38,7 @@
   int relu;
   int m, Ho, Wo;
   void* pool;
+  int wz;
 };
 
 int launch_wino_in(const WinoInArgs& a, hipStream_t s);
@@ -45,12 +48,12 @@
   int kz, vc0;
   bool dummy;
 };
-void wino_units(int Cv, std::vector<WinoUnit>& out);
+void wino_units(int Cv, std::vector<WinoUnit>& out, int taps = 3);
 
 void wino_pack_weights(const float* w, int cout, int cin, const std::vector<int>& cin_of_v, int Npad, const std::vector<WinoUnit>& units,
-                       std::vector<uint16_t>& packed, size_t& image_elems, size_t& batch_elems, int m = 2);
+                       std::vector<uint16_t>& packed, size_t& image_elems, size_t& batch_elems, int m = 2, bool wz = false);
 
 int wino_pack_weights_dev(const float* w, int cout, int cin, const std::vector<int>& cin_of_v, int Npad, const std::vector<WinoUnit>& units, int m,
-                          void** image_dev, size_t& image_elems, size_t& batch_elems);
+                          void** image_dev, size_t& image_elems, size_t& batch_elems, bool wz = false);
 
 }
diff --git a/bootstrapper_amd/csrc/wino.hip b/bootstrapper_amd/csrc/wino.hip
--- a/bootstrapper_amd/csrc/wino.hip
+++ b/bootstrapper_amd/csrc/wino.hip
@@ -378,7 +378,8 @@
   __builtin_nontemporal_store(o, (u32x4_t*)p);
 }
 
-__global__ __launch_bounds__(256, 2) void wino4_in_kernel(const WinoInArgs a, int src, size_t total, int S, int nseg) {
+template <bool WZ = false>
+__global__ __launch_bounds__(256, WZ ? 1 : 2) void wino4_in_kernel(const WinoInArgs a, int src, size_t total, int S, int nseg) {
   const unsigned nb = gridDim.x, q = nb >> 3, r = nb & 7, xcd = blockIdx.x & 7, j = blockIdx.x >> 3;
   const unsigned blk = (xcd < r ? xcd * (q + 1) : r * (q + 1) + (xcd - r) * q) + j;
   const size_t i = (size_t)blk * blockDim.x + threadIdx.x;
@@ -388,26 +389,49 @@
   size_t t = i / ncg;
   const int tx0 = (int)(t % nseg) * S, tx1 = tx0 + S < a.Tx ? tx0 + S : a.Tx;
   t /= nseg;
+  int ze = 0;
+  if constexpr (WZ) {
+    ze = (int)(t & 3);
+    t >>= 2;
+  }
   const int ty = (int)(t % a.Ty);
   const int z = (int)(t / a.Ty);
   const uint16_t* sp = (const uint16_t*)a.src[src];
   const int H = a.H[src], W = a.W[src], C = a.Cpad[src];
+  int za = z, zb = z;
+  [[maybe_unused]] float sgn = -1.f;
+  if constexpr (WZ) {
+    za = 2 * z + (ze == 0 ? 0 : ze == 2 ? 2 : 1);
+    zb = 2 * z + (ze == 2 ? 1 : ze == 3 ? 3 : 2);
+    za = za < a.Dz - 1 ? za : a.Dz - 1;
+    zb = zb < a.Dz - 1 ? zb : a.Dz - 1;
+    sgn = ze == 1 ? 1.f : -1.f;
+  }
   size_t erow[6];
 #pragma unroll
   for (int rr = 0; rr < 6; ++rr) {
     int y = 4 * ty + a.oy[src] + rr;
     y = y < H - 1 ? y : H - 1;
-    erow[rr] = (((size_t)(z + a.oz[src]) * H + y) * W) * C + 8 * cv;
-  }
+    erow[rr] = (((size_t)(za + a.oz[src]) * H + y) * W) * C + 8 * cv;
+  }
+  [[maybe_unused]] const ptrdiff_t eb = (ptrdiff_t)(zb - za) * ((ptrdiff_t)H * W * C);
   const size_t plane = (size_t)a.Dv * a.Ty * a.Tx * a.Cv;
-  const size_t e_out = (((size_t)z * a.Ty + ty) * a.Tx) * a.Cv + a.cv0[src] + 8 * cv;
+  const size_t e_out = (((size_t)z * a.Ty + ty) * a.Tx) * a.Cv + a.cv0[src] + 8 * cv + (WZ ? (size_t)ze * 36 * plane : 0);
   float col[6][6][4];
   auto load_col = [&](int c, int x) __attribute__((always_inline)) {
     x += a.ox[src];
     x = x < W - 1 ? x : W - 1;
     float d[6][4];
 #pragma unroll
-    for (int rr = 0; rr < 6; ++rr) load_split4(sp, erow[rr] + (size_t)x * C, hf, d[rr]);
+    for (int rr = 0; rr < 6; ++rr) {
+      load_split4(sp, erow[rr] + (size_t)x * C, hf, d[rr]);
+      if constexpr (WZ) {
+        float d2[4];
+        load_split4(sp, (size_t)((ptrdiff_t)(erow[rr] + (size_t)x * C) + eb), hf, d2);
+#pragma unroll
+        for (int k = 0; k < 4; ++k) d[rr][k] += sgn * d2[k];
+      }
+    }
     bt4_apply(d, col[c]);
   };
   load_col(0, 4 * tx0);
@@ -699,6 +723,98 @@
   }
 }
 
+__global__ __launch_bounds__(256) void wino4z_out_kernel(const WinoOutArgs a, size_t total) {
+  const size_t i = (size_t)blockIdx.x * blockDim.x + threadIdx.x;
+  if (i >= total) return;
+  const int ncg = a.Co >> 2;
+  const int cg = (int)(i % ncg), cv = cg >> 1, hf = cg & 1;
+  size_t t = i / ncg;
+  const int tx = (int)(t % a.Tx);
+  t /= a.Tx;
+  const int ty = (int)(t % a.Ty);
+  const int r = (int)(t / a.Ty);
+  const size_t Mrows = (size_t)((a.Do + 1) >> 1) * a.Ty * a.Tx;
+  const size_t m = ((size_t)r * a.Ty + ty) * a.Tx + tx;
+  const float* mp = a.M + m * a.Co + 4 * cg;
+  const size_t bstride = Mrows * a.Co;
+  float o0[4][4][4], o1[4][4][4];
+#pragma unroll
+  for (int e = 0; e < kWinoZ; ++e) {
+    float tp[6][4][4];
+#pragma unroll
+    for (int nu = 0; nu < 6; ++nu) {
+      float mm[6][4];
+#pragma unroll
+      for (int xi = 0; xi < 6; ++xi) {
+        const f32x4_t v = __builtin_nontemporal_load((const f32x4_t*)(mp + (size_t)(6 * xi + nu) * bstride));
+#pragma unroll
+        for (int k = 0; k < 4; ++k) mm[xi][k] = v[k];
+      }
+      at4_apply(mm, tp[nu]);
+    }
+    mp += 36 * bstride;
+#pragma unroll
+    for (int p = 0; p < 4; ++p) {
+      float in[6][4], y[4][4];
+#pragma unroll
+      for (int nu = 0; nu < 6; ++nu)
+#pragma unroll
+        for (int k = 0; k < 4; ++k) in[nu][k] = tp[nu][p][k];
+      at4_apply(in, y);
+#pragma unroll
+      for (int q = 0; q < 4; ++q)
+#pragma unroll
+        for (int k = 0; k < 4; ++k) {
+          if (e == 0) o0[p][q][k] = y[q][k];
+          if (e == 1) { o0[p][q][k] += y[q][k]; o1[p][q][k] = y[q][k]; }
+          if (e == 2) { o0[p][q][k] += y[q][k]; o1[p][q][k] -= y[q][k]; }
+          if (e == 3) o1[p][q][k] -= y[q][k];
+        }
+    }
+    if (e < kWinoZ - 1) {
+#pragma unroll
+      for (int p = 0; p < 4; ++p)
+#pragma unroll
+        for (int q = 0; q < 4; ++q)
+#pragma unroll
+          for (int k = 0; k < 4; ++k) asm volatile("" : "+v"(o0[p][q][k]) : : "memory");
+    }
+  }
+  float bv[4];
+#pragma unroll
+  for (int k = 0; k < 4; ++k) bv[k] = a.bias[4 * cg + k];
+  uint16_t* out = (uint16_t*)a.out;
+#pragma unroll
+  for (int pl = 0; pl < 2; ++pl) {
+    const int z = 2 * r + pl;
+    if (z >= a.Do) continue;
+#pragma unroll
+    for (int p = 0; p < 4; ++p) {
+      const int oy = 4 * ty + p;
+      if (oy >= a.Ho) continue;
+#pragma unroll
+      for (int q = 0; q < 4; ++q) {
+        const int ox = 4 * tx + q;
+        if (ox >= a.Wo) continue;
+        const size_t e8 = (((size_t)z * a.Ho + oy) * a.Wo + ox) * a.Co + 8 * cv;
+        float v[4];
+#pragma unroll
+        for (int k = 0; k < 4; ++k) v[k] = (pl ? o1[p][q][k] : o0[p][q][k]) + bv[k];
+        if (a.addend) {
+          const f32x4_t r0 = __builtin_nontemporal_load((const f32x4_t*)(a.addend + e8 + 4 * hf));
+#pragma unroll
+          for (int k = 0; k < 4; ++k) v[k] += r0[k];
+        }
+        if (a.relu) {
+#pragma unroll
+          for (int k = 0; k < 4; ++k) v[k] = v[k] > 0.f ? v[k] : 0.f;
+        }
+        store_split4(out, e8, hf, v);
+      }
+    }
+  }
+}
+
 }
 
 static int wino_in_seg_mode() {
@@ -715,6 +831,7 @@
   const int m = a.m == 4 ? 4 : 2;
   if (a.m != 0 && a.m != 2 && a.m != 4) BSMI_FAIL(BSMI_ERR_INVALID, "winograd input transform: tile edge %d (2 or 4)", a.m);
   if (a.nsrc < 1 || a.nsrc > kWinoMaxSrc || a.Dv <= 0 || a.Ty <= 0 || a.Tx <= 0 || a.Cv % 8) BSMI_FAIL(BSMI_ERR_INVALID, "winograd input transform: bad geometry");
+  if (a.wz && (m != 4 || a.Dz < 3 || (a.Dz - 2 + 1) / 2 != a.Dv)) BSMI_FAIL(BSMI_ERR_INVALID, "winograd input transform: bad geometry of the z transform");
   for (int q = 0; q < a.nsrc; ++q) {
     if (a.Cpad[q] % 8 || a.cv0[q] % 8 || a.cv0[q] + a.Cpad[q] > a.Cv) BSMI_FAIL(BSMI_ERR_INVALID, "winograd input transform: bad channel layout of source %d", q);
     const int upf = a.upf[q] > 0 ? a.upf[q] : 1;
@@ -723,9 +840,10 @@
       BSMI_FAIL(BSMI_ERR_INVALID, "winograd input transform: F(4x4) tiles leave source %d by more than a tile's overhang", q);
     int S = a.Tx, nseg = 1;
     if (m == 4) wino_in_segments(a.Tx, S, nseg);
-    const size_t total = (size_t)a.Dv * a.Ty * (a.Cpad[q] / (m == 4 ? 4 : 8)) * nseg;
+    const size_t total = (size_t)a.Dv * a.Ty * (a.Cpad[q] / (m == 4 ? 4 : 8)) * nseg * (a.wz ? kWinoZ : 1);
     const dim3 grid((unsigned)((total + 255) / 256));
     if (a.upf[q] > 0) {
+      if (a.wz) BSMI_FAIL(BSMI_ERR_INVALID, "winograd input transform: the z transform does not read through an upsampling");
       if (a.upf[q] != 2 || a.oy[q] < 0 || a.ox[q] < 0) BSMI_FAIL(BSMI_ERR_INVALID, "winograd input transform: only a factor-2 upsampling can be fused");
       const int par = 2 * (a.oy[q] & 1) + (a.ox[q] & 1);
       if (m == 4) {
@@ -738,7 +856,8 @@
       else if (par == 2) hipLaunchKernelGGL((wino_in_up_kernel<1, 0>), grid, dim3(256), 0, s, a, q, total);
       else hipLaunchKernelGGL((wino_in_up_kernel<1, 1>), grid, dim3(256), 0, s, a, q, total);
     } else if (m == 4) {
-      hipLaunchKernelGGL(wino4_in_kernel, grid, dim3(256), 0, s, a, q, total, S, nseg);
+      if (a.wz) hipLaunchKernelGGL(wino4_in_kernel<true>, grid, dim3(256), 0, s, a, q, total, S, nseg);
+      else hipLaunchKernelGGL(wino4_in_kernel<false>, grid, dim3(256), 0, s, a, q, total, S, nseg);
     } else {
       hipLaunchKernelGGL(wino_in_kernel, grid, dim3(256), 0, s, a, q, total);
     }
@@ -761,9 +880,12 @@
     if (a.lH < 1 || a.lW < 1 || (int64_t)a.lH * a.lW * a.brow >= ((int64_t)1 << 31) || a.brow < a.Co || a.btap < a.Co || a.boy < 0 || a.box < 0 || a.boy + Ho + 2 > 2 * a.lH || a.box + Wo + 2 > 2 * a.lW)
       BSMI_FAIL(BSMI_ERR_INVALID, "winograd output transform: the sums below the upsampling do not cover the stage's input");
   }
-  const size_t total = (size_t)a.Do * a.Ty * a.Tx * (a.Co / (m == 4 ? 4 : 8));
+  if (a.wz && (m != 4 || a.low || a.below || a.pool)) BSMI_FAIL(BSMI_ERR_INVALID, "winograd output transform: the z transform needs F(4x4) and takes no low-resolution sums and no pooled output");
+  const size_t total = (size_t)(a.wz ? (a.Do + 1) / 2 : a.Do) * a.Ty * a.Tx * (a.Co / (m == 4 ? 4 : 8));
   const dim3 grid((unsigned)((total + 255) / 256));
-  if (m == 4) {
+  if (a.wz) {
+    hipLaunchKernelGGL(wino4z_out_kernel, grid, dim3(256), 0, s, a, total);
+  } else if (m == 4) {
     if (a.below) {
       const int par = 2 * (a.boy & 1) + (a.box & 1);
       if (par == 0) hipLaunchKernelGGL((wino4_out_kernel<false, false, 0>), grid, dim3(256), 0, s, a, total);
@@ -779,10 +901,10 @@
   return BSMI_OK;
 }
 
-void wino_units(int Cv, std::vector<WinoUnit>& out) {
+void wino_units(int Cv, std::vector<WinoUnit>& out, int taps) {
   out.clear();
   for (int c32 = 0; c32 < Cv; c32 += 32)
-    for (int kz = 0; kz < 3; ++kz)
+    for (int kz = 0; kz < taps; ++kz)
       for (int j = 0; j < kUnitsPerStep; ++j) {
         const int c = c32 + 16 * j;
         if (c < Cv) out.push_back(WinoUnit{kz, c, false});
@@ -807,9 +929,9 @@
 }
 
 void wino_pack_weights(const float* w, int cout, int cin, const std::vector<int>& cin_of_v, int Npad, const std::vector<WinoUnit>& units,
-                       std::vector<uint16_t>& packed, size_t& image_elems, size_t& batch_elems, int m) {
+                       std::vector<uint16_t>& packed, size_t& image_elems, size_t& batch_elems, int m, bool wz) {
   const size_t nsteps = units.size() / kUnitsPerStep;
-  const int T = m + 2, nbatch = T * T;
+  const int T = m + 2, nbatch = T * T * (wz ? kWinoZ : 1);
   batch_elems = nsteps * (size_t)Npad * 32;
   image_elems = nbatch * batch_elems + (size_t)kWeightRowSlack * 32;
   packed.assign(2 * image_elems, 0);
@@ -829,16 +951,21 @@
         const int c = cin_of_v[un.vc0 + kk];
         if (c < 0) continue;
         const float* g = w + (((size_t)n * cin + c) * 3 + un.kz) * 9;
-        double t[6][3];
-        for (int xi = 0; xi < T; ++xi)
-          for (int kx = 0; kx < 3; ++kx) t[xi][kx] = G[xi][0] * g[kx] + G[xi][1] * g[3 + kx] + G[xi][2] * g[6 + kx];
+        double t[3][6][3];
+        for (int kz = 0; kz < (wz ? 3 : 1); ++kz)
+          for (int xi = 0; xi < T; ++xi)
+            for (int kx = 0; kx < 3; ++kx) t[kz][xi][kx] = G[xi][0] * g[9 * kz + kx] + G[xi][1] * g[9 * kz + 3 + kx] + G[xi][2] * g[9 * kz + 6 + kx];
         for (int xi = 0; xi < T; ++xi)
           for (int nu = 0; nu < T; ++nu) {
-            const float v = (float)(t[xi][0] * G[nu][0] + t[xi][1] * G[nu][1] + t[xi][2] * G[nu][2]);
-            const size_t idx = (size_t)(T * xi + nu) * batch_elems + (s * Npad + n) * 32 + j * 16 + kk;
-            const uint16_t hi = host_bf16(v);
-            packed[idx] = hi;
-            packed[image_elems + idx] = host_bf16(v - host_bf16_f32(hi));
+            double u[3];
+            for (int kz = 0; kz < (wz ? 3 : 1); ++kz) u[kz] = t[kz][xi][0] * G[nu][0] + t[kz][xi][1] * G[nu][1] + t[kz][xi][2] * G[nu][2];
+            for (int e = 0; e < (wz ? kWinoZ : 1); ++e) {
+              const float v = wz ? (float)(G2[e][0] * u[0] + G2[e][1] * u[1] + G2[e][2] * u[2]) : (float)u[0];
+              const size_t idx = (size_t)(T * T * e + T * xi + nu) * batch_elems + (s * Npad + n) * 32 + j * 16 + kk;
+              const uint16_t hi = host_bf16(v);
+              packed[idx] = hi;
+              packed[image_elems + idx] = host_bf16(v - host_bf16_f32(hi));
+            }
           }
       }
     }
@@ -855,7 +982,7 @@
   size_t image_elems, batch_elems;
   int cout, cin, Npad, nunits, T;
 };
-template <int T>
+template <int T, bool WZ = false>
 __global__ __launch_bounds__(256) void wino_pack_kernel(const WinoPackDev a) {
 #pragma clang fp contract(off)
   const size_t i = (size_t)blockIdx.x * blockDim.x + threadIdx.x;
@@ -871,37 +998,51 @@
   const int c = a.cin_of_v[a.unit_vc0[u] + kk];
   if (c < 0) return;
   const float* g = a.w + (((size_t)n * a.cin + c) * 3 + kz) * 9;
-  double gd[9];
-#pragma unroll
-  for (int k = 0; k < 9; ++k) gd[k] = (double)g[k];
+  constexpr int NZ = WZ ? 3 : 1;
+  double gd[NZ][9];
+#pragma unroll
+  for (int kz = 0; kz < NZ; ++kz)
+#pragma unroll
+    for (int k = 0; k < 9; ++k) gd[kz][k] = (double)g[9 * kz + k];
   constexpr double aa = 0.70710678118654752440, bb = 1.41421356237309504880;
   constexpr double G4[6][3] = {{1, 0, 0}, {2. / 3, 2. / 3 * aa, 1. / 3}, {2. / 3, -2. / 3 * aa, 1. / 3}, {1. / 12, bb / 12, 1. / 6}, {1. / 12, -bb / 12, 1. / 6}, {0, 0, 1}};
   constexpr double G2[6][3] = {{1, 0, 0}, {.5, .5, .5}, {.5, -.5, .5}, {0, 0, 1}, {0, 0, 0}, {0, 0, 0}};
-  double t[T][3];
-#pragma unroll
-  for (int xi = 0; xi < T; ++xi)
-#pragma unroll
-    for (int kx = 0; kx < 3; ++kx) {
-      const double g0 = T == 6 ? G4[xi][0] : G2[xi][0], g1 = T == 6 ? G4[xi][1] : G2[xi][1], g2 = T == 6 ? G4[xi][2] : G2[xi][2];
-      t[xi][kx] = g0 * gd[kx] + g1 * gd[3 + kx] + g2 * gd[6 + kx];
-    }
+  double t[NZ][T][3];
+#pragma unroll
+  for (int kz = 0; kz < NZ; ++kz)
+#pragma unroll
+    for (int xi = 0; xi < T; ++xi)
+#pragma unroll
+      for (int kx = 0; kx < 3; ++kx) {
+        const double g0 = T == 6 ? G4[xi][0] : G2[xi][0], g1 = T == 6 ? G4[xi][1] : G2[xi][1], g2 = T == 6 ? G4[xi][2] : G2[xi][2];
+        t[kz][xi][kx] = g0 * gd[kz][kx] + g1 * gd[kz][3 + kx] + g2 * gd[kz][6 + kx];
+      }
 #pragma unroll
   for (int xi = 0; xi < T; ++xi)
 #pragma unroll
     for (int nu = 0; nu < T; ++nu) {
       const double g0 = T == 6 ? G4[nu][0] : G2[nu][0], g1 = T == 6 ? G4[nu][1] : G2[nu][1], g2 = T == 6 ? G4[nu][2] : G2[nu][2];
-      const float v = (float)(t[xi][0] * g0 + t[xi][1] * g1 + t[xi][2] * g2);
-      const size_t idx = (size_t)(T * xi + nu) * a.batch_elems + (s * a.Npad + n) * 32 + j * 16 + kk;
-      const uint16_t hi = to_bf16(v);
-      a.image[idx] = hi;
-      a.image[a.image_elems + idx] = to_bf16(v - __uint_as_float((uint32_t)hi << 16));
+      double u[NZ];
+#pragma unroll
+      for (int kz = 0; kz < NZ; ++kz) u[kz] = t[kz][xi][0] * g0 + t[kz][xi][1] * g1 + t[kz][xi][2] * g2;
+#pragma unroll
+      for (int e = 0; e < (WZ ? kWinoZ : 1); ++e) {
+        float v;
+        if constexpr (WZ) v = (float)(G2[e][0] * u[0] + G2[e][1] * u[1] + G2[e][2] * u[2]);
+        else v = (float)u[0];
+        const size_t idx = (size_t)(T * T * e + T * xi + nu) * a.batch_elems + (s * a.Npad + n) * 32 + j * 16 + kk;
+        const uint16_t hi = to_bf16(v);
+        a.image[idx] = hi;
+        a.image[a.image_elems + idx] = to_bf16(v - __uint_as_float((uint32_t)hi << 16));
+      }
     }
 }
 
 int wino_pack_weights_dev(const float* w, int cout, int cin, const std::vector<int>& cin_of_v, int Npad, const std::vector<WinoUnit>& units, int m,
-                          void** image_dev, size_t& image_elems, size_t& batch_elems) {
+                          void** image_dev, size_t& image_elems, size_t& batch_elems, bool wz) {
+  if (wz && m != 4) BSMI_FAIL(BSMI_ERR_INVALID, "winograd weights: the z transform exists for F(4x4) only");
   const size_t nsteps = units.size() / kUnitsPerStep;
-  const int T = m + 2, nbatch = T * T;
+  const int T = m + 2, nbatch = T * T * (wz ? kWinoZ : 1);
   batch_elems = nsteps * (size_t)Npad * 32;
   image_elems = nbatch * batch_elems + (size_t)kWeightRowSlack * 32;
   uint16_t* image = nullptr;
@@ -924,7 +1065,8 @@
     a.w = wd; a.cin_of_v = meta; a.unit_kz = meta + o_kz; a.unit_vc0 = meta + o_vc; a.image = image;
     a.image_elems = image_elems; a.batch_elems = batch_elems; a.cout = cout; a.cin = cin; a.Npad = Npad; a.nunits = (int)units.size(); a.T = T;
     const size_t total = nsteps * (size_t)cout * 32;
-    if (T == 6) hipLaunchKernelGGL(wino_pack_kernel<6>, dim3((unsigned)((total + 255) / 256)), dim3(256), 0, nullptr, a);
+    if (wz) hipLaunchKernelGGL((wino_pack_kernel<6, true>), dim3((unsigned)((total + 255) / 256)), dim3(256), 0, nullptr, a);
+    else if (T == 6) hipLaunchKernelGGL(wino_pack_kernel<6>, dim3((unsigned)((total + 255) / 256)), dim3(256), 0, nullptr, a);
     else hipLaunchKernelGGL(wino_pack_kernel<4>, dim3((unsigned)((total + 255) / 256)), dim3(256), 0, nullptr, a);
     err = hipGetLastError();
     if (err == hipSuccess) err = hipDeviceSynchronize();
diff --git a/bootstrapper_amd/unet.py b/bootstrapper_amd/unet.py
--- a/bootstrapper_amd/unet.py
+++ b/bootstrapper_amd/unet.py
@@ -208,7 +208,7 @@
             if d["type"] == "conv":
                 d.update(prefix=si.prefix.decode(), conv=si.conv_index, form=_lib.CONV_FORMS[si.form],
                          flags=tuple(name for bit, name in _lib.STEP_FLAGS.items() if si.flags & bit), bn=si.bn, ksteps=si.ksteps,
-                         below_up=bool(si.flags & _lib.STEP_BELOW_UP))
+                         below_up=bool(si.flags & _lib.STEP_BELOW_UP), wino_z=bool(si.flags & _lib.STEP_WINO_Z))
             elif d["type"] == "head":
                 d.update(prefix=si.prefix.decode(), head=si.head)
             elif d["type"] in ("pool", "up"):
diff --git a/include/bsmi.h b/include/bsmi.h
--- a/include/bsmi.h
+++ b/include/bsmi.h
@@ -177,7 +177,8 @@
   BSMI_STEP_FUSED_UP = 1,
   BSMI_STEP_RES_LOW = 2,
   BSMI_STEP_SPLIT_K = 4,
-  BSMI_STEP_BELOW_UP = 8
+  BSMI_STEP_BELOW_UP = 8,
+  BSMI_STEP_WINO_Z = 16
 };
 typedef struct {
   int32_t type;
@@ -194,6 +195,9 @@
   char prefix[64];
 } bsmi_unet_step_info;
 int bsmi_unet_debug_step_info(bsmi_unet *h, int step, bsmi_unet_step_info *info, int *n_steps);
+
+int bsmi_debug_wino_pack_host(const float *w, int cout, int cin, int wz, uint16_t *out, uint64_t capacity,
+                              uint64_t *image_elems, uint64_t *batch_elems, int *npad, int *ksteps);
 
 int bsmi_extract_block_reflect_u8(const uint8_t *vol_dev, const int64_t vol_shape[3],
                                   const int64_t offset[3], const int64_t block_shape[3],
```
